# domerin0/rnn-speech

Measured on AMD Instinct MI355X. Metric: audio_frames_per_sec_train_3x512_lstm_ctc, higher is better.
Workload: dtype f32

## Files before the change

### include/amdspeech.h

```cpp
#ifndef AMDSPEECH_H
#define AMDSPEECH_H

#include <stddef.h>
#include <stdint.h>

#ifdef __cplusplus
extern "C" {
#endif

#define AMDSPEECH_OK 0
#define AMDSPEECH_EINVAL (-1)
#define AMDSPEECH_EHIP (-2)
#define AMDSPEECH_EUNSUPPORTED (-3)
#define AMDSPEECH_ETIMEOUT (-4)

int amdspeech_version(void);
const char* amdspeech_last_error(void);
int amdspeech_device_cu_count(void);

int amdspeech_linear_fwd(void* stream, const float* x, const float* w, const float* b,
                         float* y, int M, int K, int N);
int amdspeech_linear_bwd(void* stream, const float* x, const float* w, const float* dy,
                         float* dx, float* dw, float* db, int M, int K, int N);

// ... 30 lines not shown
                               float* C, int ldc, const float* bias, int accumulate, void* scratch, size_t scratch_bytes);
int amdspeech_gemm_bf16_packed_plan(int transA, int transB, int M, int N, int K, int lda, int ldb, amdspeech_gemm_plan_info* out);
int amdspeech_bf16_copy(void* stream, const float* src, long ld, long rows, int cols, int transpose, unsigned short* dst, long ldd,
                        float* colsum, unsigned short* plain);
int amdspeech_bf16_transpose(void* stream, const unsigned short* src, long rows, int cols, unsigned short* dst, long ldd);

int amdspeech_batchnorm_fwd(void* stream, const float* x, float* y, float* xhat,
                            float* inv_std, int T, int B, int H, float eps);
int amdspeech_batchnorm_bwd(void* stream, const float* dy, const float* xhat,
                            const float* inv_std, float* dx, int T, int B, int H);

int amdspeech_batchnorm_sum(void* stream, const float* x, const float* global_sum, int n_total, float* out,
                            int T, int B, int H);
int amdspeech_batchnorm_apply(void* stream, const float* x, const float* global_sum, const float* global_sq,
                              int n_total, float eps, float* y, float* xhat, float* inv_std, int T, int B, int H);
int amdspeech_batchnorm_bwd_sums(void* stream, const float* dy, const float* xhat, float* sums, int T, int B, int H);
int amdspeech_batchnorm_bwd_apply(void* stream, const float* dy, const float* xhat, const float* inv_std,
                                  const float* global_sums, int n_total, float* dx, int T, int B, int H);

typedef struct amdspeech_lstm_desc {
    int T, B, H, L;
    float keep_in, keep_out;
    uint64_t seed;
    int precision;
    int flags;
} amdspeech_lstm_desc;

enum { AMDSPEECH_LSTM_ARMED = 1, AMDSPEECH_LSTM_ARM_NEXT = 2, AMDSPEECH_LSTM_SAME_WS = 4, AMDSPEECH_LSTM_PER_DIAGONAL = 8,
       AMDSPEECH_LSTM_INJECT_TIMEOUT = 16 };

enum {
    AMDSPEECH_LSTM_WS_Z0 = 0,
    AMDSPEECH_LSTM_WS_ZTOP = 1,
    AMDSPEECH_LSTM_WS_DZTOP = 2,
    AMDSPEECH_LSTM_WS_DZ0 = 3,
    AMDSPEECH_LSTM_WS_HFINAL = 4,
    AMDSPEECH_LSTM_WS_CFINAL = 5,
    AMDSPEECH_LSTM_WS_GATES = 6
};
size_t amdspeech_lstm_workspace_bytes(const amdspeech_lstm_desc* d);
void* amdspeech_lstm_ws_ptr(const amdspeech_lstm_desc* d, void* ws, int which);

int amdspeech_lstm_workspace_release(void* stream, void* ws);

int amdspeech_lstm_beside_forward(void* stream, const void* ws);

int amdspeech_lstm_beside_tail(void* stream, const void* ws);

int amdspeech_lstm_fwd(void* stream, const amdspeech_lstm_desc* d, void* ws,
                       const float* kernels, long kernel_stride,
                       const float* biases, long bias_stride,
                       const int* lengths, const float* h0, const float* c0);
int amdspeech_lstm_pair_fusable(const amdspeech_lstm_desc* d);
int amdspeech_lstm_fwd_pair(void* stream, const amdspeech_lstm_desc* d_a, void* ws_a, const float* kernels_a, const float* biases_a,
                            const amdspeech_lstm_desc* d_b, void* ws_b, const float* kernels_b, const float* biases_b,
                            long kernel_stride, long bias_stride, const int* lengths, const float* h0_a, const float* c0_a);
int amdspeech_lstm_bwd_pair(void* stream, const amdspeech_lstm_desc* d_a, void* ws_a, const float* kernels_a, float* dkernels_a, float* dbiases_a,
                            const amdspeech_lstm_desc* d_b, void* ws_b, const float* kernels_b, float* dkernels_b, float* dbiases_b,
                            long kernel_stride, long bias_stride, const int* lengths);
int amdspeech_lstm_status(const amdspeech_lstm_desc* d, void* ws);
int amdspeech_lstm_bwd(void* stream, const amdspeech_lstm_desc* d, void* ws,
                       const float* kernels, long kernel_stride,
                       float* dkernels, float* dbiases, long bias_stride,
                       const int* lengths);

typedef struct amdspeech_ctc_head {
    const float* w_out;
    const float* b_out;
    float* logits;
    const int* dense_labels;
    float* loss;
    float* dlogits;
    void* ctc_ws;
    int C, U;
} amdspeech_ctc_head;
int amdspeech_lstm_ctc_fusable(const amdspeech_lstm_desc* d, int C, int U);
int amdspeech_lstm_fwd_ctc(void* stream, const amdspeech_lstm_desc* d, void* ws,
                           const float* kernels, long kernel_stride, const float* biases, long bias_stride,
                           const int* lengths, const float* h0, const float* c0, const amdspeech_ctc_head* head);
int amdspeech_lstm_bwd_ctc(void* stream, const amdspeech_lstm_desc* d, void* ws,
                           const float* kernels, long kernel_stride, float* dkernels, float* dbiases, long bias_stride,
                           const int* lengths, const amdspeech_ctc_head* head);

int amdspeech_lstm_dropout_multipliers(void* stream, const amdspeech_lstm_desc* d, int which, int layer, float* out);

enum { AMDSPEECH_LSTM_PATH_FLOW = 0, AMDSPEECH_LSTM_PATH_BIG1 = 1, AMDSPEECH_LSTM_PATH_BIG = 2, AMDSPEECH_LSTM_PATH_HOIST = 3,
       AMDSPEECH_LSTM_PATH_DIAG = 4, AMDSPEECH_LSTM_PATH_DIAG_BF3 = 5 };
typedef struct amdspeech_lstm_plan_info {
    int fwd_path, bwd_path, nmt, kb, mv, wpx, uw, fwd_mt, pair, bf16p, bf16p_reserved, xw_parts, nfw, w_pieces, dz0_inkernel, flow2_q;
} amdspeech_lstm_plan_info;
int amdspeech_lstm_plan(const amdspeech_lstm_desc* d, int C, int U, amdspeech_lstm_plan_info* out);
int amdspeech_lstm_plan_xw_halves(const amdspeech_lstm_desc* d, int C, int U);

enum {
    AMDSPEECH_BIDIR_WS_Z0 = 0, AMDSPEECH_BIDIR_WS_YTOP_FW = 1, AMDSPEECH_BIDIR_WS_YTOP_BW = 2, AMDSPEECH_BIDIR_WS_DYTOP_FW = 3,
    AMDSPEECH_BIDIR_WS_DYTOP_BW = 4, AMDSPEECH_BIDIR_WS_DZ0 = 5, AMDSPEECH_BIDIR_WS_HFINAL = 6, AMDSPEECH_BIDIR_WS_CFINAL = 7
};
size_t amdspeech_lstm_bidir_workspace_bytes(const amdspeech_lstm_desc* d);
void* amdspeech_lstm_bidir_ws_ptr(const amdspeech_lstm_desc* d, void* ws, int which);
long amdspeech_lstm_bidir_layer_stride(const amdspeech_lstm_desc* d);
int amdspeech_lstm_bidir_path(const amdspeech_lstm_desc* d);
int amdspeech_lstm_bidir_fwd(void* stream, const amdspeech_lstm_desc* d, void* ws, const float* const* kernels,
                             const float* const* biases, const int* lengths, const float* h0, const float* c0);
int amdspeech_lstm_bidir_bwd(void* stream, const amdspeech_lstm_desc* d, void* ws, const float* const* kernels,
                             float* const* dkernels, float* const* dbiases, const int* lengths);
int amdspeech_lstm_bidir_status(const amdspeech_lstm_desc* d, void* ws);
int amdspeech_lstm_bidir_dropout_multipliers(void* stream, const amdspeech_lstm_desc* d, int dir, int which, int layer, float* out);

size_t amdspeech_ctc_workspace_bytes(int T, int B, int C, int U);
int amdspeech_ctc_loss_fwd_bwd(void* stream, const float* logits, const int* dense_labels,
                               const int* lengths, int T, int B, int C, int U,
                               float* loss, float* dlogits, void* ws);
int amdspeech_ctc_loss_fwd_bwd_staged(void* stream, const float* logits, const int* dense_labels,
                                      const int* lengths, int T, int B, int C, int U, float* loss,
                                      float* dlogits, void* ws, int stage);

enum { AMDSPEECH_CTC_KERNEL_WAVE = 0, AMDSPEECH_CTC_KERNEL_SHIFT = 1, AMDSPEECH_CTC_KERNEL_PAIR = 2, AMDSPEECH_CTC_KERNEL_EDGE = 3 };
typedef struct amdspeech_ctc_plan_info {
    int kernel, threads, rmax, smax;
} amdspeech_ctc_plan_info;
int amdspeech_ctc_plan(int T, int B, int C, int U, amdspeech_ctc_plan_info* out);

size_t amdspeech_ctc_align_workspace_bytes(int T, int B, int C, int U);
int amdspeech_ctc_align_plan(int T, int B, int C, int U, amdspeech_ctc_plan_info* out);
int amdspeech_ctc_align(void* stream, const float* logits, const int* dense_labels, const int* lengths,
                        int T, int B, int C, int U, int* frame_label, int* frame_state, int* spans,
                        float* score, float* confidence, void* ws);

int amdspeech_ctc_greedy_decode(void* stream, const float* logits, const int* lengths,
                                int T, int B, int C, int* ids, int* out_len, int* ws);

int amdspeech_merge_repeated(void* stream, int* ids, int* lens, int T, int B, int pad);

int amdspeech_edit_distance(void* stream, const int* a, const int* a_len, int lda, const int* b,
                            const int* b_len, int ldb, int n_pairs, int* out);

int amdspeech_ctc_beam_search_host(const float* logits, const int* lengths, int T, int B, int C,
                                   int beam_width, int merge_repeated, int* ids, int* out_len,
                                   float* log_prob);
int amdspeech_ctc_beam_search_host_mt(const float* logits, const int* lengths, int T, int B, int C,
                                      int beam_width, int merge_repeated, int* ids, int* out_len,
                                      float* log_prob, int max_threads);

int amdspeech_edit_distance_host(const int* a, const int* a_len, int lda, const int* b, const int* b_len, int ldb,
                                 int n_pairs, int* out);

uint32_t amdspeech_crc32c(const void* data, size_t n, uint32_t crc);

int amdspeech_audio_probe(const char* path, int* sample_rate, int* channels, long* frames);
int amdspeech_audio_decode(const char* path, float* out, long capacity, long* frames, int* sample_rate,
                           int verify);

size_t amdspeech_resample_workspace_bytes(int B);
int amdspeech_resample_num_samples(int n_samples, int rate_in, int rate_out);
int amdspeech_resample(void* stream, const float* pcm, const int* n_samples, int B, int n_max, int rate_in,
                       int rate_out, float* out, int out_max, void* ws);

size_t amdspeech_optim_workspace_bytes(long n);
int amdspeech_clip_adam(void* stream, float* params, const float* grads, float* m, float* v,
                        long n, float clip, float lr_t, float beta1, float beta2, float eps,
                        float* norm_out, void* ws);

size_t amdspeech_frontend_workspace_bytes(int mode, int B, int n_max, int sample_rate);
int amdspeech_frontend_num_frames(int mode, int n_samples, int sample_rate);
int amdspeech_frontend_mfcc(void* stream, const float* pcm, const int* n_samples, int B,
                            int n_max, int sample_rate, int n_mfcc, int t_max,
// ... 72 lines not shown
```

### rnn-speech_amd/csrc/ctc.hip

```cpp
#include "common.h"
#include "ctc_core.h"

namespace amdspeech {

__global__ __launch_bounds__(64) void ctc_prepare_kernel(const int* __restrict__ dense, const int* __restrict__ lengths,
                                                         int T, int U, int C, int smax, int* __restrict__ ext,
                                                         int* __restrict__ slen, int* __restrict__ valid) {
    const int b = blockIdx.x, lane = threadIdx.x;
    const int blank = C - 1;
    int* e = ext + (size_t)b * smax;
    for (int s = lane; s < smax; s += 64) e[s] = blank;
    __syncthreads();
    int kept = 0, ntgt = 0;
    bool finished = false;
    const unsigned long long lt = (1ull << lane) - 1ull;
    for (int u0 = 0; u0 < U; u0 += 64) {
        const int u = u0 + lane;
        const int v = (u < U) ? dense[(size_t)b * U + u] : 0;
        const bool nz = v != 0;
        const unsigned long long mnz = __ballot(nz);
        const unsigned long long mterm = __ballot(nz && v >= blank);
        kept += __popcll(mnz);
        if (!finished) {
            unsigned long long before = ~0ull;
            if (mterm) { before = (1ull << (__ffsll((long long)mterm) - 1)) - 1ull; }
            const unsigned long long mt = mnz & before;
            if (nz && ((mt >> lane) & 1ull)) e[2 * (ntgt + __popcll(mt & lt)) + 1] = v;
            ntgt += __popcll(mt);
            if (mterm) finished = true;
        }
    }
    if (lane == 0) {
        if (kept == 0) kept = 1;
        const int len = min(lengths[b], T);
        slen[b] = 2 * ntgt + 1;
        valid[b] = (len > 0 && kept <= len) ? 1 : 0;
    }
}

__global__ __launch_bounds__(256) void log_softmax_kernel(const float* __restrict__ x, float* __restrict__ y,
                                                          long rows, int C) {
    const long row = (long)blockIdx.x * 4 + (threadIdx.x >> 6);
    const int lane = threadIdx.x & 63;
    if (row >= rows) return;
    const float* xr = x + row * C;
    const float lse = ctc_row_lse(xr, C, lane);
    for (int c = lane; c < C; c += 64) y[row * C + c] = xr[c] - lse;
}

__device__ __forceinline__ void ctc_frame_barrier() {
    asm volatile("s_waitcnt lgkmcnt(0)\n\ts_barrier" ::: "memory");
}
template <int RMAX, int PF, int NW>
__global__ __launch_bounds__(NW * 64) void ctc_alpha_beta_kernel(const float* __restrict__ logp, const int* __restrict__ ext,
                                                                 const int* __restrict__ slen, const int* __restrict__ valid,
                                                                 const int* __restrict__ lengths, int T, int B, int C,
                                                                 int smax, float* __restrict__ alpha,
                                                                 float* __restrict__ beta, float* __restrict__ ll) {
    static_assert(RMAX >= 2, "RMAX >= 2");
    constexpr int NT = NW * 64;
    __shared__ double2 edge[2][NT + 4];
    __shared__ double fin[NT];
    constexpr double NEG_INF_D = -__builtin_inf();
    const int b = blockIdx.x, dir = blockIdx.y, tid = threadIdx.x;
    if (!valid[b]) { if (dir == 0 && tid == 0) ll[b] = 0.f; return; }
    const int S = slen[b];
    const int Tb = min(lengths[b], T);
    const int R = (S + NT - 1) / NT;
    const int blank = C - 1;
    const int* e = ext + (size_t)b * smax;
    int lab[RMAX]; bool skip[RMAX]; bool act[RMAX];
#pragma unroll
    for (int r = 0; r < RMAX; ++r) {
        const int s = tid * R + r;
        act[r] = r < R && s < S;
        lab[r] = act[r] ? e[s] : blank;
        if (dir == 0) skip[r] = act[r] && s >= 2 && lab[r] != blank && lab[r] != e[s - 2];
        else skip[r] = act[r] && s + 2 < S && e[s + 2] != blank && e[s + 2] != lab[r];
    }
    if (tid < 4) {
        const int slot = tid < 2 ? tid : NT + tid;
        edge[0][slot] = make_double2(NEG_INF_D, NEG_INF_D);
        edge[1][slot] = make_double2(NEG_INF_D, NEG_INF_D);
    }
    const size_t rowstride = (size_t)B * C;
    const float* lp = logp + (size_t)b * C;
    float* out = (dir == 0 ? alpha : beta) + (size_t)b * T * smax;

    double cur[RMAX];
#pragma unroll
    for (int r = 0; r < RMAX; ++r) {
        const int s = tid * R + r;
        if (dir == 0) cur[r] = (act[r] && s < 2) ? (double)(lp[lab[r]] * LOG2E) : NEG_INF_D;
        else cur[r] = (act[r] && (s == S - 1 || s == S - 2)) ? 0.0 : NEG_INF_D;
        if (act[r]) out[(size_t)(dir == 0 ? 0 : Tb - 1) * smax + s] = (float)cur[r] * LN2;
    }

    auto load_block = [&](int i0, float (&buf)[PF][RMAX]) {
#pragma unroll
        for (int q = 0; q < PF; ++q) {
            const int i = min(i0 + q, Tb - 1);
            const int fr = dir == 0 ? i : Tb - i;
#pragma unroll
            for (int r = 0; r < RMAX; ++r) buf[q][r] = lp[(size_t)fr * rowstride + lab[r]] * LOG2E;
        }
    };
    auto step = [&](int i, const float (&lpv)[RMAX]) {
        double newv[RMAX];
        double2* ed = edge[i & 1] + 2;
        if (dir == 0) {
            double last1 = cur[0], last2 = NEG_INF_D;
#pragma unroll
            for (int r = 1; r < RMAX; ++r) if (r < R) { last2 = last1; last1 = cur[r]; }
            ed[tid] = make_double2(last1, last2);
            ctc_frame_barrier();
            const double2 n1 = ed[tid - 1];
            double p1 = n1.x;
            double p2 = (R == 1) ? ed[tid - 2].x : n1.y;
#pragma unroll
            for (int r = 0; r < RMAX; ++r) {
// ... 591 lines not shown
```

### rnn-speech_amd/csrc/ctc_core.h

```cpp
#pragma once
#include "common.h"

namespace amdspeech {

#define NEG_INF (-__builtin_inff())

struct CtcLayout { size_t logp, alpha, beta, ext, slen, valid, ll, total; int smax; };

static CtcLayout ctc_layout(int T, int B, int C, int U) {
    CtcLayout o;
    o.smax = 2 * U + 1;
    size_t off = 0;
    auto take = [&](size_t bytes) { size_t r = off; off += align_up(bytes, 256); return r; };
    o.logp = take((size_t)T * B * C * 4);
    o.alpha = take((size_t)B * T * o.smax * 4);
    o.beta = take((size_t)B * T * o.smax * 4);
    o.ext = take((size_t)B * o.smax * 4);
    o.slen = take((size_t)B * 4);
    o.valid = take((size_t)B * 4);
    o.ll = take((size_t)B * 4);
    o.total = off;
    return o;
}


struct alignas(64) CtcFlow {
    int on;
    int C, smax;
    int nfw;
    int T, B;
    const int* lengths;
    unsigned* err;
    unsigned long long limit;
    const float* ztp;
    const float* wo;
    const float* wo_pack;
    const float* bo;
    float* logits;
    float* logp;
    float* alpha;
    float* ll;
    float* loss;
    float* dlogits;
    float* dztop;
    const int* ext; const int* slen; const int* valid;
};

constexpr int CF_NTC = 5, CF_RP = 84;
constexpr int CF_FOLLOW_TEAM_FLOATS = 4 * 16 * CF_RP + 16 * CF_RP + 2 * 4 * 16 * 4 + 256 * 2;
constexpr int CF_AP = 388;
constexpr int CF_LEAD_TEAM_FLOATS = 3 * 16 * CF_RP + 2 * 4 * 16 * 4 + 16 * CF_AP;

#ifndef CTC_DIAG
#define CTC_DIAG 0
#endif
__device__ __forceinline__ float lse3(float a, float b, float c) {
    const float m = fmaxf(a, fmaxf(b, c));
    if (m == NEG_INF) return NEG_INF;
    return m + logf(expf(a - m) + expf(b - m) + expf(c - m));
}

constexpr float LOG2E = 1.4426950408889634f, LN2 = 0.6931471805599453f;
__device__ __forceinline__ float lse3_2(float a, float b, float c) {
#if defined(CTC_DIAG) && CTC_DIAG == 4
    return fmaxf(a, fmaxf(b, c)) + 0.3f;
#endif
    const float mm = fmaxf(fmaxf(a, fmaxf(b, c)), -1e30f);
    return mm + __builtin_amdgcn_logf(__builtin_amdgcn_exp2f(a - mm) + __builtin_amdgcn_exp2f(b - mm) +
                                      __builtin_amdgcn_exp2f(c - mm));
}

__device__ __forceinline__ float lse2_2(float a, float b) {
#if defined(CTC_DIAG) && CTC_DIAG == 4
    return fmaxf(a, b) + 0.3f;
#endif
    const float mm = fmaxf(fmaxf(a, b), -1e30f);
    return mm + __builtin_amdgcn_logf(__builtin_amdgcn_exp2f(a - mm) + __builtin_amdgcn_exp2f(b - mm));
}
__device__ __forceinline__ float ctc_from_lane_below(float v) {
    return __int_as_float(__builtin_amdgcn_update_dpp(__float_as_int(NEG_INF), __float_as_int(v), 0x138 , 0xf, 0xf, false));
}
__device__ __forceinline__ double lse2_2d(double a, double b) {
#if defined(CTC_DIAG) && CTC_DIAG == 4
    return fmax(a, b) + 0.3;
#endif
    const double mm = fmax(fmax(a, b), -1e30);
    return mm + (double)__builtin_amdgcn_logf(__builtin_amdgcn_exp2f((float)(a - mm)) + __builtin_amdgcn_exp2f((float)(b - mm)));
}
__device__ __forceinline__ double lse3_2d(double a, double b, double c) {
#if defined(CTC_DIAG) && CTC_DIAG == 4
    return fmax(a, fmax(b, c)) + 0.3;
#endif
    const double mm = fmax(fmax(a, fmax(b, c)), -1e30);
    return mm + (double)__builtin_amdgcn_logf(__builtin_amdgcn_exp2f((float)(a - mm)) + __builtin_amdgcn_exp2f((float)(b - mm)) +
                                              __builtin_amdgcn_exp2f((float)(c - mm)));
}
__device__ __forceinline__ double ctc_from_lane_below(double v) {
    const long long bits = __double_as_longlong(v), ninf = __double_as_longlong(-__builtin_inf());
    const int lo = __builtin_amdgcn_update_dpp((int)ninf, (int)bits, 0x138, 0xf, 0xf, false);
    const int hi = __builtin_amdgcn_update_dpp((int)(ninf >> 32), (int)(bits >> 32), 0x138, 0xf, 0xf, false);
    return __longlong_as_double(((long long)hi << 32) | (unsigned)lo);
}

__device__ __forceinline__ float ctc_row_lse(const float* xr, int C, int lane) {
    float m = NEG_INF;
    for (int c = lane; c < C; c += 64) m = fmaxf(m, xr[c]);
#pragma unroll
    for (int o = 32; o > 0; o >>= 1) m = fmaxf(m, __shfl_xor(m, o));
    float sum = 0.f;
    for (int c = lane; c < C; c += 64) sum += expf(xr[c] - m);
#pragma unroll
    for (int o = 32; o > 0; o >>= 1) sum += __shfl_xor(sum, o);
    return m + logf(sum);
}

}
```

### rnn-speech_amd/csrc/gemm_skinny.hip

```cpp
#include "common.h"
#include <string.h>

namespace amdspeech {

typedef __amdgpu_buffer_rsrc_t sk_rsrc_t;
typedef unsigned sk_u32x4 __attribute__((ext_vector_type(4)));

struct SkinnyArgs {
    const float* A; const float* B; float* C; const float* bias;
    int M, N, K, lda, ldb, ldc, accumulate;
};

constexpr unsigned SK_OOB = 0x80000000u;

__device__ __forceinline__ f32x4 sk_load4(sk_rsrc_t rs, unsigned byte_off) {
    const sk_u32x4 w = __builtin_amdgcn_raw_buffer_load_b128(rs, byte_off, 0, 0);
    f32x4 r;
    r.x = __uint_as_float(w.x); r.y = __uint_as_float(w.y); r.z = __uint_as_float(w.z); r.w = __uint_as_float(w.w);
    return r;
}
__device__ __forceinline__ float sk_load1(sk_rsrc_t rs, unsigned byte_off) {
    return __uint_as_float(__builtin_amdgcn_raw_buffer_load_b32(rs, byte_off, 0, 0));
}

struct SkinnyOut {
    sk_rsrc_t c, c_in, bias;
    __device__ __forceinline__ void init(const SkinnyArgs& g) {
        const unsigned cbytes = (unsigned)(((size_t)(g.M - 1) * g.ldc + g.N) * 4);
        c = __builtin_amdgcn_make_buffer_rsrc(g.C, 0, cbytes, 0x00020000);
        c_in = __builtin_amdgcn_make_buffer_rsrc(g.C, 0, g.accumulate ? cbytes : 0u, 0x00020000);
        bias = __builtin_amdgcn_make_buffer_rsrc(const_cast<float*>(g.bias), 0, g.bias != nullptr ? (unsigned)g.N * 4u : 0u, 0x00020000);
    }
    __device__ __forceinline__ unsigned offset(const SkinnyArgs& g, int row, int n) const {
        return (row < g.M && n < g.N) ? (unsigned)((size_t)row * g.ldc + n) * 4u : SK_OOB;
    }
    __device__ __forceinline__ f32x4 addend(const SkinnyArgs& g, unsigned off, int n) const {
        return sk_load4(bias, n < g.N ? (unsigned)n * 4u : SK_OOB) + sk_load4(c_in, off);
    }
    __device__ __forceinline__ void store(unsigned off, f32x4 v) const {
        sk_u32x4 w;
        w.x = __float_as_uint(v.x); w.y = __float_as_uint(v.y); w.z = __float_as_uint(v.z); w.w = __float_as_uint(v.w);
        __builtin_amdgcn_raw_buffer_store_b128(w, c, off, 0, 0);
    }
};

template <int NT>
__global__ __launch_bounds__(256) void gemm_skinny_n_kernel(SkinnyArgs g) {
    constexpr int KC = 64, LD = NT * 16 + ((NT & 1) ? 4 : 12);
    static_assert((4 * LD) % 32 == 16 && LD % 4 == 0, "bank spread");
    __shared__ __attribute__((aligned(16))) float wt[2][KC][LD];
    const int tid = threadIdx.x, w = tid >> 6, lane = tid & 63, m = lane & 15, kg = lane >> 4;
    const int row = blockIdx.x * 64 + w * 16 + m;
    const sk_rsrc_t ra = __builtin_amdgcn_make_buffer_rsrc(const_cast<float*>(g.A), 0, (unsigned)(((size_t)(g.M - 1) * g.lda + g.K) * 4), 0x00020000);
    const sk_rsrc_t rb = __builtin_amdgcn_make_buffer_rsrc(const_cast<float*>(g.B), 0, (unsigned)(((size_t)(g.K - 1) * g.ldb + g.N) * 4), 0x00020000);
    const int chunks = (g.K + KC - 1) / KC;

    f32x4 wreg[NT], a_cur[4], a_nxt[4];
    auto load_w = [&](int c) __attribute__((always_inline)) {
#pragma unroll
        for (int i = 0; i < NT; ++i) {
            const int slot = i * 256 + tid, k = slot / (4 * NT), n4 = slot % (4 * NT);
            const int kk = c * KC + k;
            const bool ok = n4 * 4 < g.N && kk < g.K;
            wreg[i] = sk_load4(rb, ok ? (unsigned)(kk * g.ldb + n4 * 4) * 4u : SK_OOB);
        }
    };
    auto put_w = [&](int buf) __attribute__((always_inline)) {
#pragma unroll
        for (int i = 0; i < NT; ++i) {
            const int slot = i * 256 + tid, k = slot / (4 * NT), n4 = slot % (4 * NT);
            *reinterpret_cast<f32x4*>(&wt[buf][k][n4 * 4]) = wreg[i];
        }
    };
    auto load_a = [&](int c, f32x4* a) __attribute__((always_inline)) {
#pragma unroll
        for (int s = 0; s < 4; ++s) {
            const int kk = c * KC + 16 * s + 4 * kg;
            const bool ok = row < g.M && kk < g.K;
            a[s] = sk_load4(ra, ok ? (unsigned)((size_t)row * g.lda + kk) * 4u : SK_OOB);
        }
    };

    f32x4 acc[NT];
#pragma unroll
    for (int i = 0; i < NT; ++i) acc[i] = f32x4{0.f, 0.f, 0.f, 0.f};
    load_w(0);
    load_a(0, a_cur);
    put_w(0);
    __syncthreads();
    for (int c = 0; c < chunks; ++c) {
        const int buf = c & 1;
        load_w(c + 1);
        load_a(c + 1, a_nxt);
        __builtin_amdgcn_sched_barrier(0);
        float bq[2][NT][4];
        auto read_b = [&](int s, float (*b)[4]) __attribute__((always_inline)) {
#pragma unroll
            for (int nt = 0; nt < NT; ++nt) {
                const float* col = &wt[buf][16 * s + 4 * kg][nt * 16 + m];
                b[nt][0] = col[0]; b[nt][1] = col[LD]; b[nt][2] = col[2 * LD]; b[nt][3] = col[3 * LD];
            }
        };
        read_b(0, bq[0]);
#pragma unroll
        for (int s = 0; s < 4; ++s) {
            if (s < 3) read_b(s + 1, bq[(s + 1) & 1]);
            __builtin_amdgcn_sched_barrier(0);
#pragma unroll
            for (int j = 0; j < 4; ++j)
#pragma unroll
                for (int nt = 0; nt < NT; ++nt)
                    acc[nt] = __builtin_amdgcn_mfma_f32_16x16x4f32(bq[s & 1][nt][j], a_cur[s][j], acc[nt], 0, 0, 0);
            __builtin_amdgcn_sched_barrier(0);
        }
        put_w(buf ^ 1);
#pragma unroll
        for (int s = 0; s < 4; ++s) a_cur[s] = a_nxt[s];
        __syncthreads();
    }
    SkinnyOut out;
    out.init(g);
    unsigned off[NT];
    f32x4 add[NT];
#pragma unroll
    for (int nt = 0; nt < NT; ++nt) {
        off[nt] = out.offset(g, row, nt * 16 + 4 * kg);
        add[nt] = out.addend(g, off[nt], nt * 16 + 4 * kg);
    }
#pragma unroll
    for (int nt = 0; nt < NT; ++nt) out.store(off[nt], acc[nt] + add[nt]);
}

template <int KT, bool B_KC>
__global__ __launch_bounds__(256) void gemm_skinny_k_kernel(SkinnyArgs g) {
    const int tid = threadIdx.x, w = tid >> 6, lane = tid & 63, m = lane & 15, kg = lane >> 4;
    const int row0 = blockIdx.x * 128 + w * 32;
    const sk_rsrc_t ra = __builtin_amdgcn_make_buffer_rsrc(const_cast<float*>(g.A), 0, (unsigned)(((size_t)(g.M - 1) * g.lda + g.K) * 4), 0x00020000);
    const size_t b_extent = B_KC ? (size_t)(g.N - 1) * g.ldb + g.K : (size_t)(g.K - 1) * g.ldb + g.N;
    const sk_rsrc_t rb = __builtin_amdgcn_make_buffer_rsrc(const_cast<float*>(g.B), 0, (unsigned)(b_extent * 4), 0x00020000);
    SkinnyOut out;
    out.init(g);

    f32x4 a[2][KT];
#pragma unroll
    for (int mt = 0; mt < 2; ++mt)
#pragma unroll
        for (int kt = 0; kt < KT; ++kt) {
            const int row = row0 + mt * 16 + m, kk = 16 * kt + 4 * kg;
            const bool ok = row < g.M && kk < g.K;
            a[mt][kt] = sk_load4(ra, ok ? (unsigned)((size_t)row * g.lda + kk) * 4u : SK_OOB);
        }
    struct Tile { f32x4 b[2][KT], bias[2], old[2][2]; unsigned off[2][2]; };
    auto fetch = [&](int nt, Tile& t) __attribute__((always_inline)) {
#pragma unroll
        for (int q = 0; q < 2; ++q) {
            const int n = (nt + q) * 16 + m;
#pragma unroll
            for (int kt = 0; kt < KT; ++kt) {
                const int kk = 16 * kt + 4 * kg;
                const bool ok = n < g.N && kk < g.K;
                if (B_KC) {
                    t.b[q][kt] = sk_load4(rb, ok ? (unsigned)(n * g.ldb + kk) * 4u : SK_OOB);
                } else {
                    const unsigned o = ok ? (unsigned)(kk * g.ldb + n) * 4u : SK_OOB;
                    const unsigned st = ok ? (unsigned)g.ldb * 4u : 0u;
                    t.b[q][kt].x = sk_load1(rb, o);
                    t.b[q][kt].y = sk_load1(rb, o + st);
                    t.b[q][kt].z = sk_load1(rb, o + 2 * st);
                    t.b[q][kt].w = sk_load1(rb, o + 3 * st);
                }
            }
            const int nc = (nt + q) * 16 + 4 * kg;
            t.bias[q] = sk_load4(out.bias, nc < g.N ? (unsigned)nc * 4u : SK_OOB);
#pragma unroll
            for (int mt = 0; mt < 2; ++mt) {
                t.off[mt][q] = out.offset(g, row0 + mt * 16 + m, nc);
                t.old[mt][q] = sk_load4(out.c_in, t.off[mt][q]);
            }
        }
    };
    auto tile = [&](int nt, const Tile& cur, Tile& nxt) __attribute__((always_inline)) {
        fetch(nt + 2, nxt);
        __builtin_amdgcn_sched_barrier(0);
        f32x4 acc[2][2];
#pragma unroll
        for (int mt = 0; mt < 2; ++mt)
#pragma unroll
            for (int q = 0; q < 2; ++q) acc[mt][q] = cur.bias[q] + cur.old[mt][q];
#pragma unroll
        for (int kt = 0; kt < KT; ++kt)
#pragma unroll
            for (int j = 0; j < 4; ++j)
#pragma unroll
                for (int mt = 0; mt < 2; ++mt)
#pragma unroll
                    for (int q = 0; q < 2; ++q)
                        acc[mt][q] = __builtin_amdgcn_mfma_f32_16x16x4f32(cur.b[q][kt][j], a[mt][kt][j], acc[mt][q], 0, 0, 0);
#pragma unroll
        for (int mt = 0; mt < 2; ++mt)
#pragma unroll
            for (int q = 0; q < 2; ++q) out.store(cur.off[mt][q], acc[mt][q]);
        __builtin_amdgcn_sched_barrier(0);
    };
    const int all_tiles = (g.N + 15) / 16;
    const int per = ((all_tiles + (int)gridDim.y - 1) / (int)gridDim.y + 1) & ~1;
    const int nt0 = (int)blockIdx.y * per, ntiles = min(all_tiles, nt0 + per);
    Tile t0, t1;
    fetch(nt0, t0);
    for (int nt = nt0; nt < ntiles; nt += 4) {
        tile(nt, t0, t1);
        if (nt + 2 >= ntiles) break;
        tile(nt + 2, t1, t0);
    }
}

#ifndef SKTN_DIAG
#define SKTN_DIAG 0
#endif
struct SkinnyTnArgs {
    const float* S; const float* W; float* C; float* colsum;
    int K, s, wide, lds, ldw, ldc;
    int chunk;
    int nslices;
    int small_is_a;
    int colsum_small;
};

template <int FULL, int RT>
__global__ __launch_bounds__(512) void gemm_skinny_tn_kernel(SkinnyTnArgs g) {
    constexpr int NTS = 4 * FULL + RT;
    constexpr int PD = NTS <= 4 ? 4 : 2;
    constexpr int SP = 64 * FULL + 16 * RT, LDR = 65;
    constexpr int NF = FULL > 0 ? FULL : 1, NR = RT > 0 ? RT : 1;
    extern __shared__ __attribute__((aligned(16))) float lds[];
    const int tid = threadIdx.x, w = tid >> 6, lane = tid & 63, i = lane & 15, kq = lane >> 4;
    const int v = blockIdx.x, xcd = v & 7, q = v >> 3;
    const int chunk_id = xcd + 8 * (q / g.nslices), slice = q % g.nslices;
    const int r0 = chunk_id * g.chunk;
    if (r0 >= g.K) return;
    const sk_rsrc_t rs = __builtin_amdgcn_make_buffer_rsrc(const_cast<float*>(g.S), 0, (unsigned)(((size_t)(g.K - 1) * g.lds + g.s) * 4), 0x00020000);
    const sk_rsrc_t rw = __builtin_amdgcn_make_buffer_rsrc(const_cast<float*>(g.W), 0, (unsigned)(((size_t)(g.K - 1) * g.ldw + g.wide) * 4), 0x00020000);

    const int wcol = slice * 64 + 4 * i;
    const bool w_ok = wcol < g.wide;
    const bool ones_wanted = g.colsum != nullptr && !g.colsum_small;
    const int rem = g.s - 64 * FULL;
    const int rcol = 64 * FULL + RT * i;
    bool r_valid[NR];
#pragma unroll
    for (int e = 0; e < NR; ++e) r_valid[e] = RT > 0 && rcol + e < g.s;
    const bool ones_lane = ones_wanted && RT > 0 && i == rem / NR;
    const int ones_e = rem % NR;
    const bool cs_small = g.colsum != nullptr && g.colsum_small && slice == 0;
    const int groups = g.chunk / 32;
    f32x4 smf[PD][NF], wd[PD];
    float smr[PD][NR];
    auto fetch = [&](int t, int p) __attribute__((always_inline)) {
        const int row = r0 + 4 * (8 * t + w) + kq;
        const bool r_ok = row < g.K && t < groups;
        wd[p] = sk_load4(rw, (r_ok && w_ok) ? (unsigned)((size_t)row * g.ldw + wcol) * 4u : SK_OOB);
#pragma unroll
        for (int b = 0; b < FULL; ++b) smf[p][b] = sk_load4(rs, r_ok ? (unsigned)((size_t)row * g.lds + 64 * b + 4 * i) * 4u : SK_OOB);
        if (RT > 0) {
            const unsigned off = (r_ok && r_valid[0]) ? (unsigned)((size_t)row * g.lds + rcol) * 4u : SK_OOB;
            if (RT == 1) {
                smr[p][0] = sk_load1(rs, off);
            } else if (RT == 2) {
                typedef unsigned u2 __attribute__((ext_vector_type(2)));
                const u2 x = __builtin_amdgcn_raw_buffer_load_b64(rs, off, 0, 0);
                smr[p][0] = __uint_as_float(x.x); smr[p][1 % NR] = __uint_as_float(x.y);
            } else if (RT == 3) {
                typedef unsigned u3 __attribute__((ext_vector_type(3)));
                const u3 x = __builtin_amdgcn_raw_buffer_load_b96(rs, off, 0, 0);
                smr[p][0] = __uint_as_float(x.x); smr[p][1 % NR] = __uint_as_float(x.y); smr[p][2 % NR] = __uint_as_float(x.z);
            } else {
                const f32x4 x = sk_load4(rs, off);
                smr[p][0] = x.x; smr[p][1 % NR] = x.y; smr[p][2 % NR] = x.z; smr[p][3 % NR] = x.w;
            }
        }
    };
    f32x4 acc[NTS][4], csf[NF];
    float csr[NR];
#pragma unroll
    for (int b = 0; b < NF; ++b) csf[b] = f32x4{0.f, 0.f, 0.f, 0.f};
#pragma unroll
    for (int e = 0; e < NR; ++e) csr[e] = 0.f;
#pragma unroll
    for (int ts = 0; ts < NTS; ++ts)
#pragma unroll
        for (int ew = 0; ew < 4; ++ew) acc[ts][ew] = f32x4{0.f, 0.f, 0.f, 0.f};
#pragma unroll
    for (int p = 0; p < PD; ++p) fetch(p, p);
    for (int t0 = 0; t0 < groups; t0 += PD) {
#pragma unroll
        for (int p = 0; p < PD; ++p) {
            float sv[NTS];
// ... 273 lines not shown
```

### rnn-speech_amd/csrc/lstm.hip

```cpp
#include "common.h"
#include "gemm_core.h"
#include "ctc_core.h"
#include <stdlib.h>
#include <string.h>
#include <type_traits>
#include <mutex>
#include <unordered_map>

namespace amdspeech {

#define FLOW_WEIGHTS_RESIDENT() __builtin_amdgcn_s_waitcnt(0x0F70)
static unsigned long long* dev_trace_ptr() {
#ifdef AMDSPEECH_DEVTRACE
    if (const char* e = dev_knob_str("AMDSPEECH_TRACE_PTR")) return reinterpret_cast<unsigned long long*>(strtoull(e, nullptr, 0));
#endif
    return nullptr;
}
#ifndef BIG_WEIGHTS_RESIDENT
#define BIG_WEIGHTS_RESIDENT 1
#endif

struct LstmLayout {
    size_t wp, wq, z, hs, cs, gates, dg, dztop, dz0, dc, xp0, xp, hp, dgp, sync, xph, hph, dxh, prec, pdown, xwp, bigring, wopack, bfs, total;
    size_t fwd_set = 0;
};

static bool flow_shape_ok(const amdspeech_lstm_desc* d) {
    return (d->precision == 0 || ((d->precision == 1 || d->precision == 2) && d->H % 256 == 0)) && d->H % 128 == 0 && d->H <= 512 && (long)d->L * ((d->B + 15) / 16) <= 8 &&
           (size_t)d->T * ((d->B + 15) / 16 * 16) * 4 * d->H * 4 < (1ull << 32);
}
static bool fwd_workers_fit(const amdspeech_lstm_desc* d) {
    const long groups = (long)d->L * ((d->B + 15) / 16);
    return d->precision == 0 && d->H == 512 && groups < 8 && (size_t)d->T * groups * (d->H / 16) * 4096 < (1ull << 32);
}
#ifndef FWD2_WORKER_RESERVE
#define FWD2_WORKER_RESERVE 8
#endif
static int fwd_worker_wgs_per_xcd(const amdspeech_lstm_desc* d, int waves) {
    const int groups = d->L * ((d->B + 15) / 16), spare = 8 - groups;
    const int wgs = (groups * (d->H / 16) + waves - 1) / waves;
    return (wgs + spare - 1) / spare;
}
static bool fwd_half_roles_fit(const amdspeech_lstm_desc* d) {
    const long groups = (long)d->L * ((d->B + 15) / 16);
    return fwd_workers_fit(d) && fwd_worker_wgs_per_xcd(d, 4) <= 32 - FWD2_WORKER_RESERVE &&
           (size_t)d->T * groups * (d->H / 16) * 6144 < (1ull << 32);
}
static bool bf16p_layout_reserved(const amdspeech_lstm_desc* d) {
    static const int env = runtime_switch("AMDSPEECH_BF16_PACKED", 1);
    return env != 0 && d->precision == 2 && d->H == 1024;
}
static bool bf16p_layout_on(const amdspeech_lstm_desc* d) {
    return bf16p_layout_reserved(d) && ((long)d->T * d->B) % 64 == 0 && (long)d->T * d->B >= 256;
}
struct Bf16pBufs { unsigned short *zb, *wtb, *dgb, *wb, *zht, *dgt; char* partial; size_t partial_bytes; };
static size_t bf16p_scratch_floats(const amdspeech_lstm_desc* d) {
    const size_t TB = ((size_t)d->T * d->B + 63) / 64 * 64, H = d->H;
    const size_t bytes = TB * H * 2 + 4 * H * H * 2 + TB * 4 * H * 2 + H * 4 * H * 2 + 2 * H * TB * 2 + 4 * H * TB * 2 +
                         bf16p_partial_bytes_max() + 8 * 256;
    return (bytes + 3) / 4;
}
static Bf16pBufs bf16p_bufs(const amdspeech_lstm_desc* d, float* base) {
    const size_t TB = (size_t)d->T * d->B, H = d->H;
    char* p = reinterpret_cast<char*>(base);
    auto take = [&](size_t bytes) { char* r = p; p += align_up(bytes, 256); return r; };
    Bf16pBufs b;
    b.zb = reinterpret_cast<unsigned short*>(take(TB * H * 2));
    b.wtb = reinterpret_cast<unsigned short*>(take(4 * H * H * 2));
    b.dgb = reinterpret_cast<unsigned short*>(take(TB * 4 * H * 2));
    b.wb = reinterpret_cast<unsigned short*>(take(H * 4 * H * 2));
    b.zht = reinterpret_cast<unsigned short*>(take(2 * H * TB * 2));
    b.dgt = reinterpret_cast<unsigned short*>(take(4 * H * TB * 2));
    b.partial_bytes = bf16p_partial_bytes_max();
    b.partial = take(b.partial_bytes);
    return b;
}
static int bf16p_xw(hipStream_t s, const Bf16pBufs& b, int rows, int H, const float* Z, const float* K, float* G, const float* bias) {
    if (int rc = bf16p_copy(s, Z, H, rows, H, false, b.zb, H, nullptr)) return rc;
    if (int rc = bf16p_copy(s, K, 4 * H, H, 4 * H, true, b.wtb, H, nullptr)) return rc;
    return bf16p_gemm(s, rows, 4 * H, H, b.zb, H, b.wtb, H, G, 4 * H, bias, false, b.partial, b.partial_bytes);
}
static int bf16p_dx(hipStream_t s, const Bf16pBufs& b, int rows, int H, const float* dG, const float* K, float* dX) {
    if (int rc = bf16p_copy(s, dG, 4 * H, rows, 4 * H, false, b.dgb, 4 * H, nullptr)) return rc;
    if (int rc = bf16p_copy(s, K, 4 * H, H, 4 * H, false, b.wb, 4 * H, nullptr)) return rc;
    return bf16p_gemm(s, rows, H, 4 * H, b.dgb, 4 * H, b.wb, 4 * H, dX, H, nullptr, false, b.partial, b.partial_bytes);
}
static int bf16p_layer_bwd(hipStream_t s, const Bf16pBufs& b, int rows, int H, const float* Z, const float* Hp, const float* dG, const float* K,
                           float* dX, float* dK, float* dbias) {
    if (int rc = bf16p_copy(s, dG, 4 * H, rows, 4 * H, true, b.dgt, rows, dbias, b.dgb)) return rc;
    if (int rc = bf16p_copy(s, K, 4 * H, H, 4 * H, false, b.wb, 4 * H, nullptr)) return rc;
    if (int rc = bf16p_gemm(s, rows, H, 4 * H, b.dgb, 4 * H, b.wb, 4 * H, dX, H, nullptr, false, b.partial, b.partial_bytes)) return rc;
    if (int rc = bf16p_copy(s, Z, H, rows, H, true, b.zht, rows, nullptr)) return rc;
    if (int rc = bf16p_copy(s, Hp, H, rows, H, true, b.zht + (size_t)H * rows, rows, nullptr)) return rc;
    return bf16p_gemm(s, 2 * H, 4 * H, rows, b.zht, rows, b.dgt, rows, dK, 4 * H, nullptr, true, b.partial, b.partial_bytes);
}
static int bf16p_layer_bwd_copied(hipStream_t s, const Bf16pBufs& b, int rows, int H, const float* Z, const float* Hp, const float* K,
                                  float* dX, float* dK) {
    if (int rc = bf16p_copy(s, K, 4 * H, H, 4 * H, false, b.wb, 4 * H, nullptr)) return rc;
    if (int rc = bf16p_gemm(s, rows, H, 4 * H, b.dgb, 4 * H, b.wb, 4 * H, dX, H, nullptr, false, b.partial, b.partial_bytes)) return rc;
    if (int rc = bf16p_copy(s, Z, H, rows, H, true, b.zht, rows, nullptr)) return rc;
    if (int rc = bf16p_copy(s, Hp, H, rows, H, true, b.zht + (size_t)H * rows, rows, nullptr)) return rc;
    if (int rc = bf16p_transpose(s, b.dgb, rows, 4 * H, b.dgt, rows)) return rc;
    return bf16p_gemm(s, 2 * H, 4 * H, rows, b.zht, rows, b.dgt, rows, dK, 4 * H, nullptr, true, b.partial, b.partial_bytes);
}
static int bf16p_dk(hipStream_t s, const Bf16pBufs& b, int rows, int H, const float* Z, const float* Hp, const float* dG, float* dK, float* dbias) {
    if (int rc = bf16p_copy(s, Z, H, rows, H, true, b.zht, rows, nullptr)) return rc;
    if (int rc = bf16p_copy(s, Hp, H, rows, H, true, b.zht + (size_t)H * rows, rows, nullptr)) return rc;
    if (int rc = bf16p_copy(s, dG, 4 * H, rows, 4 * H, true, b.dgt, rows, dbias)) return rc;
    return bf16p_gemm(s, 2 * H, 4 * H, rows, b.zht, rows, b.dgt, rows, dK, 4 * H, nullptr, true, b.partial, b.partial_bytes);
}

static int check_desc(const amdspeech_lstm_desc* d) {
    AS_CHECK_ARG(d != nullptr, "lstm: null descriptor");
    AS_CHECK_ARG(d->T > 0 && d->B > 0 && d->H > 0 && d->L > 0, "lstm: bad shape T=%d B=%d H=%d L=%d",
                 d->T, d->B, d->H, d->L);
    AS_CHECK_ARG(d->H % 16 == 0, "lstm: hidden size %d must be a multiple of 16", d->H);
    AS_CHECK_ARG(d->keep_in > 0.f && d->keep_in <= 1.f && d->keep_out > 0.f && d->keep_out <= 1.f,
                 "lstm: keep probabilities must be in (0,1]");
    AS_CHECK_ARG((size_t)d->T * d->B * d->H < (1ull << 32), "lstm: T*B*H too large for the dropout counter");
    AS_CHECK_ARG(d->precision == 0 || ((d->precision == 1 || d->precision == 2) && d->H % 32 == 0),
                 "lstm: precision %d unsupported (0 = f32; 1 = bf16x3, 2 = bf16: both need H %% 32 == 0, H = %d)", d->precision, d->H);
    AS_CHECK_ARG((d->flags & ~(AMDSPEECH_LSTM_ARMED | AMDSPEECH_LSTM_ARM_NEXT | AMDSPEECH_LSTM_SAME_WS | AMDSPEECH_LSTM_PER_DIAGONAL |
                               AMDSPEECH_LSTM_INJECT_TIMEOUT)) == 0, "lstm: unknown flags 0x%x", d->flags);
    return AMDSPEECH_OK;
}

struct DropCfg { float keep_in, keep_out; uint64_t seed; int L; };

__device__ __forceinline__ float zmult(const DropCfg& c, int lp, uint32_t idx) {
    float m = 1.0f;
    if (c.keep_in < 1.0f && lp < c.L)
        m *= (uniform01(c.seed, 2u * lp, idx) < c.keep_in) ? (1.0f / c.keep_in) : 0.0f;
    if (c.keep_out < 1.0f && lp >= 1)
        m *= (uniform01(c.seed, 2u * (lp - 1) + 1u, idx) < c.keep_out) ? (1.0f / c.keep_out) : 0.0f;
    return m;
}

__global__ void apply_zmult_kernel(float* x, long n, DropCfg c, int lp) {
    long i = (long)blockIdx.x * blockDim.x + threadIdx.x;
    if (i < n) x[i] *= zmult(c, lp, (uint32_t)i);
}

__global__ void pack_fwd_kernel(const float* __restrict__ kernels, long kstride, float* __restrict__ wp,
                                int H, int L, int UW, int grouped) {
    const int NT = UW / 4, NKB = 2 * H / 16, NUB = H / UW;
    const long total = (long)L * 2 * H * 4 * H;
    long o = (long)blockIdx.x * blockDim.x + threadIdx.x;
    if (o >= total) return;
    int m = o & 3, lane = (o >> 2) & 63;
    long r = o >> 8;
    int nt = r % NT; r /= NT;
    int kb = r % NKB; r /= NKB;
    int ub = r % NUB; int l = r / NUB;
    int j = lane & 15, kq = lane >> 4;
    int c = nt * 16 + j, g = c / UW, u = c % UW;
    if (grouped) { g = j >> 2; u = nt * 4 + (j & 3); }
    int k = kb * 16 + 4 * kq + m;
    wp[o] = kernels[l * kstride + (long)k * 4 * H + g * H + ub * UW + u];
}

__global__ void pack_bwd_kernel(const float* __restrict__ kernels, long kstride, float* __restrict__ wq,
                                int H, int L) {
    const int NRB = 2 * H / 16, NKB = 4 * H / 16;
    const long total = (long)L * 2 * H * 4 * H;
    long o = (long)blockIdx.x * blockDim.x + threadIdx.x;
    if (o >= total) return;
    int m = o & 3, lane = (o >> 2) & 63;
    long r = o >> 8;
    int kb = r % NKB; r /= NKB;
    int rb = r % NRB; int l = r / NRB;
    int row = rb * 16 + (lane & 15), col = kb * 16 + 4 * (lane >> 4) + m;
    wq[o] = kernels[l * kstride + (long)row * 4 * H + col];
}

__device__ __forceinline__ size_t packed_off(int row, int k, int K) {
    return ((((size_t)(row >> 4) * (K >> 4) + (k >> 4)) * 64) + (((k >> 2) & 3) * 16 + (row & 15))) * 4 + (k & 3);
}

__global__ void pack_rows_kernel(const float* __restrict__ src, size_t src_stride, float* __restrict__ dst,
                                 int B, int K, int nmat) {
    const size_t per = (size_t)B * K;
    const size_t i = (size_t)blockIdx.x * blockDim.x + threadIdx.x;
    if (i >= per * nmat) return;
    const int mat = i / per;
    const size_t r = i % per;
    const int row = r / K, k = r % K;
    const size_t bpk = (size_t)((B + 15) / 16 * 16) * K;
    dst[(size_t)mat * bpk + packed_off(row, k, K)] = src[(size_t)mat * src_stride + r];
}

__global__ __launch_bounds__(256) void mask_pack_rows_kernel(float* __restrict__ z, float* __restrict__ dst, int B, int K, int T,
                                                             DropCfg c, int masked) {
    const size_t per4 = (size_t)B * K / 4;
    const size_t i = (size_t)blockIdx.x * blockDim.x + threadIdx.x;
    if (i >= per4 * T) return;
    const int t = i / per4;
    const size_t r = (i % per4) * 4;
    const int row = r / K, k = r % K;
    const size_t e = (size_t)t * B * K + r;
    float4 v = *reinterpret_cast<const float4*>(z + e);
    if (masked) {
        v.x *= zmult(c, 0, (uint32_t)e); v.y *= zmult(c, 0, (uint32_t)(e + 1));
        v.z *= zmult(c, 0, (uint32_t)(e + 2)); v.w *= zmult(c, 0, (uint32_t)(e + 3));
        *reinterpret_cast<float4*>(z + e) = v;
    }
    const size_t bpk = (size_t)((B + 15) / 16 * 16) * K;
    *reinterpret_cast<float4*>(dst + (size_t)t * bpk + packed_off(row, k, K)) = v;
}

__global__ __launch_bounds__(256) void flow_fwd_prepare_kernel(const float* __restrict__ h0, const float* __restrict__ c0,
                                                               float* __restrict__ hs, float* __restrict__ cs,
                                                               float* __restrict__ hph, unsigned* __restrict__ sync_words,
                                                               int T, int B, int H, int L) {
    const int bp = (B + 15) / 16 * 16;
    const size_t per = (size_t)bp * H;
    const size_t i = (size_t)blockIdx.x * blockDim.x + threadIdx.x;
    if (i < 40) sync_words[i] = 0u;
    if (i >= per * L) return;
    const int l = i / per;
    const size_t r = i % per;
    const int row = r / H, k = r % H;
    float hv = 0.f;
    if (row < B) {
        const size_t e = (size_t)row * H + k, bh = (size_t)B * H;
        hv = h0 ? h0[l * bh + e] : 0.f;
        hs[(size_t)l * (T + 1) * bh + e] = hv;
        cs[(size_t)l * (T + 1) * bh + e] = c0 ? c0[l * bh + e] : 0.f;
    }
    hph[(size_t)l * (T + 1) * per + packed_off(row, k, H)] = hv;
}

__device__ __forceinline__ float sigmoidf_(float x) { return 1.0f / (1.0f + expf(-x)); }

#include "lstm_step_fwd.h"
#include "lstm_flow.h"
}
#include "ctc_flow.h"
namespace amdspeech {

#include "lstm_flow_fwd.h"
#include "lstm_big_fwd.h"
#include "lstm_step_bwd.h"
#include "lstm_flow_bwd.h"
#include "lstm_big_bwd.h"
#include "lstm_step_bf3.h"
constexpr int PROF_SEGS = 16;
static bool g_prof_on = false;
static hipEvent_t g_prof_ev[2][PROF_SEGS][2];
static int g_prof_launches[2] = {0, 0};
static int g_prof_nseg[2] = {0, 0};
static bool g_prof_valid[2] = {false, false};
static double g_prof_flops[2][2] = {{0, 0}, {0, 0}};
static void prof_flops(int which, double recurrence, double other) { g_prof_flops[which][0] = recurrence; g_prof_flops[which][1] = other; }

static void prof_begin(int which, hipStream_t s, int seg = 0) {
    if (g_prof_on && seg < PROF_SEGS) (void)hipEventRecord(g_prof_ev[which][seg][0], s);
}
static void prof_end(int which, hipStream_t s, int launches, int seg = 0) {
    if (!g_prof_on || seg >= PROF_SEGS) return;
    (void)hipEventRecord(g_prof_ev[which][seg][1], s);
    g_prof_launches[which] = launches;
    g_prof_nseg[which] = seg + 1;
    g_prof_valid[which] = true;
}

static hipStream_t g_side = nullptr;
static hipEvent_t g_fork = nullptr;
static int side_stream_init() {
    if (g_side) return AMDSPEECH_OK;
    AS_CHECK_HIP(hipStreamCreateWithFlags(&g_side, hipStreamNonBlocking));
    AS_CHECK_HIP(hipEventCreateWithFlags(&g_fork, hipEventDisableTiming));
    return AMDSPEECH_OK;
}
static hipStream_t g_chain = nullptr, g_gemm = nullptr;
static hipEvent_t g_ev_a = nullptr, g_ev_b = nullptr, g_ev_c = nullptr;
static int g_overlap_state = 0;
static int overlap_init() {
    if (g_overlap_state != 0) return g_overlap_state;
    g_overlap_state = -1;
    int dev = 0, cus = 0;
    if (hipGetDevice(&dev) != hipSuccess) return -1;
    if (hipDeviceGetAttribute(&cus, hipDeviceAttributeMultiprocessorCount, dev) != hipSuccess || cus != 256) return -1;
    uint32_t chain_mask[8] = {0, 0, ~0u, ~0u, ~0u, ~0u, ~0u, ~0u}, gemm_mask[8] = {~0u, ~0u, 0, 0, 0, 0, 0, 0};
    if (hipExtStreamCreateWithCUMask(&g_chain, 8, chain_mask) != hipSuccess) return -1;
    if (hipExtStreamCreateWithCUMask(&g_gemm, 8, gemm_mask) != hipSuccess) return -1;
    if (hipEventCreateWithFlags(&g_ev_a, hipEventDisableTiming) != hipSuccess) return -1;
    if (hipEventCreateWithFlags(&g_ev_b, hipEventDisableTiming) != hipSuccess) return -1;
    if (hipEventCreateWithFlags(&g_ev_c, hipEventDisableTiming) != hipSuccess) return -1;
    g_overlap_state = 1;
    return 1;
}
constexpr int DK_CHUNKS = 8, DK_SIDE = 5;

static int gemm_reduced(const amdspeech_lstm_desc* d, hipStream_t s, bool ta, bool tb, int M, int N, int K, const float* A, int lda,
                        const float* B, int ldb, float* C, int ldc, const float* bias, bool accumulate) {
    return (d->precision == 2 ? gemm_bf16 : gemm_bf3)(s, ta, tb, M, N, K, A, lda, B, ldb, C, ldc, bias, accumulate);
}
static int gemm_batched(const amdspeech_lstm_desc* d, hipStream_t s, bool ta, bool tb, int M, int N, int K, const float* A, int lda,
                        const float* B, int ldb, float* C, int ldc, const float* bias, bool accumulate) {
    if (d->precision != 0) return gemm_reduced(d, s, ta, tb, M, N, K, A, lda, B, ldb, C, ldc, bias, accumulate);
    return gemm_f32(s, ta, tb, M, N, K, A, lda, B, ldb, C, ldc, bias, accumulate);
}
static int pick_uw(const amdspeech_lstm_desc* d) {
    const long wgs8 = (long)d->L * (d->H / 8) * ceil_div(d->B, 32);
    return (d->H % 8 == 0 && wgs8 >= 96) ? 8 : 4;
}

static int device_cus() {
    static int cus = -1;
    if (cus < 0) {
        int dev = 0;
        if (hipGetDevice(&dev) != hipSuccess ||
            hipDeviceGetAttribute(&cus, hipDeviceAttributeMultiprocessorCount, dev) != hipSuccess) cus = 0;
    }
    return cus;
}

static bool use_big_fwd(const amdspeech_lstm_desc* d) {
    static const int env = runtime_switch("AMDSPEECH_BIG", 1);
    return env != 0 && !(d->flags & AMDSPEECH_LSTM_PER_DIAGONAL) && d->precision >= 0 && d->precision <= 2 && d->H == 1024 &&
           (d->B + 15) / 16 <= 4 && device_cus() == 256 &&
           (size_t)2 * ((d->B + 15) / 16 * 16) * d->H * 4 < (1ull << 32);
}

static bool use_flow(const amdspeech_lstm_desc* d) {
    static const int env = runtime_switch("AMDSPEECH_FLOW", 1);
    return env != 0 && !(d->flags & AMDSPEECH_LSTM_PER_DIAGONAL) && flow_shape_ok(d) && device_cus() == 256 && d->L * ((d->B + 15) / 16) <= 8;
}

template <bool CF>
static void (*flow_fwd_kernel(int kb, int pr, int mv, int mh))(FlowArgs) {
    switch (kb) {
        case 1: return lstm_fwd_flow2<1, 0, 0, CF>;
        case 2: return pr == 2 ? lstm_fwd_flow2<2, 2, 0, CF> : (pr == 1 ? lstm_fwd_flow2<2, 1, 0, CF> : lstm_fwd_flow2<2, 0, 0, CF>);
        case 3: return lstm_fwd_flow2<3, 0, 0, CF>;
        default:
            if (pr == 0 && mv == 1) return mh == 1 ? lstm_fwd_flow2<4, 0, 1, CF, 1> : lstm_fwd_flow2<4, 0, 1, CF>;
            return pr == 2 ? lstm_fwd_flow2<4, 2, 0, CF> : (pr == 1 ? lstm_fwd_flow2<4, 1, 0, CF> : lstm_fwd_flow2<4, 0, 0, CF>);
    }
}
template <bool CF>
static void (*flow_bwd_kernel(int kb, int pr))(FlowBwdArgs) {
    if (pr == 2) return kb == 2 ? lstm_bwd_flow2<2, 2, CF> : lstm_bwd_flow2<4, 2, CF>;
    if (pr == 1) return kb == 2 ? lstm_bwd_flow2<2, 1, CF> : lstm_bwd_flow2<4, 1, CF>;
    return kb == 1 ? lstm_bwd_flow2<1, 0, CF> : (kb == 2 ? lstm_bwd_flow2<2, 0, CF> : (kb == 3 ? lstm_bwd_flow2<3, 0, CF> : lstm_bwd_flow2<4, 0, CF>));
}
static int flow_fill_fwd_panels(hipStream_t s, const amdspeech_lstm_desc* d, float* ws, const LstmLayout& lo, int set) {
    const size_t bph = (size_t)(d->B + 15) / 16 * 16 * d->H;
    float* base = ws + (size_t)set * lo.fwd_set;
    AS_CHECK_HIP(hipMemsetD32Async(reinterpret_cast<hipDeviceptr_t>(base + lo.xph + (size_t)d->T * bph), (int)FLOW_SENTINEL,
                                   (size_t)d->L * d->T * bph, s));
    AS_CHECK_HIP(hipMemsetD32Async(reinterpret_cast<hipDeviceptr_t>(base + lo.hph), (int)FLOW_SENTINEL, (size_t)d->L * (d->T + 1) * bph, s));
    return AMDSPEECH_OK;
}
static int flow_fill_bwd_panels(hipStream_t s, const amdspeech_lstm_desc* d, float* ws, const LstmLayout& lo, bool ctc_head = false) {
    const size_t bpg = (size_t)((d->B + 15) / 16) * 16 * 4 * d->H;
    AS_CHECK_HIP(hipMemsetAsync(ws + lo.prec, 0, (lo.total - lo.prec) * sizeof(float), s));
    if (ctc_head)
        AS_CHECK_HIP(hipMemsetD32Async(reinterpret_cast<hipDeviceptr_t>(ws + lo.dztop), (int)FLOW_SENTINEL, (size_t)d->T * d->B * d->H, s));
    if (d->L > 1)
        AS_CHECK_HIP(hipMemsetD32Async(reinterpret_cast<hipDeviceptr_t>(ws + lo.dxh), (int)FLOW_SENTINEL,
                                       (size_t)(d->L - 1) * d->T * (bpg / 4), s));
    return AMDSPEECH_OK;
}
struct ArmState {
    hipEvent_t join = nullptr; bool pending = false;
    hipEvent_t pre = nullptr; int idle_xcds = 0;
    hipEvent_t post = nullptr; int post_flags = 0;
    int clean_set = 0;
    int xw_par = -1;
    int xw_cover = 0;
    long xw_key = 0;
};
static std::mutex g_arm_mutex;
static std::unordered_map<const void*, ArmState> g_arm;
static int flow_xw_parity(hipStream_t s, const void* ws, bool trust, long key, float* xwp, size_t frame_floats, int T, unsigned* par) {
    std::lock_guard<std::mutex> lock(g_arm_mutex);
    ArmState& st = g_arm[ws];
    if (trust && st.xw_par >= 0 && st.xw_key == key) {
        const int old = st.xw_par;
        if (T > st.xw_cover)
            AS_CHECK_HIP(hipMemsetD32Async(reinterpret_cast<hipDeviceptr_t>(xwp + (size_t)st.xw_cover * frame_floats), old,
                                           (size_t)(T - st.xw_cover) * frame_floats, s));
        st.xw_par = old ^ 1;
    } else {
        AS_CHECK_HIP(hipMemsetAsync(xwp, 0, (size_t)T * frame_floats * sizeof(float), s));
        st.xw_par = 1;
    }
    st.xw_cover = T; st.xw_key = key;
    *par = (unsigned)st.xw_par;
    return AMDSPEECH_OK;
}
static void flow_xw_forget(const void* ws) {
    std::lock_guard<std::mutex> lock(g_arm_mutex);
    auto it = g_arm.find(ws);
    if (it != g_arm.end()) it->second.xw_par = -1;
}
static int flow_arm_fork(hipStream_t s) {
    if (int rc = side_stream_init()) return rc;
    AS_CHECK_HIP(hipEventRecord(g_fork, s));
    AS_CHECK_HIP(hipStreamWaitEvent(g_side, g_fork, 0));
    return AMDSPEECH_OK;
}
static int flow_clean_set(const void* ws) {
    std::lock_guard<std::mutex> lock(g_arm_mutex);
    auto it = g_arm.find(ws);
    return it == g_arm.end() ? 0 : it->second.clean_set;
}
static int flow_arm_publish(const void* ws, int clean_set) {
    std::lock_guard<std::mutex> lock(g_arm_mutex);
    ArmState& st = g_arm[ws];
    st.clean_set = clean_set;
    if (!st.join) AS_CHECK_HIP(hipEventCreateWithFlags(&st.join, hipEventDisableTiming));
    AS_CHECK_HIP(hipEventRecord(st.join, g_side));
    st.pending = true;
    return AMDSPEECH_OK;
}
static int flow_arm_settle(hipStream_t s, const void* ws) {
    std::lock_guard<std::mutex> lock(g_arm_mutex);
    auto it = g_arm.find(ws);
    if (it == g_arm.end() || !it->second.pending) return AMDSPEECH_OK;
    AS_CHECK_HIP(hipStreamWaitEvent(s, it->second.join, 0));
    it->second.pending = false;
    return AMDSPEECH_OK;
}
static int flow_arm_release(hipStream_t s, const void* ws) {
    std::lock_guard<std::mutex> lock(g_arm_mutex);
    auto it = g_arm.find(ws);
    if (it == g_arm.end()) return AMDSPEECH_OK;
    if (it->second.pending) AS_CHECK_HIP(hipStreamWaitEvent(s, it->second.join, 0));
    if (it->second.join) (void)hipEventDestroy(it->second.join);
    if (it->second.pre) (void)hipEventDestroy(it->second.pre);
    if (it->second.post) (void)hipEventDestroy(it->second.post);
    g_arm.erase(it);
    return AMDSPEECH_OK;
}
static int flow_mark_postlaunch(hipStream_t s, const void* ws, int flags) {
    std::lock_guard<std::mutex> lock(g_arm_mutex);
    ArmState& st = g_arm[ws];
    st.post_flags = flags;
    if (flags == 0) return AMDSPEECH_OK;
    if (!st.post) AS_CHECK_HIP(hipEventCreateWithFlags(&st.post, hipEventDisableTiming));
    AS_CHECK_HIP(hipEventRecord(st.post, s));
    return AMDSPEECH_OK;
}
static int flow_mark_prelaunch(hipStream_t s, const void* ws, int idle_xcds) {
    std::lock_guard<std::mutex> lock(g_arm_mutex);
    ArmState& st = g_arm[ws];
    st.idle_xcds = idle_xcds;
    if (idle_xcds <= 0) return AMDSPEECH_OK;
    if (!st.pre) AS_CHECK_HIP(hipEventCreateWithFlags(&st.pre, hipEventDisableTiming));
    AS_CHECK_HIP(hipEventRecord(st.pre, s));
    return AMDSPEECH_OK;
}

static int ctc_head_nfw(const amdspeech_lstm_desc* d, int C, int U, int wpx) {
    static const int env = runtime_switch("AMDSPEECH_FLOW_CTC", 1);
    if (env == 0) return 0;
    const int groups = d->L * ((d->B + 15) / 16), spare = 8 - groups, smax = 2 * U + 1;
    if (spare < 1 || C < 16 || C > 16 * CF_NTC || C % 16 != 0 || U < 1 || smax > 384 || d->H % 64 != 0) return 0;
    if ((size_t)d->B * d->T * smax * 4 >= (1ull << 31) || (size_t)d->T * d->B * d->H * 4 >= (1ull << 31)) return 0;
    int nfw = 32 - wpx < 4 ? 32 - wpx : 4;
    if (nfw < 1 || d->B > spare * nfw * 2 * 2) return 0;
    return nfw;
}
static CtcFlow ctc_head_args(const amdspeech_lstm_desc* d, const amdspeech_ctc_head* h, float* ws, const LstmLayout& lo, float* panels, int nfw) {
    const CtcLayout cl = ctc_layout(d->T, d->B, h->C, h->U);
    char* w = static_cast<char*>(h->ctc_ws);
    CtcFlow c;
    c.on = 1; c.C = h->C; c.smax = cl.smax; c.nfw = nfw; c.T = d->T; c.B = d->B;
    c.ztp = panels ? panels + lo.xph + (size_t)d->L * d->T * ((size_t)(d->B + 15) / 16 * 16 * d->H) : nullptr;
    c.wo = h->w_out; c.wo_pack = ws + lo.wopack; c.bo = h->b_out;
    c.logits = h->logits; c.logp = reinterpret_cast<float*>(w + cl.logp); c.alpha = reinterpret_cast<float*>(w + cl.alpha);
    c.ll = reinterpret_cast<float*>(w + cl.ll); c.loss = h->loss; c.dlogits = h->dlogits; c.dztop = ws + lo.dztop;
    c.ext = reinterpret_cast<const int*>(w + cl.ext); c.slen = reinterpret_cast<const int*>(w + cl.slen);
    c.valid = reinterpret_cast<const int*>(w + cl.valid);
    return c;
}

// ... 81 lines not shown

    static const int workers_env = runtime_switch("AMDSPEECH_FLOW_FWD_WORKERS", 2);
    const int groups = L * p.nmt, spare = 8 - groups;
    p.wpw = 8;
    if (workers_env != 0 && p.xw_parts > 0)
        for (int waves = 4; waves <= 8 && p.mv == 0; waves += 4) {
            const int per = fwd_worker_wgs_per_xcd(d, waves);
            if (per <= 32 - FWD2_WORKER_RESERVE) { p.mv = 1; p.wpx = per; p.wpw = waves; }
        }
    p.mh = (workers_env != 1 && p.mv == 1 && p.wpw == 4 && p.xw_half > 0) ? 1 : 0;
    if (head != nullptr) p.nfw = ctc_head_nfw(d, head->C, head->U, p.wpx);
    const int kb = H / 128;
    p.fwd_flow = head != nullptr ? flow_fwd_kernel<true>(kb, pr, p.mv, p.mh) : flow_fwd_kernel<false>(kb, pr, p.mv, p.mh);
    p.bwd_flow = head != nullptr ? flow_bwd_kernel<true>(kb, pr) : flow_bwd_kernel<false>(kb, pr);
    p.fwd_lds = head != nullptr ? (size_t)2 * CF_FOLLOW_TEAM_FLOATS * sizeof(float) : 0;
    p.bwd_lds = ((size_t)2 * 1024 + 2 * 8 * 256 + (FLOW2_WINDOW ? 2 : 1) * 8 * kb * 256 + (size_t)(flow2_q(kb, pr) - 1) * 1024) * sizeof(float);
    const size_t lds_workers = (size_t)2 * 2 * 2 * BK * LDS_LD * sizeof(float);
    if (p.bwd_lds < lds_workers) p.bwd_lds = lds_workers;
    if (p.bwd_lds < (size_t)2 * CF_LEAD_TEAM_FLOATS * sizeof(float)) p.bwd_lds = (size_t)2 * CF_LEAD_TEAM_FLOATS * sizeof(float);

    const FlowGemmShare g = flow_gemm_share();
    const bool workers = g.pieces > 0 && g.percent > 0 && T >= 64 && groups < 8 && H % 128 == 0;
    const int share = g.set ? g.percent : (pr != 0 ? (head != nullptr ? g.percent / 2 - 1 : g.percent * 3 / 4) : g.percent);
    static const int dz0_in = runtime_switch("AMDSPEECH_FLOW_DZ0", 1);
    p.dz0_inkernel = dz0_in ? 1 : 0;
    p.w_dz0 = (p.dz0_inkernel || workers) ? 0 : 1;
    p.w_pieces = workers ? g.pieces : 0;
    static const int deal = runtime_switch("AMDSPEECH_FLOW_WORKER_DEAL", -1);
    p.w_deal = workers && g.pieces <= 8 && (deal > 0 || (deal < 0 && head != nullptr));
    p.w_t0 = workers ? T - (int)((long)T * share / 100) : T;
    if (p.w_t0 < 2) p.w_t0 = 2;
    return p;
}

static LstmLayout lstm_layout(const LstmPlan& p) {
    const size_t T = p.d.T, B = p.d.B, H = p.d.H, L = p.d.L;
    const size_t tbh = T * B * H;
    LstmLayout o;
    size_t off = 0;
    auto take = [&](size_t n) { size_t r = off; off += (n + 63) / 64 * 64; return r; };
    o.xwp = 0;
    if (p.xw_parts > 0) o.xwp = take(T * L * ((B + 15) / 16) * (H / 16) * (p.xw_parts * 1024 + p.xw_half * 512));
    o.wp = take(L * 2 * H * 4 * H);
    o.wq = take(L * 2 * H * 4 * H);
    o.z = take((L + 1) * tbh);
    o.hs = take(L * (T + 1) * B * H);
    o.cs = take(L * (T + 1) * B * H);
    o.gates = take(L * tbh * 4);
    o.dg = take(L * tbh * 4);
    o.dztop = take(tbh);
    o.dz0 = take(tbh);
    o.dc = take(L * 2 * B * H);
    const size_t bp = (B + 15) / 16 * 16;
    o.xp0 = take(T * bp * H);
    o.xp = take(L * 2 * bp * H);
    o.hp = take(L * 2 * bp * H);
    o.dgp = take(L * 2 * bp * 4 * H);
    o.sync = take(64);
    o.xph = o.hph = o.dxh = o.prec = o.pdown = o.wopack = off;
    if (p.flow_shape) {
        o.xph = take((L + 1) * T * bp * H);
        o.hph = take(L * (T + 1) * bp * H);
        o.fwd_set = off - o.xph;
        take((L + 1) * T * bp * H);
        take(L * (T + 1) * bp * H);
        o.wopack = take((H / 16) * CF_NTC * 256);
        o.dxh = take(L * T * bp * H);
        const size_t slot = (size_t)L * (bp / 16) * (H / 16) * (H / 16) * 256;
        o.prec = take(2 * slot);
        o.pdown = take(4 * L * (bp / 16) * (H / 16) * (H / 128) * 256);
        take(L * (bp / 16) * 2 * (H / 16) * 1024);
    }
    o.bigring = off;
    if (p.big_ring) o.bigring = take((size_t)2 * (bp / 16) * (2 * 32 * 32 * 256 + 64 * 1024));
    o.bfs = off;
    if (p.bf16p_reserved) o.bfs = take(bf16p_scratch_floats(&p.d));
    o.total = off;
    return o;
}

struct FwdCall {
    const amdspeech_lstm_desc* d; float* ws; const float* kernels; long kstride; const float* biases; long bstride;
    const int* lengths; const float* h0; const float* c0; const amdspeech_ctc_head* head;
    LstmPlan p; LstmLayout lo;
};
struct BwdCall {
    const amdspeech_lstm_desc* d; float* ws; const float* kernels; long kstride; float* dkernels; float* dbiases; long bstride;
    const int* lengths; const amdspeech_ctc_head* head;
    LstmPlan p; LstmLayout lo;
};
static DropCfg drop_cfg(const amdspeech_lstm_desc* d) { return DropCfg{d->keep_in, d->keep_out, d->seed, d->L}; }
static int mask_dz0(hipStream_t s, const BwdCall& c) {
    if (c.d->keep_in < 1.0f) {
        const long n = (long)c.d->T * c.d->B * c.d->H;
        hipLaunchKernelGGL(apply_zmult_kernel, dim3(ceil_div(n, 256)), dim3(256), 0, s, c.ws + c.lo.dz0, n, drop_cfg(c.d), 0);
        AS_CHECK_LAUNCH();
    }
    return AMDSPEECH_OK;
}

static int fwd_prologue(hipStream_t s, FwdCall& c) {
    const amdspeech_lstm_desc* d = c.d;
    if (int rc = check_desc(d)) return rc;
    AS_CHECK_ARG(c.ws && c.kernels && c.biases && c.lengths, "lstm_fwd: null pointer");
    AS_CHECK_ARG(((uintptr_t)c.ws % 256) == 0, "lstm_fwd: workspace must be 256-byte aligned");
    if (int rc = flow_arm_settle(s, c.ws)) return rc;
    if (int rc = flow_mark_prelaunch(s, c.ws, 0)) return rc;
    c.p = lstm_plan(d, c.head);
    c.lo = lstm_layout(c.p);
    AS_CHECK_ARG(c.head == nullptr || c.p.fwd == Path::flow, "lstm_fwd_ctc: the fused CTC head needs the whole-sequence kernels (amdspeech_lstm_ctc_fusable)");
    prof_flops(0, 0.0, 0.0);
    AS_CHECK_HIP(hipMemsetAsync(c.ws + c.lo.sync, 0, 64, s));
    const long wtotal = (long)d->L * 2 * d->H * 4 * d->H;
    if (c.p.fwd == Path::diag_bf3)
        hipLaunchKernelGGL(pack_fwd_bf3_kernel, dim3(ceil_div(wtotal, 256)), dim3(256), 0, s, c.kernels, c.kstride,
                           reinterpret_cast<unsigned short*>(c.ws + c.lo.wp), d->H, d->L);
    else
        hipLaunchKernelGGL(pack_fwd_kernel, dim3(ceil_div(wtotal, 256)), dim3(256), 0, s, c.kernels, c.kstride,
                           c.ws + c.lo.wp, d->H, d->L, c.p.uw, 0);
    AS_CHECK_LAUNCH();
    return AMDSPEECH_OK;
}
static int fwd_stage(hipStream_t s, const FwdCall& c) {
    const amdspeech_lstm_desc* d = c.d;
    const int T = d->T, B = d->B, H = d->H, L = d->L;
    float* ws = c.ws;
    const LstmLayout& lo = c.lo;
    const size_t bh = (size_t)B * H, bp = (size_t)(B + 15) / 16 * 16, n0 = (size_t)T * bh;
    for (int l = 0; l < L; ++l) {
        float* hs0 = ws + lo.hs + (size_t)l * (T + 1) * bh;
        float* cs0 = ws + lo.cs + (size_t)l * (T + 1) * bh;
        if (c.h0) AS_CHECK_HIP(hipMemcpyAsync(hs0, c.h0 + l * bh, bh * 4, hipMemcpyDeviceToDevice, s));
        else AS_CHECK_HIP(hipMemsetAsync(hs0, 0, bh * 4, s));
        if (c.c0) AS_CHECK_HIP(hipMemcpyAsync(cs0, c.c0 + l * bh, bh * 4, hipMemcpyDeviceToDevice, s));
        else AS_CHECK_HIP(hipMemsetAsync(cs0, 0, bh * 4, s));
    }
    if (d->keep_in < 1.0f) {
        hipLaunchKernelGGL(apply_zmult_kernel, dim3(ceil_div(n0, 256)), dim3(256), 0, s, ws + lo.z, (long)n0, drop_cfg(d), 0);
        AS_CHECK_LAUNCH();
    }
    if (c.p.fwd == Path::diag_bf3) {
        hipLaunchKernelGGL(pack_rows_bf3_kernel, dim3(ceil_div(n0, 256)), dim3(256), 0, s, ws + lo.z, bh,
                           reinterpret_cast<unsigned short*>(ws + lo.xp0), B, H, T);
        for (int l = 0; l < L; ++l)
            hipLaunchKernelGGL(pack_rows_bf3_kernel, dim3(ceil_div(bh, 256)), dim3(256), 0, s,
                               ws + lo.hs + (size_t)l * (T + 1) * bh, bh,
                               reinterpret_cast<unsigned short*>(ws + lo.hp + ((size_t)l * 2 + (l & 1)) * bp * H), B, H, 1);
    } else {
        const bool diag = c.p.fwd == Path::diag;
        if (diag)
            hipLaunchKernelGGL(pack_rows_kernel, dim3(ceil_div(n0, 256)), dim3(256), 0, s, ws + lo.z, bh, ws + lo.xp0, B, H, T);
        for (int l = 0; l < L; ++l)
            hipLaunchKernelGGL(pack_rows_kernel, dim3(ceil_div(bh, 256)), dim3(256), 0, s,
                               ws + lo.hs + (size_t)l * (T + 1) * bh, bh, ws + lo.hp + ((size_t)l * 2 + (diag ? (l & 1) : 0)) * bp * H,
                               B, H, 1);
    }
    AS_CHECK_LAUNCH();
    return AMDSPEECH_OK;
}

static int fwd_flow(hipStream_t s, const FwdCall& c) {
    const amdspeech_lstm_desc* d = c.d;
    const LstmPlan& p = c.p;
    const LstmLayout& lo = c.lo;
    float* ws = c.ws;
    const int T = d->T, B = d->B, H = d->H, L = d->L;
    const size_t bp = (size_t)(B + 15) / 16 * 16, bph = bp * H, bh = (size_t)B * H;
    const DropCfg dc = drop_cfg(d);
    unsigned* err = reinterpret_cast<unsigned*>(ws + lo.sync);
    const int set = (d->flags & AMDSPEECH_LSTM_ARMED) ? flow_clean_set(ws) : 0;
    if (!(d->flags & AMDSPEECH_LSTM_ARMED))
        if (int rc = flow_fill_fwd_panels(s, d, ws, lo, set)) return rc;
    float* const panels = ws + (size_t)set * lo.fwd_set;
    hipLaunchKernelGGL(flow_fwd_prepare_kernel, dim3(ceil_div((long)L * bph, 256)), dim3(256), 0, s, c.h0, c.c0, ws + lo.hs, ws + lo.cs,
                       panels + lo.hph, err, T, B, H, L);
    hipLaunchKernelGGL(mask_pack_rows_kernel, dim3(ceil_div((long)T * bh / 4, 256)), dim3(256), 0, s, ws + lo.z, ws + lo.xp0, B, H, T,
                       dc, d->keep_in < 1.0f ? 1 : 0);
    AS_CHECK_LAUNCH();
    FlowArgs fa;
    fa.wp = ws + lo.wp; fa.bias = c.biases; fa.bias_stride = c.bstride;
    fa.z = ws + lo.z; fa.hs = ws + lo.hs; fa.cs = ws + lo.cs; fa.gates = ws + lo.gates; fa.lengths = c.lengths;
    fa.xp0 = ws + lo.xp0; fa.xph = panels + lo.xph; fa.hph = panels + lo.hph; fa.err = err;
    fa.T = T; fa.B = B; fa.H = H; fa.L = L; fa.drop = dc;
    fa.limit = p.limit;
    fa.trace = dev_trace_ptr(); fa.trace_layer = dev_knob("AMDSPEECH_TRACE_LAYER", L > 1 ? 1 : 0);
    fa.tickets = err + 16;
    fa.xwp = ws + lo.xwp; fa.xw_par = 0u; fa.w_wpx = p.wpx; fa.w_wpw = p.wpw;
    if (p.mv > 0)
        if (int rc = flow_xw_parity(s, ws, (d->flags & (AMDSPEECH_LSTM_ARMED | AMDSPEECH_LSTM_SAME_WS)) != 0,
                                    (((long)B * 4096 + H) * 64 + L) * 8 + p.mv * 2 + p.mh, fa.xwp,
                                    (size_t)L * (bp / 16) * (H / 16) * (p.mv * 1024 + p.mh * 512), T,
                                    &fa.xw_par)) return rc;
    fa.cf = CtcFlow{}; fa.cf_on = 0; fa.cf_nfw = 0;
    if (c.head != nullptr) {
        const amdspeech_ctc_head* head = c.head;
        AS_CHECK_ARG(p.nfw > 0, "lstm_fwd_ctc: this shape does not take the fused CTC head (amdspeech_lstm_ctc_fusable)");
        fa.cf = ctc_head_args(d, head, ws, lo, panels, p.nfw); fa.cf_on = 1; fa.cf_nfw = p.nfw;
        fa.cf.lengths = c.lengths; fa.cf.err = err; fa.cf.limit = fa.limit;
        if (int rc = ctc_prepare_targets(s, head->dense_labels, c.lengths, T, B, head->C, head->U, head->ctc_ws)) return rc;
        hipLaunchKernelGGL(ctc_pack_wo_kernel, dim3(ceil_div((H / 16) * CF_NTC * 64, 256)), dim3(256), 0, s, head->w_out, ws + lo.wopack, H, head->C);
        AS_CHECK_LAUNCH();
        AS_CHECK_HIP(hipFuncSetAttribute(reinterpret_cast<const void*>(p.fwd_flow), hipFuncAttributeMaxDynamicSharedMemorySize, (int)p.fwd_lds));
    }
    prof_begin(0, s);
    const bool arm = (d->flags & AMDSPEECH_LSTM_ARM_NEXT) != 0;
    if (arm)
        if (int rc = flow_arm_fork(s)) return rc;
    if (int rc = flow_mark_prelaunch(s, ws, (p.mv > 0 && c.head == nullptr) ? 0 : 8 - L * p.nmt)) return rc;
    hipLaunchKernelGGL(p.fwd_flow, dim3(256), dim3(512), p.fwd_lds, s, fa);
    prof_end(0, s, T + L - 1);
    prof_flops(0, (double)T * L * 2.0 * B * 2 * H * 4 * H, 0.0);
    AS_CHECK_LAUNCH();
    if (arm) {
        if (int rc = flow_fill_bwd_panels(g_side, d, ws, lo, c.head != nullptr)) return rc;
        const long wtotal = (long)L * 2 * H * 4 * H;
        hipLaunchKernelGGL(pack_bwd_kernel, dim3(ceil_div(wtotal, 256)), dim3(256), 0, g_side, c.kernels, c.kstride, ws + lo.wq, H, L);
        AS_CHECK_LAUNCH();
        if (int rc = flow_fill_fwd_panels(g_side, d, ws, lo, 1 - set)) return rc;
        if (int rc = flow_arm_publish(ws, 1 - set)) return rc;
    }
    return AMDSPEECH_OK;
}

static int big_fwd_layers(hipStream_t s, int n, const FwdCall* st, bool big1) {
    const amdspeech_lstm_desc* d = st[0].d;
    const int T = d->T, B = d->B, H = d->H, L = d->L, nmt = ceil_div(B, 16);
    const size_t TB = (size_t)T * B, bp = (size_t)nmt * 16, bh = (size_t)B * H;
    if (big1) {
        static const hipError_t once = hipFuncSetAttribute(reinterpret_cast<const void*>(lstm_fwd_big1), hipFuncAttributeMaxDynamicSharedMemorySize, BIG1_LDS_BYTES);
        AS_CHECK_HIP(once);
    }
    BigFwd1Args b1;
    b1.n = n;
    for (int k = 0; k < n; ++k) {
        const FwdCall& q = st[k];
        unsigned* err = reinterpret_cast<unsigned*>(q.ws + q.lo.sync);
        BigFwdArgs& ba = b1.b[k];
        ba.wp = q.ws + q.lo.wp; ba.z = q.ws + q.lo.z; ba.hs = q.ws + q.lo.hs; ba.cs = q.ws + q.lo.cs; ba.gates = q.ws + q.lo.gates;
        ba.lengths = q.lengths;
        ba.err = err; ba.tickets = err + 16;
        ba.T = T; ba.B = B; ba.H = H; ba.L = L; ba.drop = drop_cfg(q.d);
        ba.limit = q.p.limit;
    }
    if (n == 1) b1.b[1] = b1.b[0];
    for (int l = 0; l < L; ++l) {
        for (int k = 0; k < n; ++k) {
            const FwdCall& q = st[k];
            float* ws = q.ws;
            const LstmLayout& lk = q.lo;
            const float* z = ws + lk.z + (size_t)l * TB * H;
            float* g = ws + lk.gates + (size_t)l * TB * 4 * H;
            if (int rc = q.p.bf16p ? bf16p_xw(s, bf16p_bufs(q.d, ws + lk.bfs), (int)TB, H, z, q.kernels + l * q.kstride, g, q.biases + l * q.bstride)
                                   : gemm_batched(q.d, s, false, false, (int)TB, 4 * H, H, z, H, q.kernels + l * q.kstride, 4 * H, g, 4 * H,
                                                  q.biases + l * q.bstride, false)) return rc;
            float* ring = ws + lk.hp + (size_t)l * 2 * bp * H;
            AS_CHECK_HIP(hipMemsetAsync(ring, 0, 2 * bp * H * sizeof(float), s));
            hipLaunchKernelGGL(pack_rows_kernel, dim3(ceil_div(bh, 256)), dim3(256), 0, s,
                               ws + lk.hs + (size_t)l * (T + 1) * bh, bh, ring, B, H, 1);
            hipLaunchKernelGGL(tag_panel_kernel, dim3(ceil_div(bp * H, 256)), dim3(256), 0, s, ring, bp * H, 1u);
            AS_CHECK_HIP(hipMemsetAsync(b1.b[k].tickets, 0, 8 * sizeof(unsigned), s));
            b1.b[k].hring = ring; b1.b[k].layer = l;
        }
        if (n == 1) b1.b[1] = b1.b[0];
        prof_begin(0, s, l);
        if (big1) hipLaunchKernelGGL(lstm_fwd_big1, dim3(256), dim3(512), BIG1_LDS_BYTES, s, b1);
        else hipLaunchKernelGGL(st[0].p.fwd_big, dim3(256), dim3(512), 0, s, b1.b[0]);
        prof_end(0, s, T * L, l);
    }
    AS_CHECK_LAUNCH();
    return AMDSPEECH_OK;
}
static int fwd_big(hipStream_t s, const FwdCall& c) {
    if (int rc = fwd_stage(s, c)) return rc;
    return big_fwd_layers(s, 1, &c, c.p.fwd == Path::big1);
}

static int fwd_diag(hipStream_t s, const FwdCall& c) {
    if (int rc = fwd_stage(s, c)) return rc;
    const amdspeech_lstm_desc* d = c.d;
    const int T = d->T, H = d->H, L = d->L;
    float* ws = c.ws;
    const LstmLayout& lo = c.lo;
    FwdArgs a;
    a.xp0 = ws + lo.xp0; a.xp = ws + lo.xp; a.hp = ws + lo.hp;
    a.wp = ws + lo.wp; a.bias = c.biases; a.bias_stride = c.bstride;
    a.z = ws + lo.z; a.hs = ws + lo.hs; a.cs = ws + lo.cs; a.gates = ws + lo.gates; a.lengths = c.lengths;
    a.T = T; a.B = d->B; a.H = H; a.L = L; a.drop = drop_cfg(d);
    a.hoist = 0; a.l0 = 0; a.mt0 = 0; a.dbg = 0;
    a.trace = dev_trace_ptr(); a.trace_d = a.trace ? dev_knob("AMDSPEECH_TRACE_D", T / 2) : -1;
    const dim3 grid = c.p.fwd == Path::diag_bf3 ? dim3(H / 8, L, ceil_div(c.p.nmt, 2)) : dim3(H / c.p.uw, L, c.p.nmt / c.p.fwd_mt);
    prof_begin(0, s);
    for (int dd = 0; dd < T + L - 1; ++dd) {
        a.d = dd;
        hipLaunchKernelGGL(c.p.fwd_diag, grid, dim3(8 * 64), 0, s, a);
    }
    prof_end(0, s, T + L - 1);
    AS_CHECK_LAUNCH();
    return AMDSPEECH_OK;
}

static int lstm_fwd(hipStream_t s, FwdCall c) {
    if (int rc = fwd_prologue(s, c)) return rc;
    switch (c.p.fwd) {
        case Path::flow: return fwd_flow(s, c);
        case Path::big: case Path::big1: return fwd_big(s, c);
        default: return fwd_diag(s, c);
    }
}

static int bwd_prologue(hipStream_t s, BwdCall& c) {
    const amdspeech_lstm_desc* d = c.d;
    if (int rc = check_desc(d)) return rc;
    AS_CHECK_ARG(c.ws && c.kernels && c.dkernels && c.dbiases && c.lengths, "lstm_bwd: null pointer");
    if (int rc = flow_arm_settle(s, c.ws)) return rc;
    if (int rc = flow_mark_postlaunch(s, c.ws, 0)) return rc;
    c.p = lstm_plan(d, c.head);
    c.lo = lstm_layout(c.p);
    const long wtotal = (long)d->L * 2 * d->H * 4 * d->H;
    if (c.p.bwd == Path::diag_bf3)
        hipLaunchKernelGGL(pack_bwd_bf3_kernel, dim3(ceil_div(wtotal, 256)), dim3(256), 0, s, c.kernels, c.kstride,
                           reinterpret_cast<unsigned short*>(c.ws + c.lo.wq), d->H, d->L);
    else if (!(c.p.bwd == Path::flow && (d->flags & AMDSPEECH_LSTM_ARMED)))
        hipLaunchKernelGGL(pack_bwd_kernel, dim3(ceil_div(wtotal, 256)), dim3(256), 0, s, c.kernels, c.kstride, c.ws + c.lo.wq, d->H, d->L);
    AS_CHECK_LAUNCH();
    AS_CHECK_ARG(c.head == nullptr || c.p.bwd == Path::flow, "lstm_bwd_ctc: the fused CTC head needs the whole-sequence kernels (amdspeech_lstm_ctc_fusable)");
    prof_flops(1, 0.0, 0.0);
    return AMDSPEECH_OK;
}
static BwdArgs bwd_args(const BwdCall& c) {
    const amdspeech_lstm_desc* d = c.d;
    float* ws = c.ws;
    const LstmLayout& lo = c.lo;
    BwdArgs a;
    a.hoist = 0; a.l0 = 0; a.mt0 = 0;
    a.wq = ws + lo.wq; a.cs = ws + lo.cs; a.gates = ws + lo.gates; a.dg = ws + lo.dg;
    a.dztop = ws + lo.dztop; a.dc = ws + lo.dc; a.lengths = c.lengths; a.dgp = ws + lo.dgp;
    a.T = d->T; a.B = d->B; a.H = d->H; a.L = d->L; a.drop = drop_cfg(d);
    return a;
}
static int weight_grads(hipStream_t s, const BwdCall& c, int ta, int tb, int dz_tb) {
    const amdspeech_lstm_desc* d = c.d;
    const LstmLayout& lo = c.lo;
    float* ws = c.ws;
    const int T = d->T, B = d->B, H = d->H, L = d->L;
    const size_t TB = (size_t)T * B, r0 = (size_t)ta * B;
    const int rows = (tb - ta) * B, dz_rows = (dz_tb - ta) * B;
    for (int l = 0; l < L; ++l) {
        const float* z = ws + lo.z + ((size_t)l * TB + r0) * H;
        const float* hp = ws + lo.hs + ((size_t)l * (T + 1) * B + r0) * H;
        const float* dg = ws + lo.dg + ((size_t)l * TB + r0) * 4 * H;
        float* dk = c.dkernels + l * c.kstride;
        float* db = c.dbiases + l * c.bstride;
        if (c.p.bf16p && rows % 64 == 0 && rows >= 64) {
            if (int rc = bf16p_dk(s, bf16p_bufs(d, ws + lo.bfs), rows, H, z, hp, dg, dk, db)) return rc;
        } else if (d->precision != 0) {
            if (int rc = gemm_reduced(d, s, true, false, H, 4 * H, rows, z, H, dg, 4 * H, dk, 4 * H, nullptr, true)) return rc;
            if (int rc = colsum_accumulate(s, dg, rows, 4 * H, 4 * H, db)) return rc;
            if (int rc = gemm_reduced(d, s, true, false, H, 4 * H, rows, hp, H, dg, 4 * H, dk + (size_t)H * 4 * H, 4 * H, nullptr, true)) return rc;
        } else {
            const float* pa[2] = {z, hp}; const float* pb[2] = {dg, dg};
            float* pc[2] = {dk, dk + (size_t)H * 4 * H}; float* ps[2] = {db, nullptr};
            if (gemm_f32_tn_group_ok(H, 4 * H, rows, z, H, dg, 4 * H) && gemm_f32_tn_group_ok(H, 4 * H, rows, hp, H, dg, 4 * H)) {
                if (int rc = gemm_f32_tn_group(s, 2, H, 4 * H, rows, pa, H, pb, 4 * H, pc, 4 * H, ps, true)) return rc;
            } else {
                for (int i = 0; i < 2; ++i)
                    if (int rc = gemm_f32(s, true, false, H, 4 * H, rows, pa[i], H, pb[i], 4 * H, pc[i], 4 * H, nullptr, true, ps[i])) return rc;
            }
        }
    }
    if (dz_rows <= 0) return AMDSPEECH_OK;
    const float* dg0 = ws + lo.dg + r0 * 4 * H;
    float* dz0 = ws + lo.dz0 + r0 * H;
    if (c.p.bf16p && dz_rows >= 256) return bf16p_dx(s, bf16p_bufs(d, ws + lo.bfs), dz_rows, H, dg0, c.kernels, dz0);
    return gemm_batched(d, s, false, true, dz_rows, H, 4 * H, dg0, 4 * H, c.kernels, 4 * H, dz0, H, nullptr, false);
}
static int hand_down(hipStream_t s, const BwdCall& c, int l) {
    const amdspeech_lstm_desc* d = c.d;
    const int H = d->H;
    const size_t TB = (size_t)d->T * d->B;
    return gemm_batched(d, s, false, true, (int)TB, H, 4 * H, c.ws + c.lo.dg + (size_t)l * TB * 4 * H, 4 * H, c.kernels + l * c.kstride,
                        4 * H, c.ws + c.lo.dztop, H, nullptr, false);
}

static int bwd_flow(hipStream_t s, const BwdCall& c) {
    const amdspeech_lstm_desc* d = c.d;
    const LstmPlan& p = c.p;
    const LstmLayout& lo = c.lo;
    float* ws = c.ws;
    const int T = d->T, B = d->B, H = d->H, L = d->L;
    unsigned* err = reinterpret_cast<unsigned*>(ws + lo.sync);
    int* progress = reinterpret_cast<int*>(err) + 8;
    unsigned* tickets = err + 16;
    if (!(d->flags & AMDSPEECH_LSTM_ARMED))
        if (int rc = flow_fill_bwd_panels(s, d, ws, lo, c.head != nullptr)) return rc;
    AS_CHECK_HIP(hipMemsetD32Async(reinterpret_cast<hipDeviceptr_t>(progress), T, 8, s));
    AS_CHECK_HIP(hipMemsetAsync(tickets, 0, 16 * sizeof(unsigned), s));
#if FLOW2_CHECK_ORDER
    AS_CHECK_HIP(hipMemsetD32Async(reinterpret_cast<hipDeviceptr_t>(ws + lo.dg), (int)FLOW_SENTINEL, (size_t)L * T * B * 4 * H, s));
    AS_CHECK_HIP(hipMemsetAsync(ws + lo.pdown, 0, (lo.total - lo.pdown) * sizeof(float), s));
#endif
    FlowBwdArgs fb;
    fb.wq = ws + lo.wq; fb.cs = ws + lo.cs; fb.gates = ws + lo.gates; fb.dg = ws + lo.dg; fb.dztop = ws + lo.dztop;
    fb.prec = ws + lo.prec; fb.pdown = ws + lo.pdown;
    fb.nprog = p.nmt; fb.prog_slack = 0;
    fb.dxh = ws + lo.dxh; fb.tickets = tickets; fb.lengths = c.lengths; fb.err = err; fb.progress = progress;
    fb.T = T; fb.B = B; fb.H = H; fb.L = L; fb.drop = drop_cfg(d);
    fb.limit = p.limit;
    fb.trace = dev_trace_ptr();
    fb.trace_layer = dev_knob("AMDSPEECH_TRACE_LAYER", L - 1);
    fb.cf = CtcFlow{}; fb.cf_on = 0;
    if (c.head != nullptr) {
        AS_CHECK_ARG(p.nfw > 0, "lstm_bwd_ctc: this shape does not take the fused CTC head (amdspeech_lstm_ctc_fusable)");
        fb.cf = ctc_head_args(d, c.head, ws, lo, nullptr, p.nfw); fb.cf_on = 1;
        fb.cf.lengths = c.lengths; fb.cf.err = err; fb.cf.limit = fb.limit;
    }
    AS_CHECK_HIP(hipFuncSetAttribute(reinterpret_cast<const void*>(p.bwd_flow), hipFuncAttributeMaxDynamicSharedMemorySize, (int)p.bwd_lds));
    fb.z = ws + lo.z; fb.hs = ws + lo.hs; fb.kernels = c.kernels; fb.dk = c.dkernels; fb.dbias = c.dbiases; fb.dz0 = ws + lo.dz0;
    fb.kstride = c.kstride; fb.bstride = c.bstride;
    fb.dz0_inkernel = p.dz0_inkernel;
    fb.w_dz0 = p.w_dz0;
    fb.w_mode = 0;
    fb.w_pieces = p.w_pieces;
    fb.w_counters = p.w_deal ? tickets + 8 : nullptr;
    fb.w_t0 = p.w_t0;
    prof_begin(1, s);
    hipLaunchKernelGGL(p.bwd_flow, dim3(256), dim3(512), p.bwd_lds, s, fb);
    prof_end(1, s, T + L - 1);
    if (int rc = flow_mark_postlaunch(s, ws, 1 | (fb.dz0_inkernel ? 2 : 0))) return rc;
    {
        const double prod = 2.0 * B * 4 * H * H;
        const double wframes = fb.w_pieces > 0 ? (double)(T - fb.w_t0) : 0.0;
        prof_flops(1, (double)T * (2 * L - 1 + (fb.dz0_inkernel ? 1 : 0)) * prod,
                   wframes * (L * 2.0 * prod + (fb.w_dz0 ? prod : 0.0)));
    }
    AS_CHECK_LAUNCH();
    if (int rc = weight_grads(s, c, 0, p.w_pieces > 0 ? p.w_t0 : T, p.dz0_inkernel ? 0 : T)) return rc;
    return p.dz0_inkernel ? AMDSPEECH_OK : mask_dz0(s, c);
}

static int big1_bwd_layers(hipStream_t s, int n, const BwdCall* st) {
    const amdspeech_lstm_desc* d = st[0].d;
    const int T = d->T, B = d->B, H = d->H, L = d->L, nmt = ceil_div(B, 16);
    const size_t TB = (size_t)T * B;
    const size_t pring_floats = (size_t)2 * nmt * 2 * 32 * 32 * 256, xring_floats = (size_t)2 * nmt * 64 * 1024;
    BigBwd1Args b1;
    b1.n = n;
    for (int k = 0; k < n; ++k) {
        const BwdCall& q = st[k];
        const LstmLayout& lo = q.lo;
        unsigned* err = reinterpret_cast<unsigned*>(q.ws + lo.sync);
        BigBwdArgs& b2 = b1.b[k];
        b2.wq = q.ws + lo.wq; b2.cs = q.ws + lo.cs; b2.gates = q.ws + lo.gates; b2.dg = q.ws + lo.dg; b2.dup = q.ws + lo.dztop;
        b2.lengths = q.lengths; b2.pring = q.ws + lo.bigring; b2.xring = q.ws + lo.bigring + pring_floats; b2.err = err; b2.tickets = err + 16;
        b2.T = T; b2.B = B; b2.H = H; b2.L = L; b2.drop = drop_cfg(q.d);
        b2.limit = q.p.limit;
    }
    for (int l = L - 1; l >= 0; --l) {
        for (int k = 0; k < n; ++k) {
            AS_CHECK_HIP(hipMemsetAsync(b1.b[k].pring, 0, (pring_floats + xring_floats) * sizeof(float), s));
            AS_CHECK_HIP(hipMemsetAsync(b1.b[k].tickets, 0, 8 * sizeof(unsigned), s));
            b1.b[k].layer = l;
            const Bf16pBufs bufs = bf16p_bufs(st[k].d, st[k].ws + st[k].lo.bfs);
            b1.b[k].dgb = bufs.dgb; b1.b[k].dbias = st[k].dbiases + l * st[k].bstride;
        }
        if (n == 1) b1.b[1] = b1.b[0];
        prof_begin(1, s, L - 1 - l);
        hipLaunchKernelGGL(lstm_bwd_big1<BIG1_Q>, dim3(256), dim3(512), 0, s, b1);
        prof_end(1, s, T * L, L - 1 - l);
        for (int k = 0; k < n; ++k) {
            const BwdCall& q = st[k];
            float* ws = q.ws;
            if (int rc = bf16p_layer_bwd_copied(s, bf16p_bufs(q.d, ws + q.lo.bfs), (int)TB, H, ws + q.lo.z + (size_t)l * TB * H,
                                                ws + q.lo.hs + (size_t)l * (T + 1) * B * H, q.kernels + l * q.kstride,
                                                l > 0 ? ws + q.lo.dztop : ws + q.lo.dz0, q.dkernels + l * q.kstride)) return rc;
        }
    }
    AS_CHECK_LAUNCH();
    for (int k = 0; k < n; ++k)
        if (int rc = mask_dz0(s, st[k])) return rc;
// ... 261 lines not shown
}

extern "C" int amdspeech_lstm_fwd_pair(void* stream, const amdspeech_lstm_desc* d_a, void* ws_a, const float* kernels_a, const float* biases_a,
                                       const amdspeech_lstm_desc* d_b, void* ws_b, const float* kernels_b, const float* biases_b,
                                       long kernel_stride, long bias_stride, const int* lengths, const float* h0_a, const float* c0_a) {
    hipStream_t s = static_cast<hipStream_t>(stream);
    AS_CHECK_ARG(d_a && d_b, "lstm_fwd_pair: null descriptor");
    FwdCall two[2] = {{d_a, static_cast<float*>(ws_a), kernels_a, kernel_stride, biases_a, bias_stride, lengths, h0_a, c0_a},
                      {d_b, static_cast<float*>(ws_b), kernels_b, kernel_stride, biases_b, bias_stride, lengths, nullptr, nullptr}};
    if (!pair_together(d_a, ws_a, d_b, ws_b)) {
        if (int rc = lstm_fwd(s, two[0])) return rc;
        return lstm_fwd(s, two[1]);
    }
    for (FwdCall& c : two) {
        if (int rc = fwd_prologue(s, c)) return rc;
        if (int rc = fwd_stage(s, c)) return rc;
    }
    return big_fwd_layers(s, 2, two, true);
}

extern "C" int amdspeech_lstm_bwd_pair(void* stream, const amdspeech_lstm_desc* d_a, void* ws_a, const float* kernels_a, float* dkernels_a,
                                       float* dbiases_a, const amdspeech_lstm_desc* d_b, void* ws_b, const float* kernels_b, float* dkernels_b,
                                       float* dbiases_b, long kernel_stride, long bias_stride, const int* lengths) {
    hipStream_t s = static_cast<hipStream_t>(stream);
    AS_CHECK_ARG(d_a && d_b, "lstm_bwd_pair: null descriptor");
    BwdCall two[2] = {{d_a, static_cast<float*>(ws_a), kernels_a, kernel_stride, dkernels_a, dbiases_a, bias_stride, lengths},
                      {d_b, static_cast<float*>(ws_b), kernels_b, kernel_stride, dkernels_b, dbiases_b, bias_stride, lengths}};
    if (!pair_together(d_a, ws_a, d_b, ws_b) || lstm_plan(d_a, nullptr).bwd != Path::big1) {
        if (int rc = lstm_bwd(s, two[0])) return rc;
        return lstm_bwd(s, two[1]);
    }
    for (BwdCall& c : two)
        if (int rc = bwd_prologue(s, c)) return rc;
    return big1_bwd_layers(s, 2, two);
}

extern "C" int amdspeech_lstm_bwd(void* stream, const amdspeech_lstm_desc* d, void* ws, const float* kernels,
                                  long kernel_stride, float* dkernels, float* dbiases, long bias_stride,
                                  const int* lengths) {
    return lstm_bwd(static_cast<hipStream_t>(stream), BwdCall{d, static_cast<float*>(ws), kernels, kernel_stride, dkernels, dbiases, bias_stride, lengths});
}

extern "C" int amdspeech_lstm_plan(const amdspeech_lstm_desc* d, int C, int U, amdspeech_lstm_plan_info* out) {
    if (int rc = check_desc(d)) return rc;
    AS_CHECK_ARG(out != nullptr, "lstm_plan: null output");
    AS_CHECK_ARG((C > 0 && U > 0) || (C == 0 && U == 0), "lstm_plan: head C=%d U=%d (both 0: no head)", C, U);
    amdspeech_ctc_head h{};
    h.C = C; h.U = U;
    const LstmPlan p = lstm_plan(d, C > 0 ? &h : nullptr);
    const bool flow_bwd = p.bwd == Path::flow;
    static_assert((int)Path::flow == AMDSPEECH_LSTM_PATH_FLOW && (int)Path::big1 == AMDSPEECH_LSTM_PATH_BIG1 &&
                  (int)Path::big == AMDSPEECH_LSTM_PATH_BIG && (int)Path::hoist == AMDSPEECH_LSTM_PATH_HOIST &&
                  (int)Path::diag == AMDSPEECH_LSTM_PATH_DIAG && (int)Path::diag_bf3 == AMDSPEECH_LSTM_PATH_DIAG_BF3, "amdspeech.h");
    *out = amdspeech_lstm_plan_info{(int)p.fwd, (int)p.bwd, p.nmt, p.fwd == Path::flow ? d->H / 128 : 0, p.mv, p.wpx, p.uw, p.fwd_mt,
                                    p.pair ? 1 : 0, p.bf16p ? 1 : 0, p.bf16p_reserved ? 1 : 0, p.xw_parts, p.nfw, p.w_pieces,
                                    p.dz0_inkernel, flow_bwd ? flow2_q(d->H / 128, d->precision) : 0};
    return AMDSPEECH_OK;
}
extern "C" int amdspeech_lstm_plan_xw_halves(const amdspeech_lstm_desc* d, int C, int U) {
    if (check_desc(d) != AMDSPEECH_OK) return -1;
    amdspeech_ctc_head h{};
    h.C = C; h.U = U;
    const LstmPlan p = lstm_plan(d, C > 0 ? &h : nullptr);
    return 2 * p.mv + p.mh;
}
extern "C" int amdspeech_lstm_ctc_fusable(const amdspeech_lstm_desc* d, int C, int U) {
    if (check_desc(d) != AMDSPEECH_OK) return 0;
    amdspeech_ctc_head h{};
    h.C = C; h.U = U;
    return lstm_plan(d, &h).nfw > 0 ? 1 : 0;
}
static int check_head(const amdspeech_ctc_head* h, bool bwd) {
    AS_CHECK_ARG(h != nullptr, "lstm_*_ctc: null head");
    AS_CHECK_ARG(h->w_out && h->b_out && h->logits && h->dense_labels && h->loss && h->ctc_ws && (!bwd || h->dlogits),
                 "lstm_*_ctc: null pointer in the head");
    AS_CHECK_ARG(((uintptr_t)h->w_out % 16) == 0 && ((uintptr_t)h->ctc_ws % 256) == 0, "lstm_*_ctc: W_o must be 16-byte, the CTC workspace 256-byte aligned");
    return AMDSPEECH_OK;
}
extern "C" int amdspeech_lstm_fwd_ctc(void* stream, const amdspeech_lstm_desc* d, void* ws, const float* kernels,
                                      long kernel_stride, const float* biases, long bias_stride, const int* lengths,
                                      const float* h0, const float* c0, const amdspeech_ctc_head* head) {
    if (int rc = check_head(head, false)) return rc;
    return lstm_fwd(static_cast<hipStream_t>(stream), FwdCall{d, static_cast<float*>(ws), kernels, kernel_stride, biases, bias_stride, lengths, h0, c0, head});
}
extern "C" int amdspeech_lstm_bwd_ctc(void* stream, const amdspeech_lstm_desc* d, void* ws, const float* kernels,
                                      long kernel_stride, float* dkernels, float* dbiases, long bias_stride,
                                      const int* lengths, const amdspeech_ctc_head* head) {
    if (int rc = check_head(head, true)) return rc;
    return lstm_bwd(static_cast<hipStream_t>(stream), BwdCall{d, static_cast<float*>(ws), kernels, kernel_stride, dkernels, dbiases, bias_stride, lengths, head});
}

namespace amdspeech {
#include "lstm_layer.h"
#include "lstm_layer_bf3.h"

struct BidirLayout {
    size_t sync, z0, dz0, g[2], dx[2], dy[2], dc[2], total;
    size_t xin[2], hh[2], hc[2], gates[2], y[2];
    size_t per_layer;
    size_t ring[2];
};
static size_t bidir_sync_words(int T) { return 64 + 2 * ((size_t)T + 1); }
static BidirLayout bidir_layout(const amdspeech_lstm_desc* d) {
    const size_t T = d->T, B = d->B, H = d->H, L = d->L, tbh = T * B * H;
    BidirLayout o;
    size_t off = 0;
    auto take = [&](size_t n) { size_t r = off; off += (n + 63) / 64 * 64; return r; };
    o.sync = take(bidir_sync_words(d->T));
    o.z0 = take(tbh);
    o.dz0 = take(tbh);
    for (int k = 0; k < 2; ++k) {
        o.g[k] = take(4 * tbh);
        o.dx[k] = take(2 * tbh);
        o.dy[k] = take(tbh);
        o.dc[k] = take(B * H);
    }
    const size_t start = off;
    for (int k = 0; k < 2; ++k) {
        o.xin[k] = take(2 * tbh);
        o.hh[k] = take((T + 1) * B * H);
        o.hc[k] = take((T + 1) * B * H);
        o.gates[k] = take(4 * tbh);
        o.y[k] = take(tbh);
    }
    o.per_layer = off - start;
    off = start + L * o.per_layer;
    o.ring[0] = o.ring[1] = 0;
    if (d->precision == 1)
        for (int k = 0; k < 2; ++k) o.ring[k] = take(2 * ((B + 15) / 16 * 16) * 4 * H);
    o.total = off;
    return o;
}
static size_t bidir_at(const BidirLayout& o, size_t base, int l) { return base + (size_t)l * o.per_layer; }

static int bf3_kpw(int nkb, int max_waves, int max_kpw) {
    for (int kpw = 1; kpw <= max_kpw; kpw *= 2)
        if (nkb % kpw == 0 && nkb / kpw <= max_waves) return kpw;
    return 0;
}
static int bf3_fwd_kpw(const amdspeech_lstm_desc* d) { return bf3_kpw(d->H / 32, LBF3_FWD_MAXW, 4); }
static int bf3_bwd_kpw(const amdspeech_lstm_desc* d) { return bf3_kpw(4 * d->H / 32, LBF3_BWD_MAXW, 16); }

static int bidir_check(const amdspeech_lstm_desc* d) {
    if (int rc = check_desc(d)) return rc;
    if (d->precision == 2) {
        set_error("lstm_bidir: the layer-wise bidirectional mode runs in exact f32 (precision 0) or bf16x3 (1), not plain bf16 (2)");
        return AMDSPEECH_EUNSUPPORTED;
    }
    if (d->precision == 1 && (d->H > 1024 || bf3_fwd_kpw(d) == 0 || bf3_bwd_kpw(d) == 0)) {
        set_error("lstm_bidir: bf16x3 does not take hidden size %d: its kernels split the H (forward) and 4H (backward) rows of "
                  "W_hh over at most 8 waves, 32 x 1, 2, 4, 8 or 16 rows each (H = 64, 128, 256, 512, 768, 1024 qualify)", d->H);
        return AMDSPEECH_EUNSUPPORTED;
    }
    if (d->H > 1024) {
        set_error("lstm_bidir: hidden size %d above 1024 (the recurrence keeps H x %d floats of W_hh per workgroup in LDS)", d->H, 4 * LAYER_U);
        return AMDSPEECH_EUNSUPPORTED;
    }
    AS_CHECK_ARG((size_t)d->T * d->B * 2 * d->H < (1ull << 32), "lstm_bidir: T*B*2H too large for the dropout counter");
    return AMDSPEECH_OK;
}
struct Bf3Launch {
    void (*kern)(LayerBf3Args);
    int nwg, threads, ngrp;
    size_t lds;
};
static Bf3Launch bf3_launch(const amdspeech_lstm_desc* d, bool bwd) {
// ... 297 lines not shown
```

### rnn-speech_amd/engine.py

```python
import contextlib
import math
import os

import numpy as np
import torch

from . import lib as _lib
from . import ops


def _pad64(n):
    return (n + 63) // 64 * 64


class ParamLayout(object):

    def __init__(self, num_layers, hidden, input_dim, num_labels, bidirectional=False, bidirectional_mode="top"):
        self.L, self.H, self.D, self.C = num_layers, hidden, input_dim, num_labels
        self.bidirectional = bool(bidirectional)
        self.layerwise = self.bidirectional and bidirectional_mode == "layer"
        off = 0
        self.slots = {}

        def take(name, shape):
            nonlocal off
            n = 1
            for s in shape:
                n *= s
            self.slots[name] = (off, shape)
            off += _pad64(n)

        take("input_w", (input_dim, hidden))
        take("input_b", (hidden,))
        def rows(l):
            return (3 if self.layerwise and l > 0 else 2) * hidden

        for l in range(num_layers):
            take("kernel_%d" % l, (rows(l), 4 * hidden))
            take("bias_%d" % l, (4 * hidden,))
        if self.bidirectional:
            for l in range(num_layers):
                take("bw_kernel_%d" % l, (rows(l), 4 * hidden))
                take("bw_bias_%d" % l, (4 * hidden,))
        take("output_w", ((2 if self.bidirectional else 1) * hidden, num_labels))
        take("output_b", (num_labels,))
        self.total = off
        if self.layerwise:
            self.kernel_stride = self.bias_stride = None
        elif num_layers > 1:
            self.kernel_stride = self.slots["kernel_1"][0] - self.slots["kernel_0"][0]
            self.bias_stride = self.slots["bias_1"][0] - self.slots["bias_0"][0]
        else:
            self.kernel_stride = self.bias_stride = 0

    def names(self):
        return list(self.slots.keys())

    def view(self, flat, name):
        off, shape = self.slots[name]
        n = 1
        for s in shape:
            n *= s
        return flat[off:off + n].view(*shape)

    def num_params(self):
        tot = 0
        for _, shape in self.slots.values():
            n = 1
            for s in shape:
                n *= s
            tot += n
        return tot


_BESIDE_FORWARD = os.environ.get("AMDSPEECH_BESIDE_FORWARD", "1") != "0"
_BESIDE_TAIL = os.environ.get("AMDSPEECH_BESIDE_TAIL", "1") != "0"
_BIDIR_PAIR = os.environ.get("AMDSPEECH_BIDIR_PAIR", "1") != "0"
_FUSED_CTC = os.environ.get("AMDSPEECH_FUSED_CTC", "1") != "0"


PRECISIONS = {"f32": 0, "bf16x3": 1, "bf16": 2}


class Engine(object):
    def __init__(self, num_layers, hidden, input_dim, num_labels, batch_size, max_T, max_U,
                 device="cuda", seed=1234, normalization=False, precision="f32", bidirectional=False,
                 sync_batch_norm=False, bidirectional_mode="top"):
        if not torch.cuda.is_available():
            raise RuntimeError("rnn_speech_amd needs a ROCm GPU (MI355X); there is no CPU path")
        self.L, self.H, self.D, self.C = num_layers, hidden, input_dim, num_labels
        self.B, self.T, self.U = batch_size, max_T, max_U
        self.device = torch.device(device)
        self.bidirectional = bool(bidirectional)
        if bidirectional_mode not in ("top", "layer"):
            raise ValueError("bidirectional_mode must be 'top' (two stacks joined in front of the output layer) or 'layer' "
                             "(stack_bidirectional_dynamic_rnn: every layer reads both directions of the layer below)")
        self.layerwise = self.bidirectional and bidirectional_mode == "layer"
        if self.layerwise and precision not in ("f32", "bf16x3"):
            raise ValueError("bidirectional_mode 'layer' runs in exact f32 or bf16x3 (precision %r requested): the layer-wise kernels "
                             "have no plain-bf16 variant" % (precision,))
        self.layout = ParamLayout(num_layers, hidden, input_dim, num_labels, bidirectional=self.bidirectional,
                                  bidirectional_mode="layer" if self.layerwise else "top")
        n = self.layout.total
        self.params = torch.zeros(n, device=self.device)
        self.grads = torch.zeros(n, device=self.device)
        self.adam_m = torch.zeros(n, device=self.device)
        self.adam_v = torch.zeros(n, device=self.device)
        self.norm = torch.zeros(1, device=self.device)
        self.adam_step = 0
        if precision not in PRECISIONS:
            raise ValueError("precision must be 'f32' (exact, default), 'bf16x3' (split-precision MFMA) or 'bf16' (plain bf16 "
                             "operands, f32 accumulation and master weights)")
        self.precision = precision
        if self.layerwise:
            self.lstm_ws = ops.BidirWorkspace(max_T, batch_size, hidden, num_layers, device=self.device, precision=PRECISIONS[precision])
        else:
            self.lstm_ws = ops.LstmWorkspace(max_T, batch_size, hidden, num_layers, device=self.device, precision=PRECISIONS[precision])
        if self.bidirectional and not self.layerwise:
            self.lstm_ws_b = ops.LstmWorkspace(max_T, batch_size, hidden, num_layers, device=self.device,
                                               precision=PRECISIONS[precision])
            self.ytop_b = torch.empty(max_T, batch_size, hidden, device=self.device)
            self.dytop_b = torch.empty(max_T, batch_size, hidden, device=self.device)
        self.ctc_ws = ops.CtcWorkspace(max_T, batch_size, num_labels, max_U, self.device)
        self.logits = torch.empty(max_T, batch_size, num_labels, device=self.device)
        self.dlogits = torch.empty_like(self.logits)
        self.loss = torch.zeros(batch_size, device=self.device)
        self.state_h = torch.zeros(num_layers, batch_size, hidden, device=self.device)
        self.state_c = torch.zeros(num_layers, batch_size, hidden, device=self.device)
        self.normalization = bool(normalization)
        self.sync_batch_norm = bool(sync_batch_norm) and self.normalization
        if self.normalization:
            self.bn_xhat = torch.empty(max_T, batch_size, hidden, device=self.device)
            self.bn_inv_std = torch.empty(max_T, hidden, device=self.device)
            self.bn_scratch = torch.empty(2, max_T, hidden, device=self.device)
        self._ws, self._Tr = self.lstm_ws, max_T
        self._head = None
        self._per_diagonal = False
        self._paired = False
        self._ws_b = self.lstm_ws_b if self.bidirectional and not self.layerwise else None
        self._layer_path = None
        self.stream = torch.cuda.Stream(device=self.device, priority=-1)
        self._aux_stream = None
        self._tail_stream = None
        self.init_parameters(seed)

    def p(self, name):
        return self.layout.view(self.params, name)

    def g(self, name):
        return self.layout.view(self.grads, name)

    def init_parameters(self, seed=1234):
        gen = torch.Generator(device="cpu")
        gen.manual_seed(seed)
        self.params.zero_()
        for name in self.layout.names():
            _, shape = self.layout.slots[name]
            if len(shape) == 2:
                lim = math.sqrt(6.0 / (shape[0] + shape[1]))
                w = (torch.rand(shape, generator=gen) * 2.0 - 1.0) * lim
                self.p(name).copy_(w)

    def load_numpy(self, arrays, flat=None):
        flat = self.params if flat is None else flat
        for name, a in arrays.items():
            if name not in self.layout.slots:
                raise KeyError("unknown parameter tensor %r (layout has %s)" % (name, ", ".join(self.layout.names())))
            want = tuple(self.layout.slots[name][1])
            got = tuple(np.shape(a))
            if got != want:
                raise ValueError("checkpoint tensor %s has shape %s, the model (L=%d, H=%d, D=%d, C=%d) needs %s"
                                 % (name, got, self.L, self.H, self.D, self.C, want))
            self.layout.view(flat, name).copy_(torch.as_tensor(np.asarray(a), dtype=torch.float32))

    def to_numpy(self, flat=None):
        flat = self.params if flat is None else flat
        return {n: self.layout.view(flat, n).detach().cpu().numpy().copy() for n in self.layout.names()}

    @staticmethod
    def _dp_group():
        from . import dataparallel
        return dataparallel.current()

    def _run_length(self, max_len):
        if max_len is None:
            return self.T
        if self.sync_batch_norm and self._dp_group().world > 1:
            return self.T
        return max(1, min(int(max_len), self.T))

    def forward(self, x, lengths, keep_in=1.0, keep_out=1.0, seed=0, use_state=False, max_len=None, after_lstm=None, training=False,
                per_diagonal=False, dense_labels=None):
        T, B, D = x.shape
        assert (T, B, D) == (self.T, self.B, self.D), ((T, B, D), (self.T, self.B, self.D))
        x = x.contiguous()
        Tr = self._run_length(max_len)
        ws = self.lstm_ws.prefix(Tr)
        self._ws, self._Tr = ws, Tr
        ws.set_dropout(keep_in, keep_out, seed)
        ops.linear_fwd(x[:Tr].view(Tr * B, D), self.p("input_w"), self.p("input_b"), out=ws.z0.view(Tr * B, self.H))
        if self.normalization:
            grp = self._dp_group() if self.sync_batch_norm else None
            if grp is not None and grp.world > 1:
                ops.batchnorm_fwd_dp(ws.z0, ws.z0, self.bn_xhat, self.bn_inv_std, grp, self.bn_scratch, 1e-3)
            else:
                ops.batchnorm_fwd(ws.z0, ws.z0, self.bn_xhat[:Tr], self.bn_inv_std[:Tr], 1e-3)
        if self.layerwise:
            return self._forward_layerwise(ws, lengths, keep_in, keep_out, seed, use_state, after_lstm, per_diagonal, Tr)
        if self.bidirectional:
            wb = self.lstm_ws_b.prefix(Tr)
            self._ws_b = wb
            ops.reverse_sequences(ws.z0, lengths, out=wb.z0)
        self._per_diagonal = bool(per_diagonal)
        self._head = None
        if (dense_labels is not None and _FUSED_CTC and not self.bidirectional
                and ops.lstm_ctc_fusable(ws, self.C, dense_labels.shape[1], per_diagonal=per_diagonal)):
            self._head = ops.CtcHead(self.p("output_w"), self.p("output_b"), self.logits[:Tr], dense_labels, self.loss,
                                     self.dlogits[:Tr], self.ctc_ws)
        paired = self.bidirectional and _BIDIR_PAIR and not per_diagonal and ops.lstm_pair_fusable(ws)
        self._paired = bool(paired)
        if paired:
            wb.set_dropout(keep_in, keep_out, seed ^ 0x5bd1e995)
            ops.lstm_fwd_pair(ws, self.p("kernel_0"), self.p("bias_0"), wb, self.p("bw_kernel_0"), self.p("bw_bias_0"),
                              self.layout.kernel_stride, self.layout.bias_stride, lengths,
                              self.state_h if use_state else None, self.state_c if use_state else None)
        else:
            ops.lstm_fwd(ws, self.p("kernel_0"), self.layout.kernel_stride, self.p("bias_0"),
                         self.layout.bias_stride, lengths,
                         self.state_h if use_state else None, self.state_c if use_state else None, training=training,
                         per_diagonal=per_diagonal, head=self._head)
        H = self.H
        if not self.bidirectional:
            if after_lstm is not None:
                after_lstm()
            if self._head is None:
                ops.linear_fwd(ws.ztop.view(Tr * B, H), self.p("output_w"), self.p("output_b"),
                               out=self.logits[:Tr].view(Tr * B, self.C))
        else:
            if not paired:
                wb.set_dropout(keep_in, keep_out, seed ^ 0x5bd1e995)
                ops.lstm_fwd(wb, self.p("bw_kernel_0"), self.layout.kernel_stride, self.p("bw_bias_0"),
                             self.layout.bias_stride, lengths, None, None, training=training, per_diagonal=per_diagonal)
            if after_lstm is not None:
                after_lstm()
            ops.reverse_sequences(wb.ztop, lengths, out=self.ytop_b[:Tr])
            wo = self.p("output_w")
            ops.linear_fwd(ws.ztop.view(Tr * B, H), wo[:H], self.p("output_b"), out=self.logits[:Tr].view(Tr * B, self.C))
            ops.gemm(self.ytop_b[:Tr].view(Tr * B, H), wo[H:], out=self.logits[:Tr].view(Tr * B, self.C), accumulate=True)
        if Tr < T:
            self.logits[Tr:] = self.p("output_b")
        return self.logits

    def _cells(self, flat):
        L = self.L
        ks = [self.layout.view(flat, "kernel_%d" % l) for l in range(L)] + [self.layout.view(flat, "bw_kernel_%d" % l) for l in range(L)]
        bs = [self.layout.view(flat, "bias_%d" % l) for l in range(L)] + [self.layout.view(flat, "bw_bias_%d" % l) for l in range(L)]
        return ks, bs

    def _forward_layerwise(self, ws, lengths, keep_in, keep_out, seed, use_state, after_lstm, per_diagonal, Tr):
        B, H = self.B, self.H
        ws.set_dropout(keep_in, keep_out, seed)
        ks, bs = self._cells(self.params)
        self._layer_path = 0 if per_diagonal else ws.path()
        ops.lstm_bidir_fwd(ws, ks, bs, lengths, self.state_h if use_state else None, self.state_c if use_state else None,
                           per_frame=per_diagonal)
        if after_lstm is not None:
            after_lstm()
        wo = self.p("output_w")
        ops.linear_fwd(ws.ytop_fw.view(Tr * B, H), wo[:H], self.p("output_b"), out=self.logits[:Tr].view(Tr * B, self.C))
        ops.gemm(ws.ytop_bw.view(Tr * B, H), wo[H:], out=self.logits[:Tr].view(Tr * B, self.C), accumulate=True)
        if Tr < self.T:
            self.logits[Tr:] = self.p("output_b")
        return self.logits

    def kernel_path(self):
        path = {"fused_ctc_head": self._head is not None, "paired": self._paired, "run_length": self._Tr}
        if not self.layerwise:
            plan = ops.lstm_plan(self._ws, head=self._head, per_diagonal=self._per_diagonal)
            path["lstm_fwd"], path["lstm_bwd"] = ("big1" if self._paired else plan["fwd_path"]), plan["bwd_path"]
        if self.layerwise:
            path["layer_recurrence"] = {2: "persistent", 1: "persistent_per_direction", 0: "per_frame"}.get(self._layer_path)
            path["layer_product"] = self.precision
        return path

    def final_state(self):
        return self._ws.final_state()

    def keep_state(self):
        h, c = self._ws.final_state()
        self.state_h.copy_(h)
        self.state_c.copy_(c)

    def zero_state(self):
        self.state_h.zero_()
        self.state_c.zero_()

    def ctc(self, dense_labels, lengths, stage=0):
        Tr = self._Tr
        if self._head is not None:
            if Tr < self.T and stage != 1:
                self.dlogits[Tr:].zero_()
            return self.loss
        ops.ctc_loss_fwd_bwd(self.logits[:Tr], dense_labels, lengths, ws=self.ctc_ws, loss=self.loss,
                             dlogits=self.dlogits[:Tr], stage=stage)
        if Tr < self.T and stage != 1:
            self.dlogits[Tr:].zero_()
        return self.loss

    def align(self, x, lengths, dense_labels):
        self.forward(x, lengths)
        shape = (self.T, self.B, self.C, dense_labels.shape[1])
        if getattr(self, "_align_ws", None) is None or self._align_ws.shape != shape:
            self._align_ws = ops.CtcAlignWorkspace(*shape, device=self.device)
        return ops.ctc_align(self.logits, dense_labels.contiguous(), lengths, ws=self._align_ws)

    @contextlib.contextmanager
    def on_stream(self):
        cur = torch.cuda.current_stream(self.device)
        if cur.cuda_stream != 0:
            yield
            return
        self.stream.wait_stream(cur)
        with torch.cuda.stream(self.stream):
            yield
        cur.wait_stream(self.stream)

    def backward(self, x, lengths, wait_for=None, per_diagonal=False):
        T, B, D = x.shape
        x = x.contiguous()
        ws, Tr = self._ws, self._Tr
        H = self.H
        dl = self.dlogits[:Tr].view(Tr * B, self.C)
        if self.layerwise:
            self._backward_layerwise(x, lengths, wait_for, per_diagonal)
            return
        head = self._head if not per_diagonal else None
        if self._head is not None and head is None:
            raise _lib.AmdSpeechError("backward(per_diagonal=True) after a forward with the fused CTC head: repeat the forward too")
        if head is not None:
            pass
        elif not self.bidirectional:
            ops.linear_bwd(ws.ztop.view(Tr * B, H), self.p("output_w"), dl,
                           self.g("output_w"), self.g("output_b"), need_dx=True, dx=ws.dztop.view(Tr * B, H))
        else:
            wo, gwo, wb = self.p("output_w"), self.g("output_w"), self._ws_b
            ops.linear_bwd(ws.ztop.view(Tr * B, H), wo[:H], dl, gwo[:H], self.g("output_b"), need_dx=True,
                           dx=ws.dztop.view(Tr * B, H))
            yb = self.ytop_b[:Tr].view(Tr * B, H)
            ops.gemm(yb, dl, trans_a=True, out=gwo[H:], accumulate=True)
            ops.gemm(dl, wo[H:], trans_b=True, out=self.dytop_b[:Tr].view(Tr * B, H))
            ops.reverse_sequences(self.dytop_b[:Tr], lengths, out=wb.dztop)
        if wait_for is not None:
            torch.cuda.current_stream(self.device).wait_event(wait_for)
        paired = self.bidirectional and _BIDIR_PAIR and not per_diagonal and ops.lstm_pair_fusable(ws)
        if paired:
            wb = self._ws_b
            ops.lstm_bwd_pair(ws, self.p("kernel_0"), self.g("kernel_0"), self.g("bias_0"),
                              wb, self.p("bw_kernel_0"), self.g("bw_kernel_0"), self.g("bw_bias_0"),
                              self.layout.kernel_stride, self.layout.bias_stride, lengths)
# ... 161 lines not shown
```

### rnn-speech_amd/lib.py

```python
import ctypes as C
import os

HERE = os.path.dirname(os.path.abspath(__file__))
LIB_PATH = os.environ.get("AMDSPEECH_LIB") or os.path.join(HERE, "libamdspeech.so")


class AmdSpeechError(RuntimeError):
    pass


class DataflowTimeout(AmdSpeechError):
    """amdspeech_lstm_status returned AMDSPEECH_ETIMEOUT: a whole-sequence launch gave up waiting.  The mini-batch's results are
    invalid; it can be repeated on the launch-per-diagonal kernels.  Any OTHER error of that call is a device fault."""


ETIMEOUT = -4


class LstmDesc(C.Structure):
    _fields_ = [("T", C.c_int), ("B", C.c_int), ("H", C.c_int), ("L", C.c_int),
                ("keep_in", C.c_float), ("keep_out", C.c_float), ("seed", C.c_uint64),
                ("precision", C.c_int), ("flags", C.c_int)]


class CtcHead(C.Structure):
    _fields_ = [("w_out", C.c_void_p), ("b_out", C.c_void_p), ("logits", C.c_void_p), ("dense_labels", C.c_void_p),
                ("loss", C.c_void_p), ("dlogits", C.c_void_p), ("ctc_ws", C.c_void_p), ("C", C.c_int), ("U", C.c_int)]


class LstmPlanInfo(C.Structure):
    _fields_ = [(n, C.c_int) for n in ("fwd_path", "bwd_path", "nmt", "kb", "mv", "wpx", "uw", "fwd_mt", "pair", "bf16p", "bf16p_reserved",
                                       "xw_parts", "nfw", "w_pieces", "dz0_inkernel", "flow2_q")]


class CtcPlanInfo(C.Structure):
    _fields_ = [(n, C.c_int) for n in ("kernel", "threads", "rmax", "smax")]


class GemmPlanInfo(C.Structure):
    _fields_ = [(n, C.c_int) for n in ("family", "variant", "splits", "k_chunk", "atomic", "zero_fill", "grid", "tiles_m", "tiles_n", "map",
                                       "bm", "bn", "col_slices", "a_vec", "b_vec")]


class FrontendPlanInfo(C.Structure):
    _fields_ = [(n, C.c_int) for n in ("frames_kernel", "maxq", "n_dft", "frame_len", "hop", "n_bins", "bin_tiles", "kp", "lds_bytes", "t_full",
                                       "tiles_per_utt", "n_items", "workgroups", "dct_kernel", "dct_col_tiles", "meta_by_copy")]


class FrameStackPlanInfo(C.Structure):
    _fields_ = [(n, C.c_int) for n in ("t_out", "d_out", "vec", "workgroups", "meta_by_copy")]


class SpecAugmentDesc(C.Structure):
    _fields_ = [(n, C.c_int) for n in ("period", "freq_masks", "freq_width", "time_masks", "time_width", "time_permille")] + \
               [("seed", C.c_uint64)]


class SpecAugmentPlanInfo(C.Structure):
    _fields_ = [(n, C.c_int) for n in ("vec", "lanes", "items_per_workgroup", "workgroups", "reps")]


class FeatureNormDesc(C.Structure):
    _fields_ = [("mode", C.c_int), ("norm_vars", C.c_int), ("var_floor", C.c_double)]


class FeatureNormPlanInfo(C.Structure):
    _fields_ = [(n, C.c_int) for n in ("vec", "split", "workgroups", "lds_bytes", "meta_by_copy", "workspace_bytes")]


GEMM_FAMILIES = ("skinny_n", "skinny_k", "skinny_tn", "tn_direct", "kc_direct", "lds", "bf3", "bf16p")
GEMM_MAP_LINEAR, GEMM_MAP_XCD, GEMM_MAP_XCD_BLOCKS, GEMM_MAP_KC_BAND = range(4)
GEMM_GROUP_MAX = 10
CTC_KERNELS = ("wave", "shift", "pair", "edge")
LSTM_PATHS = ("flow", "big1", "big", "hoist", "diag", "diag_bf3")
FEATURE_NORM_MODES = ("none", "utterance", "global")
LSTM_ARMED, LSTM_ARM_NEXT, LSTM_SAME_WS, LSTM_PER_DIAGONAL, LSTM_INJECT_TIMEOUT = 1, 2, 4, 8, 16


COMM_ID_BYTES = 128
WS_Z0, WS_ZTOP, WS_DZTOP, WS_DZ0, WS_HFINAL, WS_CFINAL, WS_GATES = range(7)
BIDIR_WS_Z0, BIDIR_WS_YTOP_FW, BIDIR_WS_YTOP_BW, BIDIR_WS_DYTOP_FW, BIDIR_WS_DYTOP_BW, BIDIR_WS_DZ0, BIDIR_WS_HFINAL, BIDIR_WS_CFINAL = range(8)

_P = C.c_void_p
_I = C.c_int
_F = C.c_float
_L = C.c_long
_SZ = C.c_size_t

PROTOTYPES = {
    "amdspeech_version": (_I, []),
    "amdspeech_last_error": (C.c_char_p, []),
    "amdspeech_device_cu_count": (_I, []),
    "amdspeech_linear_fwd": (_I, [_P, _P, _P, _P, _P, _I, _I, _I]),
    "amdspeech_linear_bwd": (_I, [_P, _P, _P, _P, _P, _P, _P, _I, _I, _I]),
    "amdspeech_gemm_f32": (_I, [_P, _I, _I, _I, _I, _I, _P, _I, _P, _I, _P, _I, _P, _I]),
    "amdspeech_gemm_bf16x3": (_I, [_P, _I, _I, _I, _I, _I, _P, _I, _P, _I, _P, _I, _P, _I]),
    "amdspeech_gemm_bf16": (_I, [_P, _I, _I, _I, _I, _I, _P, _I, _P, _I, _P, _I, _P, _I]),
    "amdspeech_gemm_plan": (_I, [_I, _I, _I, _I, _I, _I, _P, _I, _P, _I, _P, _I, _P, _I, _I, _I, C.POINTER(GemmPlanInfo)]),
    "amdspeech_gemm_f32_tn_group": (_I, [_P, _I, _I, _I, _I, _P, _I, _P, _I, _P, _I, _P, _I]),
    "amdspeech_colsum_accumulate": (_I, [_P, _P, _I, _I, _I, _P]),
    "amdspeech_gemm_bf16_packed_scratch_bytes": (_SZ, [_I, _I, _I, _I, _I, _I, _I]),
    "amdspeech_gemm_bf16_packed": (_I, [_P, _I, _I, _I, _I, _I, _P, _I, _P, _I, _P, _I, _P, _I, _P, _SZ]),
    "amdspeech_gemm_bf16_packed_plan": (_I, [_I, _I, _I, _I, _I, _I, _I, C.POINTER(GemmPlanInfo)]),
    "amdspeech_bf16_copy": (_I, [_P, _P, C.c_long, C.c_long, _I, _I, _P, C.c_long, _P, _P]),
    "amdspeech_bf16_transpose": (_I, [_P, _P, C.c_long, _I, _P, C.c_long]),
    "amdspeech_batchnorm_fwd": (_I, [_P, _P, _P, _P, _P, _I, _I, _I, _F]),
    "amdspeech_batchnorm_bwd": (_I, [_P, _P, _P, _P, _P, _I, _I, _I]),
    "amdspeech_batchnorm_sum": (_I, [_P, _P, _P, _I, _P, _I, _I, _I]),
    "amdspeech_batchnorm_apply": (_I, [_P, _P, _P, _P, _I, _F, _P, _P, _P, _I, _I, _I]),
    "amdspeech_batchnorm_bwd_sums": (_I, [_P, _P, _P, _P, _I, _I, _I]),
    "amdspeech_batchnorm_bwd_apply": (_I, [_P, _P, _P, _P, _P, _I, _P, _I, _I, _I]),
    "amdspeech_lstm_workspace_bytes": (_SZ, [C.POINTER(LstmDesc)]),
    "amdspeech_lstm_ws_ptr": (_P, [C.POINTER(LstmDesc), _P, _I]),
    "amdspeech_lstm_fwd": (_I, [_P, C.POINTER(LstmDesc), _P, _P, _L, _P, _L, _P, _P, _P]),
    "amdspeech_lstm_status": (_I, [C.POINTER(LstmDesc), _P]),
    "amdspeech_lstm_workspace_release": (_I, [_P, _P]),
    "amdspeech_lstm_beside_forward": (_I, [_P, _P]),
    "amdspeech_lstm_beside_tail": (_I, [_P, _P]),
    "amdspeech_lstm_bwd": (_I, [_P, C.POINTER(LstmDesc), _P, _P, _L, _P, _P, _L, _P]),
    "amdspeech_lstm_ctc_fusable": (_I, [C.POINTER(LstmDesc), _I, _I]),
    "amdspeech_lstm_pair_fusable": (_I, [C.POINTER(LstmDesc)]),
    "amdspeech_lstm_fwd_pair": (_I, [_P, C.POINTER(LstmDesc), _P, _P, _P, C.POINTER(LstmDesc), _P, _P, _P, _L, _L, _P, _P, _P]),
    "amdspeech_lstm_bwd_pair": (_I, [_P, C.POINTER(LstmDesc), _P, _P, _P, _P, C.POINTER(LstmDesc), _P, _P, _P, _P, _L, _L, _P]),
    "amdspeech_lstm_fwd_ctc": (_I, [_P, C.POINTER(LstmDesc), _P, _P, _L, _P, _L, _P, _P, _P, C.POINTER(CtcHead)]),
    "amdspeech_lstm_bwd_ctc": (_I, [_P, C.POINTER(LstmDesc), _P, _P, _L, _P, _P, _L, _P, C.POINTER(CtcHead)]),
    "amdspeech_lstm_dropout_multipliers": (_I, [_P, C.POINTER(LstmDesc), _I, _I, _P]),
    "amdspeech_lstm_plan": (_I, [C.POINTER(LstmDesc), _I, _I, C.POINTER(LstmPlanInfo)]),
    "amdspeech_lstm_plan_xw_halves": (_I, [C.POINTER(LstmDesc), _I, _I]),
    "amdspeech_lstm_bidir_workspace_bytes": (_SZ, [C.POINTER(LstmDesc)]),
    "amdspeech_lstm_bidir_ws_ptr": (_P, [C.POINTER(LstmDesc), _P, _I]),
    "amdspeech_lstm_bidir_layer_stride": (_L, [C.POINTER(LstmDesc)]),
    "amdspeech_lstm_bidir_path": (_I, [C.POINTER(LstmDesc)]),
    "amdspeech_lstm_bidir_fwd": (_I, [_P, C.POINTER(LstmDesc), _P, _P, _P, _P, _P, _P]),
    "amdspeech_lstm_bidir_bwd": (_I, [_P, C.POINTER(LstmDesc), _P, _P, _P, _P, _P]),
    "amdspeech_lstm_bidir_status": (_I, [C.POINTER(LstmDesc), _P]),
    "amdspeech_lstm_bidir_dropout_multipliers": (_I, [_P, C.POINTER(LstmDesc), _I, _I, _I, _P]),
    "amdspeech_ctc_workspace_bytes": (_SZ, [_I, _I, _I, _I]),
    "amdspeech_ctc_plan": (_I, [_I, _I, _I, _I, C.POINTER(CtcPlanInfo)]),
    "amdspeech_ctc_loss_fwd_bwd": (_I, [_P, _P, _P, _P, _I, _I, _I, _I, _P, _P, _P]),
    "amdspeech_ctc_loss_fwd_bwd_staged": (_I, [_P, _P, _P, _P, _I, _I, _I, _I, _P, _P, _P, _I]),
    "amdspeech_ctc_align_workspace_bytes": (_SZ, [_I, _I, _I, _I]),
    "amdspeech_ctc_align_plan": (_I, [_I, _I, _I, _I, C.POINTER(CtcPlanInfo)]),
    "amdspeech_ctc_align": (_I, [_P, _P, _P, _P, _I, _I, _I, _I, _P, _P, _P, _P, _P, _P]),
    "amdspeech_ctc_greedy_decode": (_I, [_P, _P, _P, _I, _I, _I, _P, _P, _P]),
    "amdspeech_merge_repeated": (_I, [_P, _P, _P, _I, _I, _I]),
    "amdspeech_edit_distance": (_I, [_P, _P, _P, _I, _P, _P, _I, _I, _P]),
    "amdspeech_ctc_beam_search_host": (_I, [_P, _P, _I, _I, _I, _I, _I, _P, _P, _P]),
    "amdspeech_ctc_beam_search_host_mt": (_I, [_P, _P, _I, _I, _I, _I, _I, _P, _P, _P, _I]),
    "amdspeech_edit_distance_host": (_I, [_P, _P, _I, _P, _P, _I, _I, _P]),
    "amdspeech_crc32c": (C.c_uint32, [_P, _SZ, C.c_uint32]),
    "amdspeech_resample_workspace_bytes": (_SZ, [C.c_int]),
    "amdspeech_resample_num_samples": (C.c_int, [C.c_int, C.c_int, C.c_int]),
    "amdspeech_resample": (C.c_int, [_P, _P, C.POINTER(C.c_int), C.c_int, C.c_int, C.c_int, C.c_int, _P, C.c_int, _P]),
    "amdspeech_audio_probe": (C.c_int, [C.c_char_p, C.POINTER(C.c_int), C.POINTER(C.c_int), C.POINTER(C.c_long)]),
    "amdspeech_audio_decode": (C.c_int, [C.c_char_p, _P, C.c_long, C.POINTER(C.c_long), C.POINTER(C.c_int), C.c_int]),
    "amdspeech_optim_workspace_bytes": (_SZ, [_L]),
    "amdspeech_clip_adam": (_I, [_P, _P, _P, _P, _P, _L, _F, _F, _F, _F, _F, _P, _P]),
    "amdspeech_frontend_workspace_bytes": (_SZ, [_I, _I, _I, _I]),
    "amdspeech_frontend_num_frames": (_I, [_I, _I, _I]),
    "amdspeech_frontend_plan": (_I, [_I, _I, _I, _I, _I, _I, C.POINTER(FrontendPlanInfo)]),
    "amdspeech_frontend_mfcc": (_I, [_P, _P, _P, _I, _I, _I, _I, _I, _P, _P, _P]),
    "amdspeech_frontend_fbank": (_I, [_P, _P, _P, _I, _I, _I, _I, _P, _P, _P]),
    "amdspeech_frame_stack_num_frames": (_I, [_I, _I]),
    "amdspeech_frame_stack": (_I, [_P, _P, _P, _I, _I, _I, _I, _I, _P, _P]),
    "amdspeech_frame_stack_plan": (_I, [_I, _I, _I, _I, _I, C.POINTER(FrameStackPlanInfo)]),
    "amdspeech_spec_augment": (_I, [_P, _P, _P, _I, _I, _I, C.POINTER(SpecAugmentDesc)]),
    "amdspeech_spec_augment_spans": (_I, [C.POINTER(SpecAugmentDesc), _I, _I, C.POINTER(C.c_int)]),
    "amdspeech_spec_augment_plan": (_I, [_I, _I, _I, C.POINTER(SpecAugmentDesc), C.POINTER(SpecAugmentPlanInfo)]),
    "amdspeech_feature_norm_plan": (_I, [_I, _I, _I, _I, C.POINTER(FeatureNormPlanInfo)]),
    "amdspeech_feature_moments": (_I, [_P, _P, _P, _I, _I, _I, _P, _P]),
    "amdspeech_feature_norm": (_I, [_P, _P, _P, _I, _I, _I, C.POINTER(FeatureNormDesc), _P, _P]),
    "amdspeech_profile_enable": (_I, [_I]),
    "amdspeech_profile_get": (_I, [_I, C.POINTER(C.c_float), C.POINTER(C.c_int)]),
    "amdspeech_profile_get_flops": (_I, [_I, C.POINTER(C.c_double), C.POINTER(C.c_double)]),
    "amdspeech_comm_available": (_I, []),
    "amdspeech_comm_unique_id": (_I, [_P]),
    "amdspeech_comm_init": (_I, [_P, _I, _I, C.POINTER(_P)]),
    "amdspeech_comm_destroy": (_I, [_P]),
    "amdspeech_comm_info": (_I, [_P, C.POINTER(_I), C.POINTER(_I), C.POINTER(_I), C.c_char_p, _I]),
    "amdspeech_allreduce_sum_f32": (_I, [_P, _P, _P, _L]),
    "amdspeech_broadcast_f32": (_I, [_P, _P, _P, _L, _I]),
    "amdspeech_reverse_sequences": (_I, [_P, _P, _P, _P, _I, _I, _I, _I]),
    "amdspeech_axpy": (_I, [_P, _F, _P, _P, _L]),
    "amdspeech_fill": (_I, [_P, _P, _F, _L]),
}

_lib = None


def load():
    global _lib
    if _lib is not None:
        return _lib
    if not os.path.exists(LIB_PATH):
        raise AmdSpeechError(
            "libamdspeech.so not found at %s -- build it with "
            "`python -c 'import __graft_entry__ as g; g.build()'` (hipcc, gfx950)" % LIB_PATH)
    lib = C.CDLL(LIB_PATH)
    for name, (res, args) in PROTOTYPES.items():
        fn = getattr(lib, name)
        fn.restype = res
        fn.argtypes = args
    _lib = lib
    return lib


def check(rc, what=""):
# ... 4 lines not shown
```

### rnn-speech_amd/ops.py

```python
import ctypes as C
import os

import torch

from . import lib as _l

MODE_MFCC, MODE_FBANK = 0, 1


def _stream():
    return C.c_void_p(torch.cuda.current_stream().cuda_stream)


def _p(t):
    return C.c_void_p(t.data_ptr()) if t is not None else C.c_void_p(0)


def _chk_f32(*ts):
    for t in ts:
        if t is None:
            continue
        if not (t.is_cuda and t.dtype == torch.float32 and t.is_contiguous()):
            raise ValueError("expected a contiguous float32 device tensor, got %s %s" % (t.dtype, t.device))

# ... 228 lines not shown
        self.T, self.B, self.H, self.L = T, B, H, L
        if _share is None:
            self.buf = torch.empty(nbytes // 4, device=device, dtype=torch.float32)
        else:
            if _share.numel() * 4 < nbytes:
                raise _l.AmdSpeechError("lstm workspace: the layout for T = %d needs %d bytes, the shared allocation has %d"
                                        % (T, nbytes, _share.numel() * 4))
            self.buf = _share
        if self.buf.data_ptr() % 256 != 0:
            raise _l.AmdSpeechError("lstm workspace: allocation not 256-byte aligned")
        self.z0 = self._view(_l.WS_Z0, (T, B, H))
        self.ztop = self._view(_l.WS_ZTOP, (T, B, H))
        self.dztop = self._view(_l.WS_DZTOP, (T, B, H))
        self.dz0 = self._view(_l.WS_DZ0, (T, B, H))
        self._prefixes = {}
        self._root = self
        self._armed = None
        self._ever_armed = False
        self._fwd_seen = False
        self._lib_state = False

    def __del__(self):
        try:
            if self._root is self and (self._ever_armed or self._fwd_seen or self._lib_state) and torch.cuda.is_available():
                self.lib.amdspeech_lstm_workspace_release(_stream(), _p(self.buf))
        except Exception:
            pass

    def prefix(self, T_run):
        if T_run >= self.T:
            return self
        ws = self._prefixes.get(T_run)
        if ws is None:
            if len(self._prefixes) > 64:
                self._prefixes.clear()
            ws = LstmWorkspace(T_run, self.B, self.H, self.L, device=self.buf.device,
                               precision=self.desc.precision, _share=self.buf)
            ws._root = self
            self._prefixes[T_run] = ws
        return ws

    def _offset(self, which):
        p = self.lib.amdspeech_lstm_ws_ptr(C.byref(self.desc), _p(self.buf), which)
        if not p:
            raise _l.AmdSpeechError("lstm_ws_ptr failed")
        return (p - self.buf.data_ptr()) // 4

    def _view(self, which, shape):
        off = self._offset(which)
        n = 1
        for s in shape:
            n *= s
        return self.buf[off:off + n].view(*shape)

    def set_dropout(self, keep_in, keep_out, seed):
        self.desc.keep_in, self.desc.keep_out, self.desc.seed = keep_in, keep_out, seed

    def final_state(self):
        T, B, H, L = self.T, self.B, self.H, self.L
        stride = (T + 1) * B * H
        oh, oc = self._offset(_l.WS_HFINAL), self._offset(_l.WS_CFINAL)
        h = torch.as_strided(self.buf, (L, B, H), (stride, H, 1), oh)
        c = torch.as_strided(self.buf, (L, B, H), (stride, H, 1), oc)
        return h, c


_ARM = os.environ.get("AMDSPEECH_ARM", "1") != "0"


class CtcHead(object):

    def __init__(self, w_out, b_out, logits, dense_labels, loss, dlogits, ctc_ws):
        _chk_f32(w_out, b_out, logits, loss, dlogits)
        _chk_i32(dense_labels)
        T, B, C_ = logits.shape
        if ctc_ws.shape[0] < T or tuple(ctc_ws.shape[1:]) != (B, C_, dense_labels.shape[1]):
            raise ValueError("CtcHead: the CTC workspace was sized for %r, the logits are %r with U = %d"
                             % (ctc_ws.shape, (T, B, C_), dense_labels.shape[1]))
        self.keep = (w_out, b_out, logits, dense_labels, loss, dlogits, ctc_ws)
        self.c = _l.CtcHead(_p(w_out).value, _p(b_out).value, _p(logits).value, _p(dense_labels).value, _p(loss).value,
                            _p(dlogits).value if dlogits is not None else None, _p(ctc_ws.buf).value, C_, dense_labels.shape[1])


def lstm_ctc_fusable(ws, C_, U, per_diagonal=False):
    if per_diagonal:
        return False
    return bool(ws.lib.amdspeech_lstm_ctc_fusable(C.byref(ws.desc), int(C_), int(U)))


def lstm_plan(ws, head=None, per_diagonal=False):
    c_u = (0, 0) if head is None else ((head.c.C, head.c.U) if isinstance(head, CtcHead) else (int(head[0]), int(head[1])))
    d = _l.LstmDesc(ws.desc.T, ws.desc.B, ws.desc.H, ws.desc.L, ws.desc.keep_in, ws.desc.keep_out, ws.desc.seed, ws.desc.precision,
                    _l.LSTM_PER_DIAGONAL if per_diagonal else 0)
    info = _l.LstmPlanInfo()
    _l.check(ws.lib.amdspeech_lstm_plan(C.byref(d), c_u[0], c_u[1], C.byref(info)), "lstm_plan")
    out = {name: int(getattr(info, name)) for name, _ in _l.LstmPlanInfo._fields_}
    out["fwd_path"], out["bwd_path"] = _l.LSTM_PATHS[out["fwd_path"]], _l.LSTM_PATHS[out["bwd_path"]]
    return out


def lstm_plan_xw_halves(ws, head=None, per_diagonal=False):
    c_u = (0, 0) if head is None else ((head.c.C, head.c.U) if isinstance(head, CtcHead) else (int(head[0]), int(head[1])))
    d = _l.LstmDesc(ws.desc.T, ws.desc.B, ws.desc.H, ws.desc.L, ws.desc.keep_in, ws.desc.keep_out, ws.desc.seed, ws.desc.precision,
                    _l.LSTM_PER_DIAGONAL if per_diagonal else 0)
    n = int(ws.lib.amdspeech_lstm_plan_xw_halves(C.byref(d), c_u[0], c_u[1]))
    if n < 0:
        raise ValueError("lstm_plan_xw_halves: bad descriptor")
    return n


def lstm_fwd(ws, kernels, kernel_stride, biases, bias_stride, lengths, h0=None, c0=None, training=False, per_diagonal=False, head=None):
    _chk_i32(lengths)
    _chk_f32(h0, c0)
    root, key = ws._root, (ws.T, int(ws.desc.precision))
    if per_diagonal:
        root._armed, training = None, False
    armed = _ARM and root._armed is not None and root._armed["fwd"] == key
    root._armed = None
    inject, root._inject_timeout = getattr(root, "_inject_timeout", 0), 0
    ws.desc.flags = ((_l.LSTM_ARMED if armed else 0) | (_l.LSTM_ARM_NEXT if (training and _ARM) else 0) |
                     (_l.LSTM_SAME_WS if (root._fwd_seen and _ARM) else 0) | (_l.LSTM_PER_DIAGONAL if per_diagonal else 0) |
                     (_l.LSTM_INJECT_TIMEOUT if inject else 0))
    root._fwd_seen = False
    try:
        if head is None:
            _l.check(ws.lib.amdspeech_lstm_fwd(_stream(), C.byref(ws.desc), _p(ws.buf), _p(kernels), kernel_stride,
                                               _p(biases), bias_stride, _p(lengths), _p(h0), _p(c0)), "lstm_fwd")
        else:
            _l.check(ws.lib.amdspeech_lstm_fwd_ctc(_stream(), C.byref(ws.desc), _p(ws.buf), _p(kernels), kernel_stride,
                                                   _p(biases), bias_stride, _p(lengths), _p(h0), _p(c0), C.byref(head.c)), "lstm_fwd_ctc")
        root._fwd_seen = not per_diagonal
        root._lib_state = True
    finally:
        ws.desc.flags = 0
    if training and _ARM:
        root._armed = {"fwd": key, "bwd": key}
        root._ever_armed = True


def lstm_pair_fusable(ws):
    ws.desc.flags = 0
    return bool(ws.lib.amdspeech_lstm_pair_fusable(C.byref(ws.desc)))


def lstm_fwd_pair(ws_a, kernels_a, biases_a, ws_b, kernels_b, biases_b, kernel_stride, bias_stride, lengths, h0=None, c0=None):
    _chk_i32(lengths)
    _chk_f32(h0, c0)
    for ws in (ws_a, ws_b):
        ws._root._armed, ws._root._fwd_seen, ws._root._lib_state = None, False, True
        ws.desc.flags = 0
    _l.check(ws_a.lib.amdspeech_lstm_fwd_pair(_stream(), C.byref(ws_a.desc), _p(ws_a.buf), _p(kernels_a), _p(biases_a),
                                              C.byref(ws_b.desc), _p(ws_b.buf), _p(kernels_b), _p(biases_b),
                                              kernel_stride, bias_stride, _p(lengths), _p(h0), _p(c0)), "lstm_fwd_pair")


def lstm_status(ws):
    try:
        _l.check(ws.lib.amdspeech_lstm_status(C.byref(ws.desc), _p(ws.buf)), "lstm_status")
    except _l.AmdSpeechError:
        ws._root._armed = None
        ws._root._fwd_seen = False
        raise


def lstm_beside_forward(ws, stream):
    rc = _l.load().amdspeech_lstm_beside_forward(C.c_void_p(stream.cuda_stream), _p(ws._root.buf))
    if rc < 0:
        _l.check(rc, "lstm_beside_forward")
    return rc


def lstm_beside_tail(ws, stream):
    rc = _l.load().amdspeech_lstm_beside_tail(C.c_void_p(stream.cuda_stream), _p(ws._root.buf))
    if rc < 0:
        _l.check(rc, "lstm_beside_tail")
    return rc


def lstm_bwd(ws, kernels, kernel_stride, dkernels, dbiases, bias_stride, lengths, per_diagonal=False, head=None):
    _chk_i32(lengths)
    root, key = ws._root, (ws.T, int(ws.desc.precision))
    armed = root._armed is not None and root._armed["bwd"] == key and not per_diagonal
    if root._armed is not None:
        root._armed["bwd"] = None
    root._lib_state = True
    inject, root._inject_timeout_bwd = getattr(root, "_inject_timeout_bwd", 0), 0
    ws.desc.flags = ((_l.LSTM_ARMED if armed else 0) | (_l.LSTM_PER_DIAGONAL if per_diagonal else 0) |
                     (_l.LSTM_INJECT_TIMEOUT if inject else 0))
    try:
        if head is None:
            _l.check(ws.lib.amdspeech_lstm_bwd(_stream(), C.byref(ws.desc), _p(ws.buf), _p(kernels), kernel_stride,
                                               _p(dkernels), _p(dbiases), bias_stride, _p(lengths)), "lstm_bwd")
        else:
            _l.check(ws.lib.amdspeech_lstm_bwd_ctc(_stream(), C.byref(ws.desc), _p(ws.buf), _p(kernels), kernel_stride,
                                                   _p(dkernels), _p(dbiases), bias_stride, _p(lengths), C.byref(head.c)), "lstm_bwd_ctc")
    finally:
        ws.desc.flags = 0


def lstm_bwd_pair(ws_a, kernels_a, dkernels_a, dbiases_a, ws_b, kernels_b, dkernels_b, dbiases_b, kernel_stride, bias_stride, lengths):
    _chk_i32(lengths)
    for ws in (ws_a, ws_b):
        if ws._root._armed is not None:
            ws._root._armed["bwd"] = None
        ws._root._lib_state = True
        ws.desc.flags = 0
    _l.check(ws_a.lib.amdspeech_lstm_bwd_pair(_stream(), C.byref(ws_a.desc), _p(ws_a.buf), _p(kernels_a), _p(dkernels_a), _p(dbiases_a),
                                              C.byref(ws_b.desc), _p(ws_b.buf), _p(kernels_b), _p(dkernels_b), _p(dbiases_b),
# ... 480 lines not shown
```

Baseline: 2.741 million.

## Fuse input projection GEMM and CTC label preparation into the LSTM forward launch

Adds an input head so the LSTM forward entry point computes the input linear projection (x·W_in + b) itself, instead of the engine issuing a separate linear_fwd beforehand. The skinny-K GEMM body moves into a shared header with a pluggable store policy so the LSTM kernel can reuse it. CTC label preparation is likewise split into a device function so it can run inside other kernels. The aim is to remove separate kernel launches and a round trip of z0 through global memory, at the cost of more complex fused kernels and a fallback path when fusion is not possible.

Result: no change. 2.753 million, median of 5 (+0.4%).

```diff
diff --git a/include/amdspeech.h b/include/amdspeech.h
--- a/include/amdspeech.h
+++ b/include/amdspeech.h
@@ -136,6 +136,21 @@
                            const float* kernels, long kernel_stride, float* dkernels, float* dbiases, long bias_stride,
                            const int* lengths, const amdspeech_ctc_head* head);
 
+typedef struct amdspeech_input_head {
+    const float* x;
+    const float* w_in;
+    const float* b_in;
+    int D;
+} amdspeech_input_head;
+int amdspeech_lstm_fwd_in(void* stream, const amdspeech_lstm_desc* d, void* ws,
+                          const float* kernels, long kernel_stride, const float* biases, long bias_stride,
+                          const int* lengths, const float* h0, const float* c0, const amdspeech_input_head* in);
+int amdspeech_lstm_fwd_ctc_in(void* stream, const amdspeech_lstm_desc* d, void* ws,
+                              const float* kernels, long kernel_stride, const float* biases, long bias_stride,
+                              const int* lengths, const float* h0, const float* c0, const amdspeech_ctc_head* head,
+                              const amdspeech_input_head* in);
+int amdspeech_lstm_plan_input_fused(const amdspeech_lstm_desc* d, int D);
+
 int amdspeech_lstm_dropout_multipliers(void* stream, const amdspeech_lstm_desc* d, int which, int layer, float* out);
 
 enum { AMDSPEECH_LSTM_PATH_FLOW = 0, AMDSPEECH_LSTM_PATH_BIG1 = 1, AMDSPEECH_LSTM_PATH_BIG = 2, AMDSPEECH_LSTM_PATH_HOIST = 3,
diff --git a/rnn-speech_amd/csrc/ctc.hip b/rnn-speech_amd/csrc/ctc.hip
--- a/rnn-speech_amd/csrc/ctc.hip
+++ b/rnn-speech_amd/csrc/ctc.hip
@@ -6,36 +6,7 @@
 __global__ __launch_bounds__(64) void ctc_prepare_kernel(const int* __restrict__ dense, const int* __restrict__ lengths,
                                                          int T, int U, int C, int smax, int* __restrict__ ext,
                                                          int* __restrict__ slen, int* __restrict__ valid) {
-    const int b = blockIdx.x, lane = threadIdx.x;
-    const int blank = C - 1;
-    int* e = ext + (size_t)b * smax;
-    for (int s = lane; s < smax; s += 64) e[s] = blank;
-    __syncthreads();
-    int kept = 0, ntgt = 0;
-    bool finished = false;
-    const unsigned long long lt = (1ull << lane) - 1ull;
-    for (int u0 = 0; u0 < U; u0 += 64) {
-        const int u = u0 + lane;
-        const int v = (u < U) ? dense[(size_t)b * U + u] : 0;
-        const bool nz = v != 0;
-        const unsigned long long mnz = __ballot(nz);
-        const unsigned long long mterm = __ballot(nz && v >= blank);
-        kept += __popcll(mnz);
-        if (!finished) {
-            unsigned long long before = ~0ull;
-            if (mterm) { before = (1ull << (__ffsll((long long)mterm) - 1)) - 1ull; }
-            const unsigned long long mt = mnz & before;
-            if (nz && ((mt >> lane) & 1ull)) e[2 * (ntgt + __popcll(mt & lt)) + 1] = v;
-            ntgt += __popcll(mt);
-            if (mterm) finished = true;
-        }
-    }
-    if (lane == 0) {
-        if (kept == 0) kept = 1;
-        const int len = min(lengths[b], T);
-        slen[b] = 2 * ntgt + 1;
-        valid[b] = (len > 0 && kept <= len) ? 1 : 0;
-    }
+    ctc_prepare_row(dense, lengths, T, U, C, smax, ext, slen, valid, blockIdx.x, threadIdx.x, true);
 }
 
 __global__ __launch_bounds__(256) void log_softmax_kernel(const float* __restrict__ x, float* __restrict__ y,
diff --git a/rnn-speech_amd/csrc/ctc_core.h b/rnn-speech_amd/csrc/ctc_core.h
--- a/rnn-speech_amd/csrc/ctc_core.h
+++ b/rnn-speech_amd/csrc/ctc_core.h
@@ -50,6 +50,42 @@
 constexpr int CF_FOLLOW_TEAM_FLOATS = 4 * 16 * CF_RP + 16 * CF_RP + 2 * 4 * 16 * 4 + 256 * 2;
 constexpr int CF_AP = 388;
 constexpr int CF_LEAD_TEAM_FLOATS = 3 * 16 * CF_RP + 2 * 4 * 16 * 4 + 16 * CF_AP;
+
+__device__ __forceinline__ void ctc_prepare_row(const int* __restrict__ dense, const int* __restrict__ lengths, int T, int U, int C,
+                                                int smax, int* __restrict__ ext, int* __restrict__ slen, int* __restrict__ valid,
+                                                int b, int lane, bool active) {
+    const int blank = C - 1;
+    int* e = ext + (size_t)b * smax;
+    if (active)
+        for (int s = lane; s < smax; s += 64) e[s] = blank;
+    __syncthreads();
+    if (!active) return;
+    int kept = 0, ntgt = 0;
+    bool finished = false;
+    const unsigned long long lt = (1ull << lane) - 1ull;
+    for (int u0 = 0; u0 < U; u0 += 64) {
+        const int u = u0 + lane;
+        const int v = (u < U) ? dense[(size_t)b * U + u] : 0;
+        const bool nz = v != 0;
+        const unsigned long long mnz = __ballot(nz);
+        const unsigned long long mterm = __ballot(nz && v >= blank);
+        kept += __popcll(mnz);
+        if (!finished) {
+            unsigned long long before = ~0ull;
+            if (mterm) { before = (1ull << (__ffsll((long long)mterm) - 1)) - 1ull; }
+            const unsigned long long mt = mnz & before;
+            if (nz && ((mt >> lane) & 1ull)) e[2 * (ntgt + __popcll(mt & lt)) + 1] = v;
+            ntgt += __popcll(mt);
+            if (mterm) finished = true;
+        }
+    }
+    if (lane == 0) {
+        if (kept == 0) kept = 1;
+        const int len = min(lengths[b], T);
+        slen[b] = 2 * ntgt + 1;
+        valid[b] = (len > 0 && kept <= len) ? 1 : 0;
+    }
+}
 
 #ifndef CTC_DIAG
 #define CTC_DIAG 0
diff --git a/rnn-speech_amd/csrc/gemm_skinny.hip b/rnn-speech_amd/csrc/gemm_skinny.hip
--- a/rnn-speech_amd/csrc/gemm_skinny.hip
+++ b/rnn-speech_amd/csrc/gemm_skinny.hip
@@ -1,48 +1,8 @@
 #include "common.h"
+#include "gemm_skinny_k.h"
 #include <string.h>
 
 namespace amdspeech {
-
-typedef __amdgpu_buffer_rsrc_t sk_rsrc_t;
-typedef unsigned sk_u32x4 __attribute__((ext_vector_type(4)));
-
-struct SkinnyArgs {
-    const float* A; const float* B; float* C; const float* bias;
-    int M, N, K, lda, ldb, ldc, accumulate;
-};
-
-constexpr unsigned SK_OOB = 0x80000000u;
-
-__device__ __forceinline__ f32x4 sk_load4(sk_rsrc_t rs, unsigned byte_off) {
-    const sk_u32x4 w = __builtin_amdgcn_raw_buffer_load_b128(rs, byte_off, 0, 0);
-    f32x4 r;
-    r.x = __uint_as_float(w.x); r.y = __uint_as_float(w.y); r.z = __uint_as_float(w.z); r.w = __uint_as_float(w.w);
-    return r;
-}
-__device__ __forceinline__ float sk_load1(sk_rsrc_t rs, unsigned byte_off) {
-    return __uint_as_float(__builtin_amdgcn_raw_buffer_load_b32(rs, byte_off, 0, 0));
-}
-
-struct SkinnyOut {
-    sk_rsrc_t c, c_in, bias;
-    __device__ __forceinline__ void init(const SkinnyArgs& g) {
-        const unsigned cbytes = (unsigned)(((size_t)(g.M - 1) * g.ldc + g.N) * 4);
-        c = __builtin_amdgcn_make_buffer_rsrc(g.C, 0, cbytes, 0x00020000);
-        c_in = __builtin_amdgcn_make_buffer_rsrc(g.C, 0, g.accumulate ? cbytes : 0u, 0x00020000);
-        bias = __builtin_amdgcn_make_buffer_rsrc(const_cast<float*>(g.bias), 0, g.bias != nullptr ? (unsigned)g.N * 4u : 0u, 0x00020000);
-    }
-    __device__ __forceinline__ unsigned offset(const SkinnyArgs& g, int row, int n) const {
-        return (row < g.M && n < g.N) ? (unsigned)((size_t)row * g.ldc + n) * 4u : SK_OOB;
-    }
-    __device__ __forceinline__ f32x4 addend(const SkinnyArgs& g, unsigned off, int n) const {
-        return sk_load4(bias, n < g.N ? (unsigned)n * 4u : SK_OOB) + sk_load4(c_in, off);
-    }
-    __device__ __forceinline__ void store(unsigned off, f32x4 v) const {
-        sk_u32x4 w;
-        w.x = __float_as_uint(v.x); w.y = __float_as_uint(v.y); w.z = __float_as_uint(v.z); w.w = __float_as_uint(v.w);
-        __builtin_amdgcn_raw_buffer_store_b128(w, c, off, 0, 0);
-    }
-};
 
 template <int NT>
 __global__ __launch_bounds__(256) void gemm_skinny_n_kernel(SkinnyArgs g) {
@@ -133,85 +93,8 @@
 
 template <int KT, bool B_KC>
 __global__ __launch_bounds__(256) void gemm_skinny_k_kernel(SkinnyArgs g) {
-    const int tid = threadIdx.x, w = tid >> 6, lane = tid & 63, m = lane & 15, kg = lane >> 4;
-    const int row0 = blockIdx.x * 128 + w * 32;
-    const sk_rsrc_t ra = __builtin_amdgcn_make_buffer_rsrc(const_cast<float*>(g.A), 0, (unsigned)(((size_t)(g.M - 1) * g.lda + g.K) * 4), 0x00020000);
-    const size_t b_extent = B_KC ? (size_t)(g.N - 1) * g.ldb + g.K : (size_t)(g.K - 1) * g.ldb + g.N;
-    const sk_rsrc_t rb = __builtin_amdgcn_make_buffer_rsrc(const_cast<float*>(g.B), 0, (unsigned)(b_extent * 4), 0x00020000);
-    SkinnyOut out;
-    out.init(g);
-
-    f32x4 a[2][KT];
-#pragma unroll
-    for (int mt = 0; mt < 2; ++mt)
-#pragma unroll
-        for (int kt = 0; kt < KT; ++kt) {
-            const int row = row0 + mt * 16 + m, kk = 16 * kt + 4 * kg;
-            const bool ok = row < g.M && kk < g.K;
-            a[mt][kt] = sk_load4(ra, ok ? (unsigned)((size_t)row * g.lda + kk) * 4u : SK_OOB);
-        }
-    struct Tile { f32x4 b[2][KT], bias[2], old[2][2]; unsigned off[2][2]; };
-    auto fetch = [&](int nt, Tile& t) __attribute__((always_inline)) {
-#pragma unroll
-        for (int q = 0; q < 2; ++q) {
-            const int n = (nt + q) * 16 + m;
-#pragma unroll
-            for (int kt = 0; kt < KT; ++kt) {
-                const int kk = 16 * kt + 4 * kg;
-                const bool ok = n < g.N && kk < g.K;
-                if (B_KC) {
-                    t.b[q][kt] = sk_load4(rb, ok ? (unsigned)(n * g.ldb + kk) * 4u : SK_OOB);
-                } else {
-                    const unsigned o = ok ? (unsigned)(kk * g.ldb + n) * 4u : SK_OOB;
-                    const unsigned st = ok ? (unsigned)g.ldb * 4u : 0u;
-                    t.b[q][kt].x = sk_load1(rb, o);
-                    t.b[q][kt].y = sk_load1(rb, o + st);
-                    t.b[q][kt].z = sk_load1(rb, o + 2 * st);
-                    t.b[q][kt].w = sk_load1(rb, o + 3 * st);
-                }
-            }
-            const int nc = (nt + q) * 16 + 4 * kg;
-            t.bias[q] = sk_load4(out.bias, nc < g.N ? (unsigned)nc * 4u : SK_OOB);
-#pragma unroll
-            for (int mt = 0; mt < 2; ++mt) {
-                t.off[mt][q] = out.offset(g, row0 + mt * 16 + m, nc);
-                t.old[mt][q] = sk_load4(out.c_in, t.off[mt][q]);
-            }
-        }
-    };
-    auto tile = [&](int nt, const Tile& cur, Tile& nxt) __attribute__((always_inline)) {
-        fetch(nt + 2, nxt);
-        __builtin_amdgcn_sched_barrier(0);
-        f32x4 acc[2][2];
-#pragma unroll
-        for (int mt = 0; mt < 2; ++mt)
-#pragma unroll
-            for (int q = 0; q < 2; ++q) acc[mt][q] = cur.bias[q] + cur.old[mt][q];
-#pragma unroll
-        for (int kt = 0; kt < KT; ++kt)
-#pragma unroll
-            for (int j = 0; j < 4; ++j)
-#pragma unroll
-                for (int mt = 0; mt < 2; ++mt)
-#pragma unroll
-                    for (int q = 0; q < 2; ++q)
-                        acc[mt][q] = __builtin_amdgcn_mfma_f32_16x16x4f32(cur.b[q][kt][j], a[mt][kt][j], acc[mt][q], 0, 0, 0);
-#pragma unroll
-        for (int mt = 0; mt < 2; ++mt)
-#pragma unroll
-            for (int q = 0; q < 2; ++q) out.store(cur.off[mt][q], acc[mt][q]);
-        __builtin_amdgcn_sched_barrier(0);
-    };
-    const int all_tiles = (g.N + 15) / 16;
-    const int per = ((all_tiles + (int)gridDim.y - 1) / (int)gridDim.y + 1) & ~1;
-    const int nt0 = (int)blockIdx.y * per, ntiles = min(all_tiles, nt0 + per);
-    Tile t0, t1;
-    fetch(nt0, t0);
-    for (int nt = nt0; nt < ntiles; nt += 4) {
-        tile(nt, t0, t1);
-        if (nt + 2 >= ntiles) break;
-        tile(nt + 2, t1, t0);
-    }
+    SkinnyStorePlain st;
+    gemm_skinny_k_body<KT, B_KC>(g, (int)blockIdx.x, (int)blockIdx.y, (int)gridDim.y, st);
 }
 
 #ifndef SKTN_DIAG
diff --git a/rnn-speech_amd/csrc/gemm_skinny_k.h b/rnn-speech_amd/csrc/gemm_skinny_k.h
--- /dev/null
+++ b/rnn-speech_amd/csrc/gemm_skinny_k.h
@@ -0,0 +1,139 @@
+#pragma once
+#include "common.h"
+
+namespace amdspeech {
+
+typedef __amdgpu_buffer_rsrc_t sk_rsrc_t;
+typedef unsigned sk_u32x4 __attribute__((ext_vector_type(4)));
+
+struct SkinnyArgs {
+    const float* A; const float* B; float* C; const float* bias;
+    int M, N, K, lda, ldb, ldc, accumulate;
+};
+
+constexpr unsigned SK_OOB = 0x80000000u;
+
+__device__ __forceinline__ f32x4 sk_load4(sk_rsrc_t rs, unsigned byte_off) {
+    const sk_u32x4 w = __builtin_amdgcn_raw_buffer_load_b128(rs, byte_off, 0, 0);
+    f32x4 r;
+    r.x = __uint_as_float(w.x); r.y = __uint_as_float(w.y); r.z = __uint_as_float(w.z); r.w = __uint_as_float(w.w);
+    return r;
+}
+__device__ __forceinline__ float sk_load1(sk_rsrc_t rs, unsigned byte_off) {
+    return __uint_as_float(__builtin_amdgcn_raw_buffer_load_b32(rs, byte_off, 0, 0));
+}
+__device__ __forceinline__ void sk_store4(sk_rsrc_t rs, unsigned byte_off, f32x4 v) {
+    sk_u32x4 w;
+    w.x = __float_as_uint(v.x); w.y = __float_as_uint(v.y); w.z = __float_as_uint(v.z); w.w = __float_as_uint(v.w);
+    __builtin_amdgcn_raw_buffer_store_b128(w, rs, byte_off, 0, 0);
+}
+
+struct SkinnyOut {
+    sk_rsrc_t c, c_in, bias;
+    __device__ __forceinline__ void init(const SkinnyArgs& g) {
+        const unsigned cbytes = (unsigned)(((size_t)(g.M - 1) * g.ldc + g.N) * 4);
+        c = __builtin_amdgcn_make_buffer_rsrc(g.C, 0, cbytes, 0x00020000);
+        c_in = __builtin_amdgcn_make_buffer_rsrc(g.C, 0, g.accumulate ? cbytes : 0u, 0x00020000);
+        bias = __builtin_amdgcn_make_buffer_rsrc(const_cast<float*>(g.bias), 0, g.bias != nullptr ? (unsigned)g.N * 4u : 0u, 0x00020000);
+    }
+    __device__ __forceinline__ unsigned offset(const SkinnyArgs& g, int row, int n) const {
+        return (row < g.M && n < g.N) ? (unsigned)((size_t)row * g.ldc + n) * 4u : SK_OOB;
+    }
+    __device__ __forceinline__ f32x4 addend(const SkinnyArgs& g, unsigned off, int n) const {
+        return sk_load4(bias, n < g.N ? (unsigned)n * 4u : SK_OOB) + sk_load4(c_in, off);
+    }
+    __device__ __forceinline__ void store(unsigned off, f32x4 v) const { sk_store4(c, off, v); }
+};
+
+struct SkinnyStorePlain {
+    static constexpr bool kOld = true;
+    __device__ __forceinline__ void prepare(const SkinnyArgs&, int, int) {}
+    __device__ __forceinline__ void operator()(const SkinnyOut& out, unsigned off, int, int, int, f32x4 v) const { out.store(off, v); }
+};
+
+template <int KT, bool B_KC, class Store>
+__device__ __forceinline__ void gemm_skinny_k_body(const SkinnyArgs& g, int bx, int by, int ny, Store& st) {
+    const int tid = threadIdx.x, w = tid >> 6, lane = tid & 63, m = lane & 15, kg = lane >> 4;
+    const int row0 = bx * 128 + w * 32;
+    const sk_rsrc_t ra = __builtin_amdgcn_make_buffer_rsrc(const_cast<float*>(g.A), 0, (unsigned)(((size_t)(g.M - 1) * g.lda + g.K) * 4), 0x00020000);
+    const size_t b_extent = B_KC ? (size_t)(g.N - 1) * g.ldb + g.K : (size_t)(g.K - 1) * g.ldb + g.N;
+    const sk_rsrc_t rb = __builtin_amdgcn_make_buffer_rsrc(const_cast<float*>(g.B), 0, (unsigned)(b_extent * 4), 0x00020000);
+    SkinnyOut out;
+    out.init(g);
+
+    f32x4 a[2][KT];
+#pragma unroll
+    for (int mt = 0; mt < 2; ++mt) {
+        st.prepare(g, mt, row0 + mt * 16 + m);
+#pragma unroll
+        for (int kt = 0; kt < KT; ++kt) {
+            const int row = row0 + mt * 16 + m, kk = 16 * kt + 4 * kg;
+            const bool ok = row < g.M && kk < g.K;
+            a[mt][kt] = sk_load4(ra, ok ? (unsigned)((size_t)row * g.lda + kk) * 4u : SK_OOB);
+        }
+    }
+    struct Tile { f32x4 b[2][KT], bias[2], old[2][2]; unsigned off[2][2]; };
+    auto fetch = [&](int nt, Tile& t) __attribute__((always_inline)) {
+#pragma unroll
+        for (int q = 0; q < 2; ++q) {
+            const int n = (nt + q) * 16 + m;
+#pragma unroll
+            for (int kt = 0; kt < KT; ++kt) {
+                const int kk = 16 * kt + 4 * kg;
+                const bool ok = n < g.N && kk < g.K;
+                if (B_KC) {
+                    t.b[q][kt] = sk_load4(rb, ok ? (unsigned)(n * g.ldb + kk) * 4u : SK_OOB);
+                } else {
+                    const unsigned o = ok ? (unsigned)(kk * g.ldb + n) * 4u : SK_OOB;
+                    const unsigned sd = ok ? (unsigned)g.ldb * 4u : 0u;
+                    t.b[q][kt].x = sk_load1(rb, o);
+                    t.b[q][kt].y = sk_load1(rb, o + sd);
+                    t.b[q][kt].z = sk_load1(rb, o + 2 * sd);
+                    t.b[q][kt].w = sk_load1(rb, o + 3 * sd);
+                }
+            }
+            const int nc = (nt + q) * 16 + 4 * kg;
+            t.bias[q] = sk_load4(out.bias, nc < g.N ? (unsigned)nc * 4u : SK_OOB);
+#pragma unroll
+            for (int mt = 0; mt < 2; ++mt) {
+                t.off[mt][q] = out.offset(g, row0 + mt * 16 + m, nc);
+                if (Store::kOld) t.old[mt][q] = sk_load4(out.c_in, t.off[mt][q]);
+            }
+        }
+    };
+    auto tile = [&](int nt, const Tile& cur, Tile& nxt) __attribute__((always_inline)) {
+        fetch(nt + 2, nxt);
+        __builtin_amdgcn_sched_barrier(0);
+        f32x4 acc[2][2];
+#pragma unroll
+        for (int mt = 0; mt < 2; ++mt)
+#pragma unroll
+            for (int q = 0; q < 2; ++q) acc[mt][q] = cur.bias[q] + (Store::kOld ? cur.old[mt][q] : f32x4{0.f, 0.f, 0.f, 0.f});
+#pragma unroll
+        for (int kt = 0; kt < KT; ++kt)
+#pragma unroll
+            for (int j = 0; j < 4; ++j)
+#pragma unroll
+                for (int mt = 0; mt < 2; ++mt)
+#pragma unroll
+                    for (int q = 0; q < 2; ++q)
+                        acc[mt][q] = __builtin_amdgcn_mfma_f32_16x16x4f32(cur.b[q][kt][j], a[mt][kt][j], acc[mt][q], 0, 0, 0);
+#pragma unroll
+        for (int mt = 0; mt < 2; ++mt)
+#pragma unroll
+            for (int q = 0; q < 2; ++q) st(out, cur.off[mt][q], mt, row0 + mt * 16 + m, (nt + q) * 16 + 4 * kg, acc[mt][q]);
+        __builtin_amdgcn_sched_barrier(0);
+    };
+    const int all_tiles = (g.N + 15) / 16;
+    const int per = ((all_tiles + ny - 1) / ny + 1) & ~1;
+    const int nt0 = by * per, ntiles = min(all_tiles, nt0 + per);
+    Tile t0, t1;
+    fetch(nt0, t0);
+    for (int nt = nt0; nt < ntiles; nt += 4) {
+        tile(nt, t0, t1);
+        if (nt + 2 >= ntiles) break;
+        tile(nt + 2, t1, t0);
+    }
+}
+
+}
diff --git a/rnn-speech_amd/csrc/lstm.hip b/rnn-speech_amd/csrc/lstm.hip
--- a/rnn-speech_amd/csrc/lstm.hip
+++ b/rnn-speech_amd/csrc/lstm.hip
@@ -1,6 +1,7 @@
 #include "common.h"
 #include "gemm_core.h"
 #include "ctc_core.h"
+#include "gemm_skinny_k.h"
 #include <stdlib.h>
 #include <string.h>
 #include <type_traits>
@@ -141,11 +142,10 @@
     if (i < n) x[i] *= zmult(c, lp, (uint32_t)i);
 }
 
-__global__ void pack_fwd_kernel(const float* __restrict__ kernels, long kstride, float* __restrict__ wp,
-                                int H, int L, int UW, int grouped) {
+__device__ __forceinline__ void pack_fwd_item(long o, const float* __restrict__ kernels, long kstride, float* __restrict__ wp,
+                                              int H, int L, int UW, int grouped) {
     const int NT = UW / 4, NKB = 2 * H / 16, NUB = H / UW;
     const long total = (long)L * 2 * H * 4 * H;
-    long o = (long)blockIdx.x * blockDim.x + threadIdx.x;
     if (o >= total) return;
     int m = o & 3, lane = (o >> 2) & 63;
     long r = o >> 8;
@@ -157,6 +157,10 @@
     if (grouped) { g = j >> 2; u = nt * 4 + (j & 3); }
     int k = kb * 16 + 4 * kq + m;
     wp[o] = kernels[l * kstride + (long)k * 4 * H + g * H + ub * UW + u];
+}
+__global__ void pack_fwd_kernel(const float* __restrict__ kernels, long kstride, float* __restrict__ wp,
+                                int H, int L, int UW, int grouped) {
+    pack_fwd_item((long)blockIdx.x * blockDim.x + threadIdx.x, kernels, kstride, wp, H, L, UW, grouped);
 }
 
 __global__ void pack_bwd_kernel(const float* __restrict__ kernels, long kstride, float* __restrict__ wq,
@@ -208,14 +212,15 @@
     *reinterpret_cast<float4*>(dst + (size_t)t * bpk + packed_off(row, k, K)) = v;
 }
 
-__global__ __launch_bounds__(256) void flow_fwd_prepare_kernel(const float* __restrict__ h0, const float* __restrict__ c0,
-                                                               float* __restrict__ hs, float* __restrict__ cs,
-                                                               float* __restrict__ hph, unsigned* __restrict__ sync_words,
-                                                               int T, int B, int H, int L) {
+constexpr int FLOW_BWD_AHEAD = 40;
+__device__ __forceinline__ void flow_fwd_prepare_item(size_t i, const float* __restrict__ h0, const float* __restrict__ c0,
+                                                      float* __restrict__ hs, float* __restrict__ cs,
+                                                      float* __restrict__ hph, unsigned* __restrict__ sync_words,
+                                                      int T, int B, int H, int L, int bwd_ahead) {
     const int bp = (B + 15) / 16 * 16;
     const size_t per = (size_t)bp * H;
-    const size_t i = (size_t)blockIdx.x * blockDim.x + threadIdx.x;
     if (i < 40) sync_words[i] = 0u;
+    else if (bwd_ahead && i < 64) sync_words[i] = i < FLOW_BWD_AHEAD + 8 ? (unsigned)T : 0u;
     if (i >= per * L) return;
     const int l = i / per;
     const size_t r = i % per;
@@ -228,6 +233,90 @@
         cs[(size_t)l * (T + 1) * bh + e] = c0 ? c0[l * bh + e] : 0.f;
     }
     hph[(size_t)l * (T + 1) * per + packed_off(row, k, H)] = hv;
+}
+__global__ __launch_bounds__(256) void flow_fwd_prepare_kernel(const float* __restrict__ h0, const float* __restrict__ c0,
+                                                               float* __restrict__ hs, float* __restrict__ cs,
+                                                               float* __restrict__ hph, unsigned* __restrict__ sync_words,
+                                                               int T, int B, int H, int L) {
+    flow_fwd_prepare_item((size_t)blockIdx.x * blockDim.x + threadIdx.x, h0, c0, hs, cs, hph, sync_words, T, B, H, L, 0);
+}
+
+struct FwdHeadArgs {
+    SkinnyArgs g; int gemm_bx, gemm_ny;
+    float* xp0; int T, B, H, L; DropCfg drop; int masked;
+    const float* kernels; long kstride; float* wp; int uw;
+    const float* h0; const float* c0; float* hs; float* cs; float* hph; unsigned* sync_words; int bwd_ahead;
+    const int* dense; const int* lengths; int U, C, smax; int* ext; int* slen; int* valid;
+    const float* wo; float* wopack;
+    int nb_gemm, nb_pack, nb_prep, nb_ctc, nb_wo;
+};
+struct HeadStore {
+    static constexpr bool kOld = false;
+    sk_rsrc_t xp; unsigned base[2]; int B, H; size_t bpk; DropCfg drop; int masked;
+    __device__ __forceinline__ void prepare(const SkinnyArgs& g, int mt, int row) {
+        const int t = row / B, b = row - t * B;
+        base[mt] = row < g.M ? (unsigned)(((size_t)t * bpk + (size_t)(b >> 4) * (H >> 4) * 256 + (b & 15) * 4) * 4) : SK_OOB;
+    }
+    __device__ __forceinline__ void operator()(const SkinnyOut& out, unsigned off, int mt, int row, int n, f32x4 v) const {
+        if (masked) {
+            const uint32_t e = (uint32_t)row * (uint32_t)H + (uint32_t)n;
+            v.x *= zmult(drop, 0, e); v.y *= zmult(drop, 0, e + 1); v.z *= zmult(drop, 0, e + 2); v.w *= zmult(drop, 0, e + 3);
+        }
+        out.store(off, v);
+        const unsigned col = (unsigned)(((n >> 4) * 256 + ((n >> 2) & 3) * 64) * 4);
+        sk_store4(xp, (off != SK_OOB && base[mt] != SK_OOB) ? base[mt] + col : SK_OOB, v);
+    }
+};
+template <int KT, int ROLES>
+__global__ __launch_bounds__(256) void lstm_fwd_head_kernel(FwdHeadArgs a) {
+    int blk = blockIdx.x;
+    if (ROLES & 1) {
+        if (blk < a.nb_gemm) {
+            HeadStore st;
+            st.B = a.B; st.H = a.H; st.bpk = (size_t)((a.B + 15) / 16 * 16) * a.H; st.drop = a.drop; st.masked = a.masked;
+            st.xp = __builtin_amdgcn_make_buffer_rsrc(a.xp0, 0, (unsigned)((size_t)a.T * st.bpk * 4), 0x00020000);
+            gemm_skinny_k_body<KT, false>(a.g, blk % a.gemm_bx, blk / a.gemm_bx, a.gemm_ny, st);
+            return;
+        }
+        blk -= a.nb_gemm;
+    }
+    if (!(ROLES & 2)) return;
+    if (blk < a.nb_pack) {
+        const long o4 = ((long)blk * 256 + threadIdx.x) * 4;
+        if (o4 >= (long)a.L * 2 * a.H * 4 * a.H) return;
+        const int NT = a.uw / 4, NKB = 2 * a.H / 16, NUB = a.H / a.uw;
+        const int lane = (o4 >> 2) & 63;
+        long r = o4 >> 8;
+        const int nt = r % NT; r /= NT;
+        const int kb = r % NKB; r /= NKB;
+        const int ub = r % NUB, l = r / NUB;
+        const int j = lane & 15, kq = lane >> 4, c = nt * 16 + j, g = c / a.uw, u = c % a.uw;
+        const float* src = a.kernels + l * a.kstride + (long)(kb * 16 + 4 * kq) * 4 * a.H + g * a.H + ub * a.uw + u;
+        const size_t row = (size_t)4 * a.H;
+        *reinterpret_cast<float4*>(a.wp + o4) = make_float4(src[0], src[row], src[2 * row], src[3 * row]);
+        return;
+    }
+    blk -= a.nb_pack;
+    if (blk < a.nb_prep) {
+        flow_fwd_prepare_item((size_t)blk * 256 + threadIdx.x, a.h0, a.c0, a.hs, a.cs, a.hph, a.sync_words, a.T, a.B, a.H, a.L, a.bwd_ahead);
+        return;
+    }
+    blk -= a.nb_prep;
+    if (blk < a.nb_ctc) {
+        const int b = blk * 4 + (threadIdx.x >> 6);
+        ctc_prepare_row(a.dense, a.lengths, a.T, a.U, a.C, a.smax, a.ext, a.slen, a.valid, b < a.B ? b : 0, threadIdx.x & 63, b < a.B);
+        return;
+    }
+    blk -= a.nb_ctc;
+    if (blk < a.nb_wo) {
+        const int i = blk * 256 + threadIdx.x;
+        if (i >= (a.H / 16) * CF_NTC * 64) return;
+        const int lane = i & 63, j = (i >> 6) % CF_NTC, kb = (i >> 6) / CF_NTC;
+        const int n = j * 16 + (lane & 15), k = kb * 16 + 4 * (lane >> 4);
+        float4 v = make_float4(0.f, 0.f, 0.f, 0.f);
+        if (n < a.C) { v.x = a.wo[(size_t)k * a.C + n]; v.y = a.wo[(size_t)(k + 1) * a.C + n]; v.z = a.wo[(size_t)(k + 2) * a.C + n]; v.w = a.wo[(size_t)(k + 3) * a.C + n]; }
+        reinterpret_cast<float4*>(a.wopack)[i] = v;
+    }
 }
 
 __device__ __forceinline__ float sigmoidf_(float x) { return 1.0f / (1.0f + expf(-x)); }
@@ -371,6 +460,7 @@
     int xw_par = -1;
     int xw_cover = 0;
     long xw_key = 0;
+    bool bwd_ahead = false;
 };
 static std::mutex g_arm_mutex;
 static std::unordered_map<const void*, ArmState> g_arm;
@@ -395,6 +485,17 @@
     std::lock_guard<std::mutex> lock(g_arm_mutex);
     auto it = g_arm.find(ws);
     if (it != g_arm.end()) it->second.xw_par = -1;
+}
+static void flow_set_bwd_ahead(const void* ws, bool on) {
+    std::lock_guard<std::mutex> lock(g_arm_mutex);
+    g_arm[ws].bwd_ahead = on;
+}
+static bool flow_take_bwd_ahead(const void* ws) {
+    std::lock_guard<std::mutex> lock(g_arm_mutex);
+    auto it = g_arm.find(ws);
+    if (it == g_arm.end() || !it->second.bwd_ahead) return false;
+    it->second.bwd_ahead = false;
+    return true;
 }
 static int flow_arm_fork(hipStream_t s) {
     if (int rc = side_stream_init()) return rc;
@@ -642,7 +743,9 @@
 struct FwdCall {
     const amdspeech_lstm_desc* d; float* ws; const float* kernels; long kstride; const float* biases; long bstride;
     const int* lengths; const float* h0; const float* c0; const amdspeech_ctc_head* head;
+    const amdspeech_input_head* in;
     LstmPlan p; LstmLayout lo;
+    bool one_launch;
 };
 struct BwdCall {
     const amdspeech_lstm_desc* d; float* ws; const float* kernels; long kstride; float* dkernels; float* dbiases; long bstride;
@@ -670,6 +773,9 @@
     c.lo = lstm_layout(c.p);
     AS_CHECK_ARG(c.head == nullptr || c.p.fwd == Path::flow, "lstm_fwd_ctc: the fused CTC head needs the whole-sequence kernels (amdspeech_lstm_ctc_fusable)");
     prof_flops(0, 0.0, 0.0);
+    flow_set_bwd_ahead(c.ws, false);
+    c.one_launch = c.in != nullptr && c.p.fwd == Path::flow;
+    if (c.one_launch) return AMDSPEECH_OK;
     AS_CHECK_HIP(hipMemsetAsync(c.ws + c.lo.sync, 0, 64, s));
     const long wtotal = (long)d->L * 2 * d->H * 4 * d->H;
     if (c.p.fwd == Path::diag_bf3)
@@ -719,6 +825,68 @@
     return AMDSPEECH_OK;
 }
 
+static bool input_gemm_fusable(const LstmPlan& p, int D, const float* x, const float* w, const float* z, const float* b, GemmPlan* gp) {
+    const amdspeech_lstm_desc& d = p.d;
+    if (p.fwd != Path::flow || D <= 0 || (size_t)d.T * d.B > (size_t)0x7fffffff) return false;
+    if (!gemm_skinny_plan(false, d.T * d.B, d.H, D, x, D, w, d.H, z, d.H, b, gp)) return false;
+    return gp->family == AMDSPEECH_GEMM_SKINNY_K;
+}
+#ifndef FWD_HEAD_NY
+#define FWD_HEAD_NY 4
+#endif
+#ifndef FWD_HEAD_LAUNCHES
+#define FWD_HEAD_LAUNCHES 1
+#endif
+static int fwd_head_launch(hipStream_t s, const FwdCall& c, float* panels) {
+    const amdspeech_lstm_desc* d = c.d;
+    const LstmLayout& lo = c.lo;
+    float* ws = c.ws;
+    const int T = d->T, B = d->B, H = d->H, L = d->L;
+    const size_t bph = (size_t)(B + 15) / 16 * 16 * H;
+    FwdHeadArgs a{};
+    GemmPlan gp;
+    const bool fused = input_gemm_fusable(c.p, c.in->D, c.in->x, c.in->w_in, ws + lo.z, c.in->b_in, &gp);
+    if (fused) {
+        a.g = SkinnyArgs{c.in->x, c.in->w_in, ws + lo.z, c.in->b_in, T * B, H, c.in->D, c.in->D, H, H, 0};
+        a.gemm_bx = gp.tiles_m; a.gemm_ny = (H / 16) % (2 * FWD_HEAD_NY) == 0 ? FWD_HEAD_NY : gp.col_slices; a.nb_gemm = gp.tiles_m * a.gemm_ny;
+    }
+    a.xp0 = ws + lo.xp0; a.T = T; a.B = B; a.H = H; a.L = L; a.drop = drop_cfg(d); a.masked = d->keep_in < 1.0f ? 1 : 0;
+    a.kernels = c.kernels; a.kstride = c.kstride; a.wp = ws + lo.wp; a.uw = c.p.uw;
+    a.nb_pack = ceil_div((long)L * 2 * H * 4 * H / 4, 256);
+    a.h0 = c.h0; a.c0 = c.c0; a.hs = ws + lo.hs; a.cs = ws + lo.cs; a.hph = panels + lo.hph;
+    a.sync_words = reinterpret_cast<unsigned*>(ws + lo.sync);
+    a.bwd_ahead = (d->flags & AMDSPEECH_LSTM_ARM_NEXT) ? 1 : 0;
+    a.nb_prep = ceil_div((long)L * bph, 256);
+    if (c.head != nullptr) {
+        const CtcLayout cl = ctc_layout(T, B, c.head->C, c.head->U);
+        char* w = static_cast<char*>(c.head->ctc_ws);
+        a.dense = c.head->dense_labels; a.lengths = c.lengths; a.U = c.head->U; a.C = c.head->C; a.smax = cl.smax;
+        a.ext = reinterpret_cast<int*>(w + cl.ext); a.slen = reinterpret_cast<int*>(w + cl.slen); a.valid = reinterpret_cast<int*>(w + cl.valid);
+        a.nb_ctc = ceil_div(B, 4);
+        a.wo = c.head->w_out; a.wopack = ws + lo.wopack;
+        a.nb_wo = ceil_div((H / 16) * CF_NTC * 64, 256);
+    }
+    const int rest = a.nb_pack + a.nb_prep + a.nb_ctc + a.nb_wo;
+    if (!fused) {
+        hipLaunchKernelGGL((lstm_fwd_head_kernel<3, 2>), dim3(rest), dim3(256), 0, s, a);
+        AS_CHECK_LAUNCH();
+        if (int rc = gemm_f32(s, false, false, T * B, H, c.in->D, c.in->x, c.in->D, c.in->w_in, H, ws + lo.z, H, c.in->b_in, false)) return rc;
+        hipLaunchKernelGGL(mask_pack_rows_kernel, dim3(ceil_div((long)T * B * H / 4, 256)), dim3(256), 0, s, ws + lo.z, ws + lo.xp0, B, H, T,
+                           a.drop, a.masked);
+        return AMDSPEECH_OK;
+    }
+    const bool kt3 = gp.variant / 2 == 3;
+#if FWD_HEAD_LAUNCHES == 2
+    if (kt3) hipLaunchKernelGGL((lstm_fwd_head_kernel<3, 1>), dim3(a.nb_gemm), dim3(256), 0, s, a);
+    else hipLaunchKernelGGL((lstm_fwd_head_kernel<5, 1>), dim3(a.nb_gemm), dim3(256), 0, s, a);
+    hipLaunchKernelGGL((lstm_fwd_head_kernel<3, 2>), dim3(rest), dim3(256), 0, s, a);
+#else
+    if (kt3) hipLaunchKernelGGL((lstm_fwd_head_kernel<3, 3>), dim3(a.nb_gemm + rest), dim3(256), 0, s, a);
+    else hipLaunchKernelGGL((lstm_fwd_head_kernel<5, 3>), dim3(a.nb_gemm + rest), dim3(256), 0, s, a);
+#endif
+    return AMDSPEECH_OK;
+}
+
 static int fwd_flow(hipStream_t s, const FwdCall& c) {
     const amdspeech_lstm_desc* d = c.d;
     const LstmPlan& p = c.p;
@@ -732,10 +900,14 @@
     if (!(d->flags & AMDSPEECH_LSTM_ARMED))
         if (int rc = flow_fill_fwd_panels(s, d, ws, lo, set)) return rc;
     float* const panels = ws + (size_t)set * lo.fwd_set;
-    hipLaunchKernelGGL(flow_fwd_prepare_kernel, dim3(ceil_div((long)L * bph, 256)), dim3(256), 0, s, c.h0, c.c0, ws + lo.hs, ws + lo.cs,
-                       panels + lo.hph, err, T, B, H, L);
-    hipLaunchKernelGGL(mask_pack_rows_kernel, dim3(ceil_div((long)T * bh / 4, 256)), dim3(256), 0, s, ws + lo.z, ws + lo.xp0, B, H, T,
-                       dc, d->keep_in < 1.0f ? 1 : 0);
+    if (c.one_launch) {
+        if (int rc = fwd_head_launch(s, c, panels)) return rc;
+    } else {
+        hipLaunchKernelGGL(flow_fwd_prepare_kernel, dim3(ceil_div((long)L * bph, 256)), dim3(256), 0, s, c.h0, c.c0, ws + lo.hs, ws + lo.cs,
+                           panels + lo.hph, err, T, B, H, L);
+        hipLaunchKernelGGL(mask_pack_rows_kernel, dim3(ceil_div((long)T * bh / 4, 256)), dim3(256), 0, s, ws + lo.z, ws + lo.xp0, B, H, T,
+                           dc, d->keep_in < 1.0f ? 1 : 0);
+    }
     AS_CHECK_LAUNCH();
     FlowArgs fa;
     fa.wp = ws + lo.wp; fa.bias = c.biases; fa.bias_stride = c.bstride;
@@ -757,9 +929,11 @@
         AS_CHECK_ARG(p.nfw > 0, "lstm_fwd_ctc: this shape does not take the fused CTC head (amdspeech_lstm_ctc_fusable)");
         fa.cf = ctc_head_args(d, head, ws, lo, panels, p.nfw); fa.cf_on = 1; fa.cf_nfw = p.nfw;
         fa.cf.lengths = c.lengths; fa.cf.err = err; fa.cf.limit = fa.limit;
-        if (int rc = ctc_prepare_targets(s, head->dense_labels, c.lengths, T, B, head->C, head->U, head->ctc_ws)) return rc;
-        hipLaunchKernelGGL(ctc_pack_wo_kernel, dim3(ceil_div((H / 16) * CF_NTC * 64, 256)), dim3(256), 0, s, head->w_out, ws + lo.wopack, H, head->C);
-        AS_CHECK_LAUNCH();
+        if (!c.one_launch) {
+            if (int rc = ctc_prepare_targets(s, head->dense_labels, c.lengths, T, B, head->C, head->U, head->ctc_ws)) return rc;
+            hipLaunchKernelGGL(ctc_pack_wo_kernel, dim3(ceil_div((H / 16) * CF_NTC * 64, 256)), dim3(256), 0, s, head->w_out, ws + lo.wopack, H, head->C);
+            AS_CHECK_LAUNCH();
+        }
         AS_CHECK_HIP(hipFuncSetAttribute(reinterpret_cast<const void*>(p.fwd_flow), hipFuncAttributeMaxDynamicSharedMemorySize, (int)p.fwd_lds));
     }
     prof_begin(0, s);
@@ -778,6 +952,7 @@
         AS_CHECK_LAUNCH();
         if (int rc = flow_fill_fwd_panels(g_side, d, ws, lo, 1 - set)) return rc;
         if (int rc = flow_arm_publish(ws, 1 - set)) return rc;
+        if (c.one_launch) flow_set_bwd_ahead(ws, true);
     }
     return AMDSPEECH_OK;
 }
@@ -861,6 +1036,9 @@
 
 static int lstm_fwd(hipStream_t s, FwdCall c) {
     if (int rc = fwd_prologue(s, c)) return rc;
+    if (c.in != nullptr && !c.one_launch)
+        if (int rc = gemm_f32(s, false, false, c.d->T * c.d->B, c.d->H, c.in->D, c.in->x, c.in->D, c.in->w_in, c.d->H, c.ws + c.lo.z, c.d->H,
+                              c.in->b_in, false)) return rc;
     switch (c.p.fwd) {
         case Path::flow: return fwd_flow(s, c);
         case Path::big: case Path::big1: return fwd_big(s, c);
@@ -949,12 +1127,15 @@
     float* ws = c.ws;
     const int T = d->T, B = d->B, H = d->H, L = d->L;
     unsigned* err = reinterpret_cast<unsigned*>(ws + lo.sync);
-    int* progress = reinterpret_cast<int*>(err) + 8;
-    unsigned* tickets = err + 16;
+    const bool ahead = (d->flags & AMDSPEECH_LSTM_ARMED) != 0 && flow_take_bwd_ahead(ws);
+    int* progress = reinterpret_cast<int*>(err) + (ahead ? FLOW_BWD_AHEAD : 8);
+    unsigned* tickets = err + (ahead ? FLOW_BWD_AHEAD + 8 : 16);
     if (!(d->flags & AMDSPEECH_LSTM_ARMED))
         if (int rc = flow_fill_bwd_panels(s, d, ws, lo, c.head != nullptr)) return rc;
-    AS_CHECK_HIP(hipMemsetD32Async(reinterpret_cast<hipDeviceptr_t>(progress), T, 8, s));
-    AS_CHECK_HIP(hipMemsetAsync(tickets, 0, 16 * sizeof(unsigned), s));
+    if (!ahead) {
+        AS_CHECK_HIP(hipMemsetD32Async(reinterpret_cast<hipDeviceptr_t>(progress), T, 8, s));
+        AS_CHECK_HIP(hipMemsetAsync(tickets, 0, 16 * sizeof(unsigned), s));
+    }
 #if FLOW2_CHECK_ORDER
     AS_CHECK_HIP(hipMemsetD32Async(reinterpret_cast<hipDeviceptr_t>(ws + lo.dg), (int)FLOW_SENTINEL, (size_t)L * T * B * 4 * H, s));
     AS_CHECK_HIP(hipMemsetAsync(ws + lo.pdown, 0, (lo.total - lo.pdown) * sizeof(float), s));
@@ -1382,6 +1563,32 @@
                                       const float* h0, const float* c0, const amdspeech_ctc_head* head) {
     if (int rc = check_head(head, false)) return rc;
     return lstm_fwd(static_cast<hipStream_t>(stream), FwdCall{d, static_cast<float*>(ws), kernels, kernel_stride, biases, bias_stride, lengths, h0, c0, head});
+}
+static int check_input_head(const amdspeech_input_head* in) {
+    AS_CHECK_ARG(in != nullptr, "lstm_fwd_in: null input head");
+    AS_CHECK_ARG(in->x && in->w_in && in->b_in && in->D > 0, "lstm_fwd_in: null pointer or D = %d in the input head", in->D);
+    return AMDSPEECH_OK;
+}
+extern "C" int amdspeech_lstm_fwd_in(void* stream, const amdspeech_lstm_desc* d, void* ws, const float* kernels,
+                                     long kernel_stride, const float* biases, long bias_stride, const int* lengths,
+                                     const float* h0, const float* c0, const amdspeech_input_head* in) {
+    if (int rc = check_input_head(in)) return rc;
+    return lstm_fwd(static_cast<hipStream_t>(stream), FwdCall{d, static_cast<float*>(ws), kernels, kernel_stride, biases, bias_stride, lengths, h0, c0, nullptr, in});
+}
+extern "C" int amdspeech_lstm_fwd_ctc_in(void* stream, const amdspeech_lstm_desc* d, void* ws, const float* kernels,
+                                         long kernel_stride, const float* biases, long bias_stride, const int* lengths,
+                                         const float* h0, const float* c0, const amdspeech_ctc_head* head, const amdspeech_input_head* in) {
+    if (int rc = check_head(head, false)) return rc;
+    if (int rc = check_input_head(in)) return rc;
+    return lstm_fwd(static_cast<hipStream_t>(stream), FwdCall{d, static_cast<float*>(ws), kernels, kernel_stride, biases, bias_stride, lengths, h0, c0, head, in});
+}
+extern "C" int amdspeech_lstm_plan_input_fused(const amdspeech_lstm_desc* d, int D) {
+    if (check_desc(d) != AMDSPEECH_OK || D <= 0) return -1;
+    const LstmPlan p = lstm_plan(d, nullptr);
+    if (p.fwd != Path::flow) return 0;
+    GemmPlan gp;
+    const float* aligned = reinterpret_cast<const float*>(uintptr_t(256));
+    return input_gemm_fusable(p, D, aligned, aligned, aligned, aligned, &gp) ? 3 : 1;
 }
 extern "C" int amdspeech_lstm_bwd_ctc(void* stream, const amdspeech_lstm_desc* d, void* ws, const float* kernels,
                                       long kernel_stride, float* dkernels, float* dbiases, long bias_stride,
diff --git a/rnn-speech_amd/engine.py b/rnn-speech_amd/engine.py
--- a/rnn-speech_amd/engine.py
+++ b/rnn-speech_amd/engine.py
@@ -77,6 +77,7 @@
 _BESIDE_TAIL = os.environ.get("AMDSPEECH_BESIDE_TAIL", "1") != "0"
 _BIDIR_PAIR = os.environ.get("AMDSPEECH_BIDIR_PAIR", "1") != "0"
 _FUSED_CTC = os.environ.get("AMDSPEECH_FUSED_CTC", "1") != "0"
+_FUSED_INPUT = os.environ.get("AMDSPEECH_FUSED_INPUT", "1") != "0"
 
 
 PRECISIONS = {"f32": 0, "bf16x3": 1, "bf16": 2}
@@ -136,6 +137,7 @@
         self._ws, self._Tr = self.lstm_ws, max_T
         self._head = None
         self._per_diagonal = False
+        self._input_fused = 0
         self._paired = False
         self._ws_b = self.lstm_ws_b if self.bidirectional and not self.layerwise else None
         self._layer_path = None
@@ -198,7 +200,12 @@
         ws = self.lstm_ws.prefix(Tr)
         self._ws, self._Tr = ws, Tr
         ws.set_dropout(keep_in, keep_out, seed)
-        ops.linear_fwd(x[:Tr].view(Tr * B, D), self.p("input_w"), self.p("input_b"), out=ws.z0.view(Tr * B, self.H))
+        input_head = None
+        if _FUSED_INPUT and not self.normalization and not self.bidirectional and not per_diagonal:
+            input_head = ops.InputHead(x[:Tr].view(Tr * B, D), self.p("input_w"), self.p("input_b"))
+        else:
+            ops.linear_fwd(x[:Tr].view(Tr * B, D), self.p("input_w"), self.p("input_b"), out=ws.z0.view(Tr * B, self.H))
+        self._input_fused = ops.lstm_plan_input_fused(ws, D) if input_head is not None else 0
         if self.normalization:
             grp = self._dp_group() if self.sync_batch_norm else None
             if grp is not None and grp.world > 1:
@@ -228,7 +235,7 @@
             ops.lstm_fwd(ws, self.p("kernel_0"), self.layout.kernel_stride, self.p("bias_0"),
                          self.layout.bias_stride, lengths,
                          self.state_h if use_state else None, self.state_c if use_state else None, training=training,
-                         per_diagonal=per_diagonal, head=self._head)
+                         per_diagonal=per_diagonal, head=self._head, input_head=input_head)
         H = self.H
         if not self.bidirectional:
             if after_lstm is not None:
@@ -274,7 +281,8 @@
         return self.logits
 
     def kernel_path(self):
-        path = {"fused_ctc_head": self._head is not None, "paired": self._paired, "run_length": self._Tr}
+        path = {"fused_ctc_head": self._head is not None, "paired": self._paired, "run_length": self._Tr,
+                "input_fused": self._input_fused}
         if not self.layerwise:
             plan = ops.lstm_plan(self._ws, head=self._head, per_diagonal=self._per_diagonal)
             path["lstm_fwd"], path["lstm_bwd"] = ("big1" if self._paired else plan["fwd_path"]), plan["bwd_path"]
diff --git a/rnn-speech_amd/lib.py b/rnn-speech_amd/lib.py
--- a/rnn-speech_amd/lib.py
+++ b/rnn-speech_amd/lib.py
@@ -26,6 +26,10 @@
 class CtcHead(C.Structure):
     _fields_ = [("w_out", C.c_void_p), ("b_out", C.c_void_p), ("logits", C.c_void_p), ("dense_labels", C.c_void_p),
                 ("loss", C.c_void_p), ("dlogits", C.c_void_p), ("ctc_ws", C.c_void_p), ("C", C.c_int), ("U", C.c_int)]
+
+
+class InputHead(C.Structure):
+    _fields_ = [("x", C.c_void_p), ("w_in", C.c_void_p), ("b_in", C.c_void_p), ("D", C.c_int)]
 
 
 class LstmPlanInfo(C.Structure):
@@ -123,6 +127,9 @@
     "amdspeech_lstm_fwd_pair": (_I, [_P, C.POINTER(LstmDesc), _P, _P, _P, C.POINTER(LstmDesc), _P, _P, _P, _L, _L, _P, _P, _P]),
     "amdspeech_lstm_bwd_pair": (_I, [_P, C.POINTER(LstmDesc), _P, _P, _P, _P, C.POINTER(LstmDesc), _P, _P, _P, _P, _L, _L, _P]),
     "amdspeech_lstm_fwd_ctc": (_I, [_P, C.POINTER(LstmDesc), _P, _P, _L, _P, _L, _P, _P, _P, C.POINTER(CtcHead)]),
+    "amdspeech_lstm_fwd_in": (_I, [_P, C.POINTER(LstmDesc), _P, _P, _L, _P, _L, _P, _P, _P, C.POINTER(InputHead)]),
+    "amdspeech_lstm_fwd_ctc_in": (_I, [_P, C.POINTER(LstmDesc), _P, _P, _L, _P, _L, _P, _P, _P, C.POINTER(CtcHead), C.POINTER(InputHead)]),
+    "amdspeech_lstm_plan_input_fused": (_I, [C.POINTER(LstmDesc), _I]),
     "amdspeech_lstm_bwd_ctc": (_I, [_P, C.POINTER(LstmDesc), _P, _P, _L, _P, _P, _L, _P, C.POINTER(CtcHead)]),
     "amdspeech_lstm_dropout_multipliers": (_I, [_P, C.POINTER(LstmDesc), _I, _I, _P]),
     "amdspeech_lstm_plan": (_I, [C.POINTER(LstmDesc), _I, _I, C.POINTER(LstmPlanInfo)]),
diff --git a/rnn-speech_amd/ops.py b/rnn-speech_amd/ops.py
--- a/rnn-speech_amd/ops.py
+++ b/rnn-speech_amd/ops.py
@@ -334,6 +334,25 @@
                             _p(dlogits).value if dlogits is not None else None, _p(ctc_ws.buf).value, C_, dense_labels.shape[1])
 
 
+class InputHead(object):
+
+    def __init__(self, x, w_in, b_in):
+        _chk_f32(x, w_in, b_in)
+        if x.dim() != 2 or tuple(w_in.shape) != (x.shape[1], b_in.shape[0]):
+            raise ValueError("InputHead: x %r, w_in %r, b_in %r" % (tuple(x.shape), tuple(w_in.shape), tuple(b_in.shape)))
+        self.keep = (x, w_in, b_in)
+        self.c = _l.InputHead(_p(x).value, _p(w_in).value, _p(b_in).value, int(x.shape[1]))
+
+
+def lstm_plan_input_fused(ws, D, per_diagonal=False):
+    d = _l.LstmDesc(ws.desc.T, ws.desc.B, ws.desc.H, ws.desc.L, ws.desc.keep_in, ws.desc.keep_out, ws.desc.seed, ws.desc.precision,
+                    _l.LSTM_PER_DIAGONAL if per_diagonal else 0)
+    n = int(ws.lib.amdspeech_lstm_plan_input_fused(C.byref(d), int(D)))
+    if n < 0:
+        raise ValueError("lstm_plan_input_fused: bad descriptor or D")
+    return n
+
+
 def lstm_ctc_fusable(ws, C_, U, per_diagonal=False):
     if per_diagonal:
         return False
@@ -361,7 +380,8 @@
     return n
 
 
-def lstm_fwd(ws, kernels, kernel_stride, biases, bias_stride, lengths, h0=None, c0=None, training=False, per_diagonal=False, head=None):
+def lstm_fwd(ws, kernels, kernel_stride, biases, bias_stride, lengths, h0=None, c0=None, training=False, per_diagonal=False, head=None,
+             input_head=None):
     _chk_i32(lengths)
     _chk_f32(h0, c0)
     root, key = ws._root, (ws.T, int(ws.desc.precision))
@@ -375,7 +395,18 @@
                      (_l.LSTM_INJECT_TIMEOUT if inject else 0))
     root._fwd_seen = False
     try:
-        if head is None:
+        if input_head is not None:
+            if tuple(input_head.keep[0].shape) != (ws.T * ws.B, input_head.c.D) or input_head.keep[2].shape[0] != ws.H:
+                raise ValueError("lstm_fwd: the input head has %r rows x features, the layout needs %r and H = %d"
+                                 % (tuple(input_head.keep[0].shape), (ws.T * ws.B, input_head.c.D), ws.H))
+            if head is None:
+                _l.check(ws.lib.amdspeech_lstm_fwd_in(_stream(), C.byref(ws.desc), _p(ws.buf), _p(kernels), kernel_stride, _p(biases),
+                                                      bias_stride, _p(lengths), _p(h0), _p(c0), C.byref(input_head.c)), "lstm_fwd_in")
+            else:
+                _l.check(ws.lib.amdspeech_lstm_fwd_ctc_in(_stream(), C.byref(ws.desc), _p(ws.buf), _p(kernels), kernel_stride, _p(biases),
+                                                          bias_stride, _p(lengths), _p(h0), _p(c0), C.byref(head.c),
+                                                          C.byref(input_head.c)), "lstm_fwd_ctc_in")
+        elif head is None:
             _l.check(ws.lib.amdspeech_lstm_fwd(_stream(), C.byref(ws.desc), _p(ws.buf), _p(kernels), kernel_stride,
                                                _p(biases), bias_stride, _p(lengths), _p(h0), _p(c0)), "lstm_fwd")
         else:
```
